# everpeace/kube-throttler

Hardware: AMD Instinct MI355X
Metric: pod_throttle_decisions_per_sec (higher is better)
Workload: dtype int64; 1 GPU; configs[2]: 1M pods x 1k Throttle+ClusterThrottle, D=8; pods_total=1000000, pods_per_gpu=1000000, throttles=1000, dims=8, labels_per_pod=8, namespaces=64, step=reconcile(aggregate+allreduce+finalize,apply)+check(all pods), streams=one, kernel_variant=indexed, parallelism=pods row-sharded x1, throttles replicated, exchange=none

## Files before the change

include/kt_engine.h:

```cpp
#ifndef KT_ENGINE_H
#define KT_ENGINE_H

#include <stdint.h>
#include "kt_snapshot.h"

#ifdef __cplusplus
extern "C" {
#endif

#define KT_OK 0
#define KT_ERR_INVALID_ARGUMENT (-1)
#define KT_ERR_OUT_OF_RANGE (-2)
#define KT_ERR_DEVICE (-3)
#define KT_ERR_OVERFLOW_RISK (-4)
#define KT_ERR_NOT_READY (-5)
#define KT_ERR_NO_DEVICE (-6)
#define KT_ERR_UNSUPPORTED (-7)

#define KT_STATUS_NOT_AFFECTED 0
#define KT_STATUS_NOT_THROTTLED 1
#define KT_STATUS_ACTIVE 2
#define KT_STATUS_INSUFFICIENT 3
#define KT_STATUS_POD_REQUESTS_EXCEEDS_THRESHOLD 4
#define KT_STATUS_ERROR 255
// ... 135 lines not shown
#define KT_KERNEL_FINALIZE 2
#define KT_KERNEL_PREPARE 3
#define KT_KERNEL_REDUCE 4
#define KT_KERNEL_COUNT 5
int32_t kt_timing_enable(kt_engine* e, int32_t on);
int32_t kt_timing_read(kt_engine* e, int32_t kernel, double* total_ms, int64_t* launches);
int32_t kt_timing_reset(kt_engine* e);
int32_t kt_synchronize(kt_engine* e, void* stream);
const char* kt_kernel_name(kt_engine* e, int32_t kernel);
#define KT_COUNTER_FEW_CHECKS 0
#define KT_COUNTER_COMPILES 1
#define KT_COUNTER_INDEX_CHUNKS 2
#define KT_COUNTER_INDEX_WORDS 3
#define KT_COUNTER_NS_WORD_VISITS 4
#define KT_COUNTER_NS_ROWS 5
#define KT_COUNTER_NS_CHUNK_VISITS 6
#define KT_COUNTER_INDEX_IMAGE_WORDS 7
#define KT_COUNTER_SLOW_THROTTLES 8
#define KT_COUNTER_PACKED_WORDS 9
#define KT_COUNTER_VIEW_BUILDS 10
#define KT_COUNTER_AGG_WORKGROUPS 11
#define KT_COUNTER_MATCH_CACHE_BUILDS 12
#define KT_COUNTER_MATCH_CACHE_SCANS 13
#define KT_COUNTER_MATCH_CACHE_PLANES 14
#define KT_COUNTER_MATCH_CACHE_AGG_SCANS 15
int64_t kt_counter(kt_engine* e, int32_t which);
int32_t kt_paged_check(kt_engine* const* pages, int32_t n_pages, int64_t n, const int64_t* pod_rows, int32_t on_equal,
                       uint64_t* out_summary, uint8_t* out_status);
int32_t kt_paged_reconcile(kt_engine* const* pages, int32_t n_pages, int64_t now_s, int32_t now_ns, uint32_t flags, int32_t n,
                           const kt_status* page_out, uint8_t* replaced_any, uint8_t* error_any);
int32_t kt_paged_admit(kt_engine* const* pages, int32_t n_pages, int64_t n, const int64_t* pod_rows, int32_t on_equal, uint32_t flags,
                       uint64_t* out_summary, uint8_t* out_status);
int32_t kt_paged_admit_gangs(kt_engine* const* pages, int32_t n_pages, int64_t n, const int64_t* pod_rows, int64_t n_gangs,
                             const int64_t* gang_off, int32_t on_equal, uint32_t flags, uint64_t* out_summary, uint8_t* out_status,
                             uint8_t* out_gang_admitted);
int32_t kt_paged_headroom(kt_engine* const* pages, int32_t n_pages, int64_t n, const int64_t* pod_rows, int32_t on_equal,
                          int64_t cap, int64_t* out_copies, int32_t* out_limiting);
#define KT_PREEMPT_REPRIEVE 0x1u
int32_t kt_paged_preempt(kt_engine* const* pages, int32_t n_pages, int64_t n, const int64_t* pod_rows, int64_t n_cand,
                         const int64_t* cand_rows, int64_t now_s, int32_t now_ns, int32_t on_equal, uint32_t flags,
                         int64_t* out_prefix , uint8_t* out_victims );
int32_t kt_paged_preempt_gangs(kt_engine* const* pages, int32_t n_pages, int64_t n, const int64_t* pod_rows, int64_t n_gangs,
                               const int64_t* gang_off, int64_t n_cand, const int64_t* cand_rows, int64_t now_s, int32_t now_ns,
                               int32_t on_equal, uint32_t flags, int64_t* out_prefix ,
                               uint8_t* out_victims , int64_t* out_blocker );
int32_t kt_paged_forecast(kt_engine* const* pages, int32_t n_pages, int64_t n, const int64_t* pod_rows, int64_t n_inst, const int64_t* inst_s,
                          const int32_t* inst_ns, int32_t on_equal, int64_t* out_first ,
                          uint8_t* out_verdicts );

int32_t kt_debug_reload_env(kt_engine* e);

int32_t kt_debug_match_planes(kt_engine* e, int32_t which, int64_t cap, uint64_t* out, int64_t* out_rows, int64_t* out_n, int32_t* out_planes);

#ifdef __cplusplus
}
#endif
#endif
```

kube_throttler_amd/csrc/kt_engine.cpp:

```cpp
#include "kt_engine_impl.h"

thread_local std::string g_create_error;

static bool getenv_flag(const char* name) {
  const char* v = getenv(name);
  return v && *v && *v != '0';
}
static void load_env_switches(kt_engine* e) {
  for (int k = 0; k < kSwCount; ++k) e->sw[k] = getenv_flag(kEnvSwitchName[k]);
  const char* cap = getenv("KT_REPRIEVE_LDS_CAP");
  const long cap_n = cap ? strtol(cap, nullptr, 10) : 0;
  e->reprieve_lds_cap_limit = cap_n > 0 && cap_n <= 0x7FFFFFFFl ? (uint32_t)cap_n : 0u;
}

void recs_invalidate_and_drain(kt_engine* e) {
  {
    std::lock_guard<std::mutex> g(e->recs_mu);
    e->recs_valid = false;
  }
  if (e->few_ready) std::lock_guard<std::mutex> drain(e->small_mu);
}

hipStream_t pick_stream(kt_engine* e, void* s) {
  hipStream_t st = s ? (hipStream_t)s : e->own_stream;
// ... 271 lines not shown
  e->cfg.kernel_variant &= 0xFF;
  if (e->incremental && e->cfg.kernel_variant != 0) {
    g_create_error = "KT_VARIANT_INCREMENTAL needs the indexed kernels (kernel_variant 0)";
    delete e;
    return KT_ERR_INVALID_ARGUMENT;
  }
  hipError_t r = hipSetDevice(dev);
  if (r == hipSuccess) r = hipStreamCreateWithFlags(&e->own_stream, hipStreamNonBlocking);
  const size_t cap = (size_t)cfg->pod_capacity;
  e->pods.cap = cfg->pod_capacity;
  e->pods.D = e->D;
  e->pods.L = e->L;
  e->pods.DS = kt::req_stride(e->D);
  e->pods.LS = kt::label_stride(e->L);
  if (r == hipSuccess) r = kt::kt_alloc_device((void**)&e->pods.ns, cap * 4);
  if (r == hipSuccess) r = kt::kt_alloc_device((void**)&e->pods.flags, cap * 4);
  if (r == hipSuccess) r = kt::kt_alloc_device((void**)&e->pods.req, cap * 8 * e->pods.DS);
  if (r == hipSuccess) r = kt::kt_alloc_device((void**)&e->pods.lpair, cap * 4 * e->pods.LS);
  if (r == hipSuccess) r = kt::kt_alloc_device((void**)&e->pods.lkey, cap * 4 * e->pods.LS);
  if (r == hipSuccess) r = kt::kt_alloc_device((void**)&e->pods.meta, cap * 8);
  e->pods.LA = 8;
  if (r == hipSuccess) r = hipMemsetAsync(e->pods.flags, 0, cap * 4, e->own_stream);
  if (r == hipSuccess) r = hipMemsetAsync(e->pods.meta, 0, cap * 8, e->own_stream);
  if (r == hipSuccess) r = hipMemsetAsync(e->pods.lpair, 0, cap * 4 * e->pods.LS, e->own_stream);
  if (r == hipSuccess) r = hipMemsetAsync(e->pods.lkey, 0, cap * 4 * e->pods.LS, e->own_stream);
  if (r == hipSuccess) r = hipStreamSynchronize(e->own_stream);
  if (r != hipSuccess) {
    g_create_error = std::string("device setup failed: ") + hipGetErrorString(r);
    kt_engine_destroy(e);
    return KT_ERR_DEVICE;
  }
  e->ns.resize((size_t)cfg->namespace_capacity);
  e->thr.resize((size_t)cfg->throttle_capacity);
  *out = e;
  return KT_OK;
}

int32_t kt_engine_destroy(kt_engine* e) {
  if (!e) return KT_OK;
  (void)hipSetDevice(e->device);
  (void)hipDeviceSynchronize();
  if (e->comm) (void)rccl()->CommDestroy(e->comm);
  if (e->pods.ns) (void)hipFree(e->pods.ns);
  if (e->pods.flags) (void)hipFree(e->pods.flags);
  if (e->pods.req) (void)hipFree(e->pods.req);
  if (e->pods.lpair) (void)hipFree(e->pods.lpair);
  if (e->pods.lkey) (void)hipFree(e->pods.lkey);
  if (e->pods.meta) (void)hipFree(e->pods.meta);
  e->d_latom.release();
  e->d_overflow.release();
  e->views.release();
  e->d_carry.release();
  e->d_mc.release();
  if (e->h_mc_rows) (void)hipHostFree(e->h_mc_rows);
  if (e->mc_rows_ev) (void)hipEventDestroy(e->mc_rows_ev);
  e->d_slab_tag.release();
  e->d_row_mask.release();
  e->d_req_sums.release();
  e->d_ticket.release();
  if (e->h_small) (void)hipHostFree(e->h_small);
  if (e->h_few) (void)hipHostFree(e->h_few);
  e->d_few_acc.release();
  e->d_few_ticket.release();
  for (auto& ev : e->recs_ev)
    if (ev) (void)hipEventDestroy(ev);
  if (e->admit_pages_ev) (void)hipEventDestroy(e->admit_pages_ev);
  if (e->preempt_pages_ev) (void)hipEventDestroy(e->preempt_pages_ev);
  if (e->small_stream) (void)hipStreamDestroy(e->small_stream);
  if (e->h_stage) (void)hipHostFree(e->h_stage);
  for (auto& sl : e->ev_slots) {
    if (sl.ev) (void)hipEventDestroy(sl.ev);
    if (sl.h) (void)hipHostFree(sl.h);
  }
  if (e->h_overflow) (void)hipHostFree(e->h_overflow);
  DevBuf<uint32_t>* u32s[] = {&e->d_thr_term_off, &e->d_term_thr, &e->d_term_req_off, &e->d_req_key, &e->d_req_val_off,
                              &e->d_req_val, &e->d_ns_term_ok, &e->d_thr_flags, &e->d_thrl_flag, &e->d_thrl_has,
                              &e->d_ovr_off, &e->d_out_thrl_flag, &e->d_out_thrl_has};
  for (auto* b : u32s) b->release();
  DevBuf<uint8_t>* u8s[] = {&e->d_term_flags, &e->d_req_op, &e->d_ns_valid, &e->d_ovr_flags, &e->d_out_calc_updated,
                            &e->d_out_thrl_pod, &e->d_out_error, &e->d_recs2[0], &e->d_recs2[1], &e->d_wvimg[0], &e->d_wvimg[1], &e->d_status, &e->d_stage, &e->d_ev_stage, &e->d_slab, &e->d_admit, &e->d_admit_pages, &e->d_preempt_pages, &e->d_gang_out};
  for (auto* b : u8s) b->release();
  e->d_status_fp.release(); e->d_spec_fp.release(); e->d_summary.release(); e->d_rows.release(); e->d_gang_off.release();
  e->d_headroom_copies.release(); e->d_headroom_limiting.release();
  e->d_preempt_prefix.release(); e->d_preempt_victims.release(); e->d_preempt_partial.release(); e->d_preempt_gang_off.release(); e->d_preempt_blocker.release(); e->d_reprieve_ws.release();
  e->d_forecast_first.release(); e->d_forecast_verdicts.release(); e->d_forecast_inst_s.release(); e->d_forecast_inst_ns.release();
  e->d_forecast_gang_off.release(); e->d_forecast_blocker.release();
  e->d_used_hi.release(); e->d_out_used_hi.release();
  e->d_ovr_begin_s.release(); e->d_ovr_end_s.release(); e->d_ovr_begin_ns.release(); e->d_ovr_end_ns.release();
  e->d_partial.release();
  e->d_out_next_s.release();
  e->d_agg.release();
  e->d_out_next_ns.release();
  e->d_sp.release();
  AmountDev* ams[] = {&e->d_spec, &e->d_calc, &e->d_used, &e->d_reserved, &e->d_ovr_thr, &e->d_out_used, &e->d_out_calc};
  for (auto* a : ams) a->release();
  kt::release_index(e->dindex);
  for (auto& f : e->fam)
    for (auto& pr : f.pool) {
      (void)hipEventDestroy(pr.first);
      (void)hipEventDestroy(pr.second);
    }
  if (e->own_stream) (void)hipStreamDestroy(e->own_stream);
  delete e;
  return KT_OK;
}

// ... 70 lines not shown
  *launches = (int64_t)f.used;
  return KT_OK;
}

int32_t kt_synchronize(kt_engine* e, void* stream) {
  if (!e) return KT_ERR_INVALID_ARGUMENT;
  LaunchLock lk(e);
  KT_HIP(e, hipSetDevice(e->device));
  KT_HIP(e, hipStreamSynchronize(pick_stream(e, stream)));
  return KT_OK;
}

int32_t kt_debug_reload_env(kt_engine* e) {
  if (!e) return KT_ERR_INVALID_ARGUMENT;
  StateLock lk(e);
  load_env_switches(e);
  return KT_OK;
}

int32_t kt_debug_match_planes(kt_engine* e, int32_t which, int64_t cap, uint64_t* out, int64_t* out_rows, int64_t* out_n, int32_t* out_planes) {
  if (!e || which < 0 || which > 1 || cap < 0 || !out_n || !out_planes || (cap > 0 && !out)) return KT_ERR_INVALID_ARGUMENT;
  LaunchLock lk(e);
  KT_HIP(e, hipSetDevice(e->device));
  if (e->last_stream) KT_HIP(e, hipStreamSynchronize(e->last_stream));
  *out_n = 0, *out_planes = 0;
  const uint32_t planes = e->mc_planes;
  if (!e->mc_valid || e->program_dirty || e->mc_gen != e->program_gen || e->mc_planes_gen != e->program_gen || !e->mc_pending.empty() || !e->d_mc.p ||
      planes == 0u || planes > (uint32_t)kt::kMatchPlanes || e->d_mc.cap < (size_t)planes * (size_t)e->cfg.pod_capacity)
    return e->fail(KT_ERR_NOT_READY, "no current match cache: none built for this program, or rows wait for their refresh");
  const ScanView& cv = e->views.countable;
  hipStream_t s = e->own_stream;
  int64_t n = e->pod_rows_hi;
  uint64_t stride = (uint64_t)e->cfg.pod_capacity;
  const uint64_t* src = e->d_mc.p;
  if (which == 1) {
    if (!cv.valid || !cv.mx_valid || !cv.mx.p || !cv.rows.p || !cv.d_n.p || cv.mx_planes != planes || cv.mx.cap < (size_t)planes * ((size_t)cv.cap + 1))
      return e->fail(KT_ERR_NOT_READY, "the countable scan view holds no current planes");
    unsigned long long dn = 0;
    KT_HIP(e, hipMemcpyAsync(&dn, cv.d_n.p, 8, hipMemcpyDeviceToHost, s));
    KT_HIP(e, hipStreamSynchronize(s));
    n = (int64_t)std::min<unsigned long long>(std::min<unsigned long long>(dn, cv.n + (unsigned long long)cv.extra), (unsigned long long)cv.cap);
    stride = (uint64_t)cv.cap + 1u, src = cv.mx.p;
  }
  *out_n = n, *out_planes = (int32_t)planes;
  if (cap == 0 || n == 0) return KT_OK;
  if (cap < n) return e->fail(KT_ERR_OUT_OF_RANGE, "cap=%lld < %lld", (long long)cap, (long long)n);
  for (uint32_t k = 0; k < planes; ++k)
    KT_HIP(e, hipMemcpyAsync(out + (size_t)k * (size_t)cap, src + (size_t)k * stride, (size_t)n * 8, hipMemcpyDeviceToHost, s));
  if (which == 1 && out_rows) KT_HIP(e, hipMemcpyAsync(out_rows, cv.rows.p, (size_t)n * 8, hipMemcpyDeviceToHost, s));
  KT_HIP(e, hipStreamSynchronize(s));
  return KT_OK;
}

int64_t kt_counter(kt_engine* e, int32_t which) {
  if (!e) return -1;
  switch (which) {
    case KT_COUNTER_FEW_CHECKS: return e->few_served.load(std::memory_order_relaxed);
    case KT_COUNTER_COMPILES: return e->n_compiles.load(std::memory_order_relaxed);
    case KT_COUNTER_INDEX_CHUNKS: return e->ctr_index_chunks.load(std::memory_order_relaxed);
    case KT_COUNTER_INDEX_WORDS: return e->ctr_index_words.load(std::memory_order_relaxed);
    case KT_COUNTER_NS_ROWS: return e->ctr_ns_rows.load(std::memory_order_relaxed);
    case KT_COUNTER_NS_WORD_VISITS: return e->ctr_ns_word_visits.load(std::memory_order_relaxed);
    case KT_COUNTER_NS_CHUNK_VISITS: return e->ctr_ns_chunk_visits.load(std::memory_order_relaxed);
    case KT_COUNTER_INDEX_IMAGE_WORDS: return e->ctr_index_image_words.load(std::memory_order_relaxed);
    case KT_COUNTER_SLOW_THROTTLES: return e->ctr_slow_throttles.load(std::memory_order_relaxed);
    case KT_COUNTER_PACKED_WORDS: return e->ctr_packed_words.load(std::memory_order_relaxed);
    case KT_COUNTER_AGG_WORKGROUPS: return e->ctr_agg_workgroups.load(std::memory_order_relaxed);
    case KT_COUNTER_VIEW_BUILDS: return e->ctr_view_builds.load(std::memory_order_relaxed);
    case KT_COUNTER_MATCH_CACHE_BUILDS: return e->ctr_mc_builds.load(std::memory_order_relaxed);
    case KT_COUNTER_MATCH_CACHE_SCANS: return e->ctr_mc_scans.load(std::memory_order_relaxed);
    case KT_COUNTER_MATCH_CACHE_PLANES: return e->ctr_mc_planes.load(std::memory_order_relaxed);
    case KT_COUNTER_MATCH_CACHE_AGG_SCANS: return e->ctr_mc_agg_scans.load(std::memory_order_relaxed);
    default: return -1;
  }
}

int32_t kt_partial_layout(int32_t n_dims, int32_t* stride, int32_t* off_values, int32_t* off_presence, int32_t* off_pods,
                          int32_t* off_errors) {
  if (n_dims < 1 || n_dims > KT_MAX_DIMS) return KT_ERR_INVALID_ARGUMENT;
  if (stride) *stride = kt::partial_stride(n_dims);
  if (off_values) *off_values = 0;
  if (off_presence) *off_presence = kt::partial_off_presence(n_dims);
  if (off_pods) *off_pods = kt::partial_off_pods(n_dims);
  if (off_errors) *off_errors = kt::partial_off_errors(n_dims);
  return KT_OK;
}

const char* kt_kernel_name(kt_engine* e, int32_t kernel) {
  if (!e || kernel < 0 || kernel >= KT_KERNEL_COUNT) return "";
  return e->last_kernel[kernel];
}
```

kube_throttler_amd/csrc/kt_engine_check.cpp:

```cpp
#include "kt_engine_impl.h"

static int32_t ensure_check_recs(kt_engine* e, int32_t on_equal, int DT, hipStream_t s) {
  if (e->recs_valid && e->recs_eq == (on_equal != 0) && e->recs_DT == DT) return KT_OK;
  recs_invalidate_and_drain(e);
  {
    TimedLaunch tl(e, KT_KERNEL_PREPARE, s);
    kt::launch_prepare_check(e->tt, e->thr_rows_hi, e->D, DT, on_equal != 0, e->recs_ptr(), req_bound(e), s);
  }
  if (e->few_ready) KT_HIP(e, hipEventRecord(e->recs_ev[e->recs_cur], s));
  std::lock_guard<std::mutex> g(e->recs_mu);
  e->recs_ev_pending[e->recs_cur] = e->few_ready;
  e->recs_prev_valid = false;
  ++e->recs_seq[e->recs_cur];
  e->recs_valid = true;
  e->recs_eq = on_equal != 0;
  e->recs_DT = DT;
  return KT_OK;
}

int32_t match_cache_for_scan(kt_engine* e, hipStream_t s, kt::MatchCacheArgs& mc) {
  mc = kt::MatchCacheArgs();
  if (e->sw[kSw_NO_MATCH_CACHE] || e->cfg.kernel_variant != 0 || e->incremental || e->program_dirty || e->pod_rows_hi <= 0) return KT_OK;
  if (!kt::match_cache_fits(e->dindex) || e->hindex.has_slow || e->n_overflow != 0 || e->pods.LA > 8 || !e->pods.latom) return KT_OK;
  if (e->mc_planes_gen != e->program_gen) {
    const kt::BmChunk& ch = e->dindex.h_chunks[0];
    const uint32_t* rng = (const uint32_t*)(e->hindex.bm_images.data() + ch.img_off + ch.off_nsl_rng);
    uint32_t longest = 0;
    for (uint32_t n = 0; n < e->hindex.n_ns; ++n) longest = std::max(longest, rng[2 * n + 1] - rng[2 * n]);
    e->mc_planes = longest, e->mc_planes_gen = e->program_gen;
    e->ctr_mc_planes.store((int64_t)longest, std::memory_order_relaxed);
  }
  const uint32_t planes = e->mc_planes;
  if (!kt::check_replays_match_cache(e->pods, e->sp, e->dindex, planes, e->n_overflow != 0, e->sw[kSw_CHECK_ONE_PER_CU])) return KT_OK;
  const uint64_t stride = (uint64_t)e->cfg.pod_capacity;
  ScanView& cv = e->views.countable;
  kt::MatchViewPlanes vp;
  if (cv.valid && cv.mx_valid && cv.mx.p && cv.pos.p && cv.mx_planes == planes && e->mc_gen == e->program_gen)
    vp.mx = cv.mx.p, vp.pos = cv.pos.p, vp.stride = (uint64_t)cv.cap + 1u;
  else
    cv.mx_valid = false;
  if (!e->mc_valid || e->mc_gen != e->program_gen) {
    if (e->d_mc.cap < (size_t)planes * stride) {
      if (e->last_stream) KT_HIP(e, hipStreamSynchronize(e->last_stream));
      KT_HIP(e, e->d_mc.reserve((size_t)planes * stride));
    }
    order_behind_ingest(e, s);
    if (!kt::launch_build_match_cache(e->pods, e->pod_rows_hi, nullptr, e->dindex, e->d_mc.p, stride, planes, s, &vp)) {
      cv.mx_valid = false;
      return KT_OK;
    }
    KT_HIP(e, hipGetLastError());
    e->mc_valid = true, e->mc_gen = e->program_gen;
    e->mc_pending.clear();
    e->ctr_mc_builds.fetch_add(1, std::memory_order_relaxed);
  } else if (!e->mc_pending.empty()) {
    const size_t n = e->mc_pending.size();
    if (!e->h_mc_rows) {
      KT_HIP(e, hipHostMalloc((void**)&e->h_mc_rows, (size_t)kPatchBatchMax * 8, hipHostMallocDefault));
      KT_HIP(e, hipEventCreateWithFlags(&e->mc_rows_ev, hipEventDisableTiming));
    } else if (e->mc_rows_ev_used) {
      KT_HIP(e, hipEventSynchronize(e->mc_rows_ev));
    }
    memcpy(e->h_mc_rows, e->mc_pending.data(), n * 8);
    order_behind_ingest(e, s);
    if (!kt::launch_build_match_cache(e->pods, (int64_t)n, e->h_mc_rows, e->dindex, e->d_mc.p, stride, planes, s, &vp)) {
      e->mc_valid = false, cv.mx_valid = false;
      e->mc_pending.clear();
      return KT_OK;
    }
    KT_HIP(e, hipGetLastError());
    KT_HIP(e, hipEventRecord(e->mc_rows_ev, s));
    e->mc_rows_ev_used = true;
    e->mc_pending.clear();
  }
  mc.mw = e->d_mc.p, mc.stride = stride, mc.planes = planes;
  return KT_OK;
}

static int32_t check_launch_locked(kt_engine* e, int64_t n, const int64_t* pod_rows, int32_t on_equal, uint32_t flags,
                                   hipStream_t s, bool allow_small = true) {
  e->headroom_ready = false;
  e->preempt_ready = false;
  e->forecast_ready = false;
  if (pod_rows) {
    for (int64_t i = 0; i < n; ++i)
      if (pod_rows[i] < 0 || pod_rows[i] >= e->cfg.pod_capacity)
        return e->fail(KT_ERR_OUT_OF_RANGE, "pod row %lld", (long long)pod_rows[i]);
  } else if (n > e->cfg.pod_capacity) {
    return e->fail(KT_ERR_OUT_OF_RANGE, "n=%lld > pod_capacity", (long long)n);
  }
  int32_t rc = ensure_ready(e, s);
  if (rc != KT_OK) return rc;
  const bool want_status = (flags & KT_CHECK_STATUS_MATRIX) != 0;
  const size_t T = (size_t)e->thr_rows_hi;
  if (e->d_summary.cap < (size_t)n + 1 || (want_status && e->d_status.cap < (size_t)n * T + 64) ||
      (pod_rows && e->d_rows.cap < (size_t)n + 1)) {
    if (e->last_stream) KT_HIP(e, hipStreamSynchronize(e->last_stream));
    KT_HIP(e, e->d_summary.reserve((size_t)n + 1));
    if (want_status) KT_HIP(e, e->d_status.reserve((size_t)n * T + 64));
    if (pod_rows) KT_HIP(e, e->d_rows.reserve((size_t)n + 1));
  }
  const bool small = allow_small && e->cfg.kernel_variant != 1 && n > 0 && n <= kt::kCheckSmallMax;
  kt::CheckSmall sm{};
  if (small) {
    if (!e->h_small) {
      KT_HIP(e, hipHostMalloc((void**)&e->h_small, (size_t)kt::kCheckSmallMax * 8, hipHostMallocMapped));
      KT_HIP(e, e->d_ticket.reserve(16));
      KT_HIP(e, hipMemsetAsync(e->d_ticket.p, 0, 16 * 4, s));
    }
    sm.ticket = e->d_ticket.p;
    sm.host_summary = e->h_small;
    if (pod_rows && n <= 8) {
      sm.n_inline = (uint32_t)n;
      for (int64_t k = 0; k < 8; ++k) sm.inline_rows[k] = pod_rows[k < n ? k : n - 1];
    }
  }
  if (pod_rows && n && !sm.n_inline) {
    KT_HIP(e, hipMemcpyAsync(e->d_rows.p, pod_rows, (size_t)n * 8, hipMemcpyHostToDevice, s));
    KT_HIP(e, hipStreamSynchronize(s));
  }
  const int DT = e->cfg.kernel_variant == 1 ? kt::dt_bucket(e->D) : kt::dt_bucket_ix(e->D);
  if ((rc = ensure_check_recs(e, on_equal, DT, s)) != KT_OK) return rc;
  kt::MatchCacheArgs mc;
  if (e->cfg.kernel_variant != 1 && !pod_rows && !small && !want_status && n > 0 && n <= e->cfg.pod_capacity && e->dindex.n_chunks == 1 &&
      !e->sw[kSw_FORCE_NS_ORDER] && !e->sw[kSw_CHECK_ONE_PER_CU]) {
    if ((rc = match_cache_for_scan(e, s, mc)) != KT_OK) return rc;
  }
  {
    TimedLaunch tl(e, KT_KERNEL_CHECK, s);
    if (e->cfg.kernel_variant == 1)
      kt::launch_check_dense(e->pods, n, pod_rows ? e->d_rows.p : nullptr, e->sp, e->uses_keys, e->recs_ptr(),
                             e->d_summary.p, want_status ? e->d_status.p : nullptr, s),
          e->last_kernel[KT_KERNEL_CHECK] = "kt_check_dense";
    else {
      const bool by_ns = !pod_rows && !small && n == e->pod_rows_hi && (e->dindex.n_chunks > 1 || e->sw[kSw_FORCE_NS_ORDER]) && !e->sw[kSw_NO_NS_ORDER];
      if (by_ns && (rc = settle_view_patches(e, s)) != KT_OK) return rc;
      ScanView& av = e->views.all_rows;
      if (by_ns && (!av.valid || (int64_t)av.n != e->pod_rows_hi)) {
        const ViewSpec spec{false, true, kt::check_sweep_blocks, e->pod_rows_hi, false};
        KT_HIP(e, e->d_carry.reserve((size_t)e->pod_rows_hi + 1));
        if ((rc = list_view_rows(e, av, spec, s)) != KT_OK) return rc;
        if ((rc = copy_view_records(e, av, spec, 0, s)) != KT_OK) return rc;
        av.valid = true;
      }
      kt::CheckByNs view{av.meta.p, av.latom.p, e->d_carry.p};
      if (by_ns && av.range_G) view.wg_range = av.range.p, view.wg_range_G = av.range_G;
      if (by_ns && !want_status && e->dindex.n_slow == 0 && e->n_overflow == 0 && e->dindex.n_chunks > 1 && !e->sw[kSw_NO_VERDICT_IMAGES]) {
        const int b = e->recs_cur;
        if (e->wvimg_seq[b] != e->recs_seq[b] || e->wvimg_gen[b] != e->program_gen || e->wvimg_DT[b] != DT) {
          KT_HIP(e, e->d_wvimg[b].reserve(kt::verdict_images_bytes(e->dindex.bm_words, e->D)));
          TimedLaunch tl2(e, KT_KERNEL_PREPARE, s);
          kt::launch_build_verdict_images(e->dindex, e->dindex.bm_words, e->recs_ptr(), e->thr_rows_hi, e->D, e->d_wvimg[b].p, s);
          e->wvimg_seq[b] = e->recs_seq[b], e->wvimg_gen[b] = e->program_gen, e->wvimg_DT[b] = DT;
        }
        view.wv_img = e->d_wvimg[b].p, view.wv_total_words = e->dindex.bm_words;
      }
      const char* k = kt::launch_check_indexed(e->pods, n, by_ns ? av.rows.p : pod_rows ? e->d_rows.p : nullptr, e->sp, e->d_sp.p, e->dindex,
                                               e->recs_ptr(), e->d_summary.p, want_status ? e->d_status.p : nullptr, s,
                                               small ? &sm : nullptr, e->n_overflow != 0, by_ns ? &view : nullptr, e->sw[kSw_CHECK_ONE_PER_CU],
                                               mc.mw ? &mc : nullptr);
      if (mc.used) e->ctr_mc_scans.fetch_add(1, std::memory_order_relaxed);
      if (!k) return e->fail(KT_ERR_UNSUPPORTED, "%d throttle rows exceed the indexed check kernel's LDS budget (use kernel_variant 1)", e->thr_rows_hi);
      e->last_kernel[KT_KERNEL_CHECK] = k;
    }
  }
  KT_HIP(e, hipGetLastError());
  e->check_n = n;
  e->check_in_h_small = small;
  e->check_T = e->thr_rows_hi;
  e->check_has_status = want_status;
  e->check_ready = true;
  e->last_stream = s;
  return KT_OK;
}

int32_t kt_check_launch(kt_engine* e, int64_t n, const int64_t* pod_rows, int32_t on_equal, uint32_t flags, void* stream) {
  if (!e || n < 0) return KT_ERR_INVALID_ARGUMENT;
  LaunchLock lk(e);
  KT_HIP(e, hipSetDevice(e->device));
// ... 1286 lines not shown
```

kube_throttler_amd/csrc/kt_engine_impl.h:

```cpp
#pragma once
#include <hip/hip_runtime.h>
#include <dlfcn.h>

#include <algorithm>
#include <cstdarg>
#include <cstdio>
#include <cstring>
#include <memory>
#include <atomic>
#include <chrono>
#include <mutex>
#include <shared_mutex>
#include <string>
#include <unordered_set>
#include <vector>

#include "../../include/kt_engine.h"
#include "kt_index.h"
#include "kt_launch.h"


#define KT_INTERNAL __attribute__((visibility("hidden")))

namespace kte {
// ... 50 lines not shown
struct HostNamespace {
  bool valid = false;
  std::vector<std::pair<uint32_t, uint32_t>> labels;
};

template <class T>
struct DevBuf {
  T* p = nullptr;
  size_t cap = 0;
  hipError_t reserve(size_t n) {
    if (n <= cap && p) return hipSuccess;
    if (p) (void)hipFree(p);
    p = nullptr;
    cap = 0;
    size_t want = std::max<size_t>(n, 16);
    hipError_t e = kt::kt_alloc_device((void**)&p, want * sizeof(T));
    if (e == hipSuccess) cap = want;
    return e;
  }
  void release() {
    if (p) (void)hipFree(p);
    p = nullptr;
    cap = 0;
  }
};

struct AmountDev {
  DevBuf<int64_t> v;
  DevBuf<uint32_t> present;
  DevBuf<int64_t> count;
  DevBuf<uint8_t> has_count;
  hipError_t reserve(size_t n, int D) {
    hipError_t e;
    if ((e = v.reserve(n * D)) != hipSuccess) return e;
    if ((e = present.reserve(n)) != hipSuccess) return e;
    if ((e = count.reserve(n)) != hipSuccess) return e;
    return has_count.reserve(n);
  }
  kt::AmountTab tab() const { return kt::AmountTab{v.p, present.p, count.p, has_count.p}; }
  void release() { v.release(); present.release(); count.release(); has_count.release(); }
};

struct ScanView {
  DevBuf<int64_t> rows;
  DevBuf<unsigned long long> d_n;
  unsigned long long n = 0;
  DevBuf<uint64_t> meta;
  DevBuf<uint16_t> latom;
  DevBuf<int64_t> req;
  DevBuf<uint64_t> pk;
  kt::PackPlan pack;
  DevBuf<int32_t> pos;
  DevBuf<uint64_t> mx;
  uint32_t mx_planes = 0;
  bool mx_valid = false;
  DevBuf<uint32_t> range;
  int range_G = 0;
  int64_t cap = 0;
  int64_t extra = 0;
  bool by_ns = false;
  bool valid = false;
  void release() { rows.release(); d_n.release(); meta.release(); latom.release(); req.release(); pk.release(); pos.release(); range.release(); mx.release(); mx_valid = false; }
};
struct ViewSpec {
  bool countable_only;
  bool by_ns;
  int (*grid)(int64_t);
  int64_t rows_cap;
  bool requests;
};
struct ScanViews {
  ScanView countable;
  ScanView all_rows;
  DevBuf<unsigned long long> d_ns_cursor;
  std::vector<unsigned long long> h_ns_end;
  std::vector<uint32_t> h_range;
  DevBuf<uint32_t> d_dirty;
  bool check_dirty = false;
  void invalidate() { countable.valid = false, all_rows.valid = false; }
  void release() { countable.release(); all_rows.release(); d_ns_cursor.release(); d_dirty.release(); }
};

struct AmountHostFlat {
  std::vector<int64_t> v;
  std::vector<uint32_t> present;
  std::vector<int64_t> count;
  std::vector<uint8_t> has_count;
  void resize(size_t n, int D) {
    v.assign(n * D, 0);
    present.assign(n, 0);
    count.assign(n, 0);
    has_count.assign(n, 0);
  }
  void set(size_t i, int D, const HostAmount& a) {
    for (int d = 0; d < D; ++d) v[i * D + d] = (a.present >> d) & 1u ? a.v[d] : 0;
    present[i] = a.present;
    count[i] = a.has_count ? a.count : 0;
    has_count[i] = a.has_count;
  }
  void get(size_t i, int D, HostAmount& a) const {
    for (int d = 0; d < D; ++d) a.v[d] = v[i * D + d];
    a.present = present[i];
    a.count = count[i];
    a.has_count = has_count[i];
  }
};

struct TimingFamily {
  std::vector<std::pair<hipEvent_t, hipEvent_t>> pool;
  size_t used = 0;
};

}
using namespace kte;

extern thread_local std::string g_create_error;


enum EnvSwitch { kSw_FEED_NO_STAGE, kSw_FORCE_NS_ORDER, kSw_INGEST_EVENT_WAIT, kSw_NO_FEED_FEW, kSw_NO_FEED_FUSION, kSw_NO_FUSED, kSw_NO_NS_ORDER, kSw_NO_PACK, kSw_NO_SCAN_VIEW, kSw_NO_SWEEP, kSw_NO_VERDICT_IMAGES, kSw_NO_WG_RANGES, kSw_SYNC_INGEST, kSw_INGEST_TRUST_FENCE, kSw_NO_VIEW_PATCH, kSw_CHECK_ONE_PER_CU, kSw_AGG_SMALL_WINDOW, kSw_AGG_ONE_PER_CU, kSw_NO_MATCH_CACHE, kSw_NO_MATCH_CACHE_AGG, kSwCount };
static const char* const kEnvSwitchName[kSwCount] = {"KT_FEED_NO_STAGE", "KT_FORCE_NS_ORDER", "KT_INGEST_EVENT_WAIT", "KT_NO_FEED_FEW", "KT_NO_FEED_FUSION", "KT_NO_FUSED", "KT_NO_NS_ORDER", "KT_NO_PACK", "KT_NO_SCAN_VIEW", "KT_NO_SWEEP", "KT_NO_VERDICT_IMAGES", "KT_NO_WG_RANGES", "KT_SYNC_INGEST", "KT_INGEST_TRUST_FENCE", "KT_NO_VIEW_PATCH", "KT_CHECK_ONE_PER_CU", "KT_AGG_SMALL_WINDOW", "KT_AGG_ONE_PER_CU", "KT_NO_MATCH_CACHE", "KT_NO_MATCH_CACHE_AGG"};
struct kt_engine {
  bool sw[kSwCount] = {};
  uint32_t reprieve_lds_cap_limit = 0;
  kt_config cfg{};
  std::shared_mutex mu;
  std::mutex small_mu;
  std::mutex ingest_mu;
  std::mutex op_mu;
  std::mutex recs_mu;
  std::mutex err_mu;
  std::string err;
  int device = 0;
  hipStream_t own_stream = nullptr;
  int D = 0, L = 0;

  kt::PodTable pods{};
  int64_t pod_rows_hi = 0;
  unsigned __int128 max_abs[KT_MAX_DIMS] = {0};
  uint64_t or_abs[KT_MAX_DIMS] = {0};
  ScanViews views;
  bool cut_plain = false;
  void* cur_launch_lock = nullptr;
  std::atomic<int64_t> ctr_index_chunks{0}, ctr_index_words{0}, ctr_index_image_words{0}, ctr_ns_rows{0}, ctr_ns_word_visits{0}, ctr_ns_chunk_visits{0}, ctr_slow_throttles{0}, ctr_packed_words{0}, ctr_agg_workgroups{0}, ctr_view_builds{0}, ctr_mc_builds{0}, ctr_mc_scans{0}, ctr_mc_planes{0}, ctr_mc_agg_scans{0};
  DevBuf<uint16_t> d_latom;
  DevBuf<uint64_t> d_mc;
  int64_t* h_mc_rows = nullptr;
  hipEvent_t mc_rows_ev = nullptr;
  bool mc_rows_ev_used = false;
  std::vector<int64_t> mc_pending;
  bool mc_valid = false;
  uint64_t mc_gen = ~0ull;
  uint64_t mc_planes_gen = ~0ull;
  uint32_t mc_planes = 0;
  DevBuf<unsigned long long> d_overflow;
  unsigned long long n_overflow = 0;
  static constexpr int kEvSlots = 8;
  static constexpr size_t kEvSlotBytes = 64 * 1024;
  struct EvSlot {
    uint8_t* h = nullptr;
    hipEvent_t ev = nullptr;
    bool used = false;
  } ev_slots[kEvSlots];
  int ev_next = 0;
  std::atomic<bool> ingest_pending{false};
  hipEvent_t ingest_ev = nullptr;
  std::atomic<hipEvent_t> ingest_unretired{nullptr};
  hipStream_t ingest_stream = nullptr;
  unsigned long long* h_overflow = nullptr;
  bool overflow_in_flight = false;
  unsigned long long ingest_seq = 0;
  unsigned long long ingest_spin_seq = 0;
  bool req_sums_valid = true;
  unsigned __int128 req_sum_bound[KT_MAX_DIMS] = {0};
  DevBuf<unsigned long long> d_req_sums;
  DevBuf<uint8_t> d_row_mask;
  DevBuf<uint32_t> d_slab_tag;
  uint32_t slab_epoch = 0;
  bool neg_seen = false;

  std::vector<HostNamespace> ns;
  uint64_t ns_gen = 1;
  int32_t ns_rows_hi = 0;
  int64_t pod_ns_hi = 0;
  size_t ns_compiled = 0;
  std::vector<HostThrottle> thr;
  int32_t thr_rows_hi = 0;
  bool program_dirty = true;
  bool spec_dirty = false;
  bool status_host_dirty = true;
  bool reserved_dev_newer = false;
  bool incremental = false;
  bool agg_valid = false;
  DevBuf<unsigned long long> d_agg;
  bool recs_valid = false;
  bool recs_eq = false;
  int recs_DT = 0;
  bool status_dev_newer = false;

// ... 283 lines not shown
```

kube_throttler_amd/csrc/kt_engine_reconcile.cpp:

```cpp
#include "kt_engine_impl.h"

Rccl* rccl() {
  static Rccl r;
  static std::once_flag once;
  std::call_once(once, [] {
    for (const char* name : {"librccl.so.1", "librccl.so", "/opt/rocm/lib/librccl.so.1"}) {
      r.lib = dlopen(name, RTLD_NOW | RTLD_LOCAL);
      if (r.lib) break;
    }
    if (!r.lib) {
      r.err = std::string("cannot load librccl.so: ") + (dlerror() ? dlerror() : "?");
      return;
    }
    r.GetUniqueId = (decltype(r.GetUniqueId))dlsym(r.lib, "ncclGetUniqueId");
    r.CommInitRank = (decltype(r.CommInitRank))dlsym(r.lib, "ncclCommInitRank");
    r.AllReduce = (decltype(r.AllReduce))dlsym(r.lib, "ncclAllReduce");
    r.CommDestroy = (decltype(r.CommDestroy))dlsym(r.lib, "ncclCommDestroy");
    r.GetErrorString = (decltype(r.GetErrorString))dlsym(r.lib, "ncclGetErrorString");
    if (!r.GetUniqueId || !r.CommInitRank || !r.AllReduce || !r.CommDestroy) r.err = "librccl.so lacks the nccl* entry points";
  });
  return &r;
}
static constexpr int kNcclInt64 = 4, kNcclSum = 0;

// ... 171 lines not shown
    e->agg_pending = true, e->agg_words = words, e->agg_gen = e->program_gen;
    return KT_OK;
  }
  const bool by_ns = (e->dindex.n_chunks > 1 || e->sw[kSw_FORCE_NS_ORDER]) && !e->sw[kSw_NO_NS_ORDER];
  if ((rc = settle_view_patches(e, s)) != KT_OK) return rc;
  ScanView& cv = e->views.countable;
  if (cv.valid && cv.extra && !(!e->sw[kSw_NO_SCAN_VIEW] && (by_ns || e->dindex.n_chunks == 1))) cv.valid = false;
  const bool two_view = !e->sw[kSw_NO_SCAN_VIEW] && !e->sw[kSw_NO_PACK] && e->cfg.kernel_variant != 1 && !by_ns && !e->incremental && !e->wide &&
                        e->dindex.n_chunks == 1;
  const kt::AggTwoLaunch two_launch{!e->sw[kSw_AGG_ONE_PER_CU], e->sw[kSw_AGG_SMALL_WINDOW], e->n_overflow != 0, e->pods.LA};
  if (cv.valid && cv.pack.headroom >= (uint32_t)kt::kPackHeadroomBitsTwo && !(two_view && kt::aggregate_two_per_cu_fits(e->dindex, cv.pack, two_launch)))
    cv.valid = false;
  kt::MatchCacheArgs mc;
  if (two_view && two_launch.enabled && !two_launch.small_window && !two_launch.overflow_pods && e->pods.LA <= 8 && !e->sw[kSw_NO_MATCH_CACHE_AGG] &&
      !e->sw[kSw_CHECK_ONE_PER_CU]) {
    if ((rc = match_cache_for_scan(e, s, mc)) != KT_OK) return rc;
  }
  if (e->cfg.kernel_variant != 1 && (!cv.valid || cv.by_ns != by_ns)) {
    if (e->last_stream && e->last_stream != s) KT_HIP(e, hipStreamSynchronize(e->last_stream));
    const ViewSpec spec{true, by_ns, kt::aggregate_blocks, e->cfg.pod_capacity, true};
    if ((rc = list_view_rows(e, cv, spec, s)) != KT_OK) return rc;
    const int64_t headroom = std::min<int64_t>(std::max<int64_t>(65536, (int64_t)cv.n / 16), e->cfg.pod_capacity - (int64_t)cv.n);
    const bool view_scan = !e->sw[kSw_NO_SCAN_VIEW] && (cv.by_ns || e->dindex.n_chunks == 1);
    cv.pack = kt::PackPlan();
    if (view_scan && !e->incremental && !e->wide && !e->sw[kSw_NO_PACK] && !e->dindex.has_long) {
      const int64_t cap = (int64_t)cv.n + headroom;
      uint64_t slab_pods = kt::aggregate_slab_pods(cap, kt::aggregate_blocks(cap));
      if (cv.range_G) slab_pods = std::max<uint64_t>(slab_pods, (uint64_t)kt::wg_range_cap((int64_t)cv.n, cv.range_G) + 64u);
      cv.pack = kt::make_pack_plan(e->D, e->max_abs, e->or_abs, e->neg_seen, slab_pods, true, kt::pack_max_words(e->D));
      if (cv.pack.nw && cv.pack.rec_bytes > e->dindex.cut_thr_bytes) cv.pack = kt::PackPlan();
      if (two_view && cv.pack.nw) {
        const uint64_t slab_pods2 = kt::aggregate_slab_pods(cap, kt::aggregate_blocks(cap, kt::kAggWorkgroupsTwo));
        const kt::PackPlan two = kt::make_pack_plan(e->D, e->max_abs, e->or_abs, e->neg_seen, slab_pods2, false, 3,
                                                    kt::kPackHeadroomBitsTwo);
        if (two.nw && kt::aggregate_two_per_cu_fits(e->dindex, two, two_launch)) cv.pack = two;
      }
    }
    if (!cv.pack.nw && kt::agg_rec_bytes(e->D, e->incremental) > e->dindex.cut_thr_bytes) {
      upgrade_launch_lock(e);
      e->cut_plain = true, e->program_dirty = true;
      return aggregate_locked(e, s, allow_fused);
    }
    if (!e->sw[kSw_NO_SCAN_VIEW] && (rc = copy_view_records(e, cv, spec, headroom, s)) != KT_OK) return rc;
    cv.valid = true;
  }
  const bool replay = mc.mw != nullptr && mc.planes <= (uint32_t)kt::kMatchReplay && two_view && cv.valid && cv.pack.nw && cv.pk.p &&
                      cv.pack.headroom >= (uint32_t)kt::kPackHeadroomBitsTwo && kt::aggregate_two_per_cu_fits(e->dindex, cv.pack, two_launch);
  if (replay && !(cv.mx_valid && cv.mx_planes == mc.planes)) {
    const size_t need = (size_t)mc.planes * ((size_t)cv.cap + 1);
    if (cv.mx.cap < need) {
      if (e->last_stream) KT_HIP(e, hipStreamSynchronize(e->last_stream));
      KT_HIP(e, cv.mx.reserve(need));
    }
    const int64_t listed = std::min<int64_t>((int64_t)cv.n + cv.extra, cv.cap);
    kt::launch_gather_match_planes(mc.mw, mc.stride, mc.planes, cv.rows.p, listed, cv.mx.p, (uint64_t)cv.cap + 1u, s);
    KT_HIP(e, hipGetLastError());
    cv.mx_planes = mc.planes, cv.mx_valid = true;
  }
  if (words && e->clean_partial != (const void*)e->partial()) KT_HIP(e, hipMemsetAsync(e->partial(), 0, words * 8, s));
  e->clean_partial = nullptr;
  {
    TimedLaunch tl(e, KT_KERNEL_AGGREGATE, s);
    std::unique_ptr<TimedLaunch> tr;
    const bool defer = allow_fused && !e->incremental && !e->wide && e->dindex.n_chunks == 1 && !e->sw[kSw_NO_FUSED];
    auto after_scan = [&]() {
      tl.stop_now();
      if (!(defer && cv.pack.nw)) tr.reset(new TimedLaunch(e, KT_KERNEL_REDUCE, s));
    };
    const int n_pass = e->wide ? 2 : 1;
    for (int pass = 0; pass < n_pass; ++pass) {
      const int limb = e->wide ? pass + 1 : 0;
      unsigned long long* target = e->partial() + (size_t)pass * block_words;
      if (e->cfg.kernel_variant == 1) {
        kt::launch_aggregate_dense(e->pods, e->pod_rows_hi, e->sp, e->uses_keys, target, s, limb);
        e->last_kernel[KT_KERNEL_AGGREGATE] = "kt_aggregate_dense";
      } else {
        kt::AggScan sc;
        sc.n = (int64_t)cv.n, sc.rows = cv.rows.p, sc.counts = e->incremental, sc.nonneg = !e->neg_seen;
        sc.overflow_pods = two_launch.overflow_pods;
        sc.small_window = two_launch.small_window;
        sc.one_per_cu = !two_launch.enabled;
        sc.limb = limb;
        sc.by_ns = !e->sw[kSw_NO_SCAN_VIEW] && (cv.by_ns || e->dindex.n_chunks == 1);
        if (sc.by_ns) sc.n += cv.extra;
        if (sc.by_ns) sc.v_meta = cv.meta.p, sc.v_latom = cv.latom.p, sc.v_req = cv.pack.nw ? nullptr : cv.req.p;
        if (sc.by_ns && cv.pack.nw) sc.pk = &cv.pack, sc.v_pk = cv.pk.p;
        if (sc.by_ns && cv.by_ns && cv.range_G) sc.wg_range = cv.range.p, sc.wg_range_G = cv.range_G;
        if ((rc = slab_tags(e, sc, s)) != KT_OK) return rc;
        sc.defer_reduce = defer && sc.pk != nullptr;
        if (replay && sc.by_ns && sc.v_pk && limb == 0) sc.v_mx = cv.mx.p, sc.mx_stride = (uint64_t)cv.cap + 1u, sc.mx_planes = cv.mx_planes;
        const char* k = kt::launch_aggregate_indexed(e->pods, sc, e->sp, e->d_sp.p, e->dindex, target, e->d_slab.p, s,
                                                     pass == 0 ? std::function<void()>(after_scan) : std::function<void()>());
        if (sc.replayed) e->ctr_mc_agg_scans.fetch_add(1, std::memory_order_relaxed);
        if (!k && sc.refused) return e->fail(KT_ERR_OUT_OF_RANGE, "aggregate launch refused: %s", sc.refused);
        if (!k) return e->fail(KT_ERR_UNSUPPORTED, "a chunk of the selector index exceeds the aggregate kernel's LDS budget (use kernel_variant 1)");
        e->last_kernel[KT_KERNEL_AGGREGATE] = k;
        e->ctr_agg_workgroups.store((int64_t)sc.launched_blocks, std::memory_order_relaxed);
        e->ctr_packed_words.store(sc.launched_packed ? (int64_t)cv.pack.nw : 0, std::memory_order_relaxed);
        if (sc.defer_reduce && sc.launched_packed) e->fused_pending = true, e->fused_nb = sc.launched_blocks, e->fused_epoch = sc.epoch, e->fused_pack = cv.pack;
        e->last_kernel[KT_KERNEL_REDUCE] = e->fused_pending ? "(in kt_reduce_finalize_packed)" : sc.launched_packed ? "kt_reduce_packed_slabs" : "kt_reduce_bitmap_slabs";
      }
    }
  }
  KT_HIP(e, hipGetLastError());
  if (e->incremental) {
    KT_HIP(e, e->d_agg.reserve(words + 1));
    if (words) KT_HIP(e, hipMemcpyAsync(e->d_agg.p, e->partial(), words * 8, hipMemcpyDeviceToDevice, s));
    e->agg_valid = true;
  }
  e->last_stream = s;
  e->agg_pending = true, e->agg_words = words, e->agg_gen = e->program_gen;
  return KT_OK;
}

int32_t delta_scan(kt_engine* e, int64_t n, const int64_t* rows_dev, int64_t row0, int sign, hipStream_t s) {
  if (!e->incremental || !e->agg_valid || n <= 0 || e->thr_rows_hi == 0) return KT_OK;
  kt::AggScan sc;
  sc.n = n, sc.rows = rows_dev, sc.row0 = row0, sc.counts = true, sc.sign = sign, sc.overflow_pods = e->n_overflow != 0;
  sc.small_window = e->sw[kSw_AGG_SMALL_WINDOW];
  int32_t rc = slab_tags(e, sc, s);
  if (rc != KT_OK) return rc;
  const char* k = kt::launch_aggregate_indexed(e->pods, sc, e->sp, e->d_sp.p, e->dindex, e->d_agg.p, e->d_slab.p, s, nullptr);
  if (!k && sc.refused) return e->fail(KT_ERR_OUT_OF_RANGE, "aggregate launch refused: %s", sc.refused);
  if (!k) return e->fail(KT_ERR_UNSUPPORTED, "a chunk of the selector index exceeds the aggregate kernel's LDS budget");
  KT_HIP(e, hipGetLastError());
  return KT_OK;
}

int32_t finalize_locked(kt_engine* e, int64_t now_s, int32_t now_ns, uint32_t flags, hipStream_t s, bool consume,
                               const uint8_t* row_mask) {
  KT_CHECK_PARTIALS_CURRENT(e, "kt_finalize_launch");
  int32_t rc = ensure_ready(e, s);
  if (rc != KT_OK) return rc;
  if (!e->agg_pending) e->agg_wide = e->wide;
  e->agg_pending = false;
  kt::ReconcileOut out{e->d_out_used.tab(), e->d_out_calc.tab(), e->d_out_used_hi.p, e->d_out_calc_updated.p, e->d_out_thrl_flag.p,
                       e->d_out_thrl_has.p, e->d_out_thrl_pod.p, e->d_out_error.p, e->d_out_next_s.p, e->d_out_next_ns.p};
  const bool apply = (flags & KT_RECONCILE_APPLY) != 0;
  const int rec_DT = e->cfg.kernel_variant == 1 ? kt::dt_bucket(e->D) : kt::dt_bucket_ix(e->D);
  bool keep_prev;
  int wbuf;
  {
    std::lock_guard<std::mutex> g(e->recs_mu);
// ... 210 lines not shown
```

kube_throttler_amd/csrc/kt_index.cpp:

```cpp
#include "kt_index.h"

#include <algorithm>
#include <chrono>
#include <cstdio>
#include <cstdlib>
#include <cstring>
#include <map>
#include <thread>
#include <unordered_map>
#include <unordered_set>

#include "../../include/kt_snapshot.h"

namespace kt {

namespace {

struct BT {
  uint32_t g, t;
  bool adj;
  bool slow;
  uint32_t need;
  uint32_t n_pos;
  int64_t pos_key[5];
// ... 826 lines not shown
        if (g.cnt[w]++ == 0) g.words.push_back(w);
      g.ideal = std::min(g.ideal, ideal_n);
    }
    std::vector<ChunkPlan> plan;
    Maxima mx;
    for (Group& g : groups) {
      ordered(g.words, g.cnt);
      std::vector<uint32_t> cuts;
      (void)chunks_of(seq, g.cnt, g.members.size(), &mx, &cuts);
      size_t i0 = 0;
      for (uint32_t i1 : cuts) {
        ChunkPlan cp;
        cp.all = false, cp.served = g.members;
        cp.words.assign(seq.begin() + i0, seq.begin() + i1);
        std::sort(cp.words.begin(), cp.words.end());
        plan.push_back(std::move(cp));
        i0 = i1;
      }
    }
    return plan;
  }
  size_t visits(const std::vector<ChunkPlan>& plan) const {
    size_t v = 0;
    std::vector<uint8_t> in_chunk(W, 0);
    for (const ChunkPlan& cp : plan) {
      for (uint32_t w : cp.words) in_chunk[w] = 1;
      auto touches = [&](uint32_t n) {
        for (uint32_t w : ns_words[n])
          if (in_chunk[w]) return true;
        return false;
      };
      if (cp.all) {
        for (uint32_t n = 0; n < n_ns; ++n) v += touches(n);
      } else {
        for (uint32_t n : cp.served) v += touches(n);
      }
      for (uint32_t w : cp.words) in_chunk[w] = 0;
    }
    return v;
  }

  void emit(const std::vector<ChunkPlan>& plan_in) {
    const std::vector<uint64_t>&any = out.full_any, &vet = out.full_veto, &nsrows = out.full_nsrows;
    const std::vector<WordHdr>& hdr = out.full_hdr;
    const std::vector<uint32_t>&term_t = out.full_term_t, &term_g = out.full_term_g, &term_rank = out.full_term_rank;
    const std::vector<uint8_t>& real = out.full_real;
    uint64_t slab_run = 0;
    out.bm_chunks.clear();
    out.bm_images.clear();
    size_t total_words = 0;
    for (const ChunkPlan& cp : plan_in) total_words += cp.words.size();
    out.bm_images.reserve(((size_t)Rp * total_words * 8 * fam + total_words * (sizeof(WordHdr) + 64 * 10 + 64)) * 5 / 4 + plan_in.size() * ((size_t)n_ns + 8) * 4 * 4);
    out.bm_chunk_ns.clear();
    const uint32_t nsw = (n_ns + 31) / 32;
    out.ns_words = nsw ? nsw : 1u;
    out.bm_max_lds = 0, out.bm_max_thr = 0, out.bm_max_words = 0, out.bm_slab_bytes = 0;
    out.bm_rank_t.clear();
    out.ns_word_visits = 0, out.ns_chunk_visits = 0;
    uint32_t w_run = 0;
    Maxima mx;
    std::vector<ChunkPlan> work(plan_in.rbegin(), plan_in.rend());
    std::vector<uint64_t> irows;
    std::vector<uint32_t> words;
    while (!work.empty()) {
      ChunkPlan cp = std::move(work.back());
      work.pop_back();
      BmChunk ch{};
      const uint32_t nw = (uint32_t)cp.words.size();
      words = cp.words;
      uint32_t nv = 0;
      if (veto) {
        std::stable_partition(words.begin(), words.end(), [&](uint32_t w) { return has_veto(w); });
        for (uint32_t w : words) nv += has_veto(w);
      }
      const uint32_t veto_cols = veto ? nv + (nv < nw ? 1u : 0u) : 0u;
      ch.n_words = nw, ch.n_veto = nv;
      ch.zero_col = veto && nv < nw ? (nw + nv) * Rp * 8u : 0u;
      ch.ns_base = 0u, ch.ns_cnt = 0xFFFFFFFFu;
      ch.col_rows = Rp;
      std::vector<uint32_t> nsl_rng((size_t)n_ns * 2, 0u);
      std::vector<NsWord> nsl, cur;
      {
        std::unordered_map<uint64_t, std::vector<uint32_t>> by_hash;
        size_t si = 0;
        for (uint32_t n = 0; n < n_ns; ++n) {
          bool serve = cp.all;
          if (!cp.all) {
            while (si < cp.served.size() && cp.served[si] < n) ++si;
            serve = si < cp.served.size() && cp.served[si] == n;
          }
          if (!serve) continue;
          cur.clear();
          uint64_t h = 1469598103934665603ull;
          for (uint32_t w = 0; w < nw; ++w) {
            const uint64_t m = nsrows[(size_t)n * W + words[w]];
            if (!m) continue;
            cur.push_back(NsWord{w, word_form[words[w]], m});
            h = (h ^ w) * 1099511628211ull, h = (h ^ m) * 1099511628211ull;
          }
          if (cur.empty()) continue;
          uint32_t begin = ~0u;
          std::vector<uint32_t>& cands = by_hash[h];
          for (uint32_t b0 : cands) {
            if ((size_t)b0 + cur.size() > nsl.size()) continue;
            bool same = true;
            for (size_t q = 0; q < cur.size() && same; ++q) same = nsl[b0 + q].w == cur[q].w && nsl[b0 + q].mask == cur[q].mask;
            if (same) { begin = b0; break; }
          }
          if (begin == ~0u) {
            begin = (uint32_t)nsl.size();
            nsl.insert(nsl.end(), cur.begin(), cur.end());
            cands.push_back(begin);
          }
          nsl_rng[(size_t)n * 2] = begin, nsl_rng[(size_t)n * 2 + 1] = begin + (uint32_t)cur.size();
        }
      }
      const uint32_t rank0 = (uint32_t)out.bm_rank_t.size();
      std::vector<uint32_t> it((size_t)nw * 64, 0u), ig((size_t)nw * 64, 0u);
      std::vector<uint16_t> ir((size_t)nw * 64, 0);
      {
        uint32_t last_rank = ~0u;
        for (uint32_t w = 0; w < nw; ++w)
          for (uint32_t k = 0; k < 64; ++k) {
            const size_t c = (size_t)words[w] * 64 + k;
            it[(size_t)w * 64 + k] = term_t[c], ig[(size_t)w * 64 + k] = term_g[c];
            if (!real[c]) continue;
            if (term_rank[c] != last_rank) last_rank = term_rank[c], out.bm_rank_t.push_back(term_t[c] & kTermRowMask);
            ir[(size_t)w * 64 + k] = (uint16_t)(((uint32_t)out.bm_rank_t.size() - 1u - rank0) | ((term_t[c] & kTermAdj) ? kRankAdj : 0u));
            ch.has_slow |= (hdr[c >> 6].slow >> (c & 63)) & 1ull ? 1u : 0u;
            ch.has_adj |= (term_t[c] & kTermAdj) ? 1u : 0u;
          }
      }
      ch.n_thr = (uint32_t)out.bm_rank_t.size() - rank0;
      ch.rank0 = ch.n_thr ? rank0 : 0u;
      const size_t lds = image_lds(nw, nv, nsl.size());
      if (!fits(lds, nw, ch.n_thr, mx) && nw > 1 && all_splittable) {
        out.bm_rank_t.resize(rank0);
        ChunkPlan lo = cp, hi = cp;
        lo.words.assign(cp.words.begin(), cp.words.begin() + nw / 2), hi.words.assign(cp.words.begin() + nw / 2, cp.words.end());
        work.push_back(std::move(hi)), work.push_back(std::move(lo));
        continue;
      }
      ch.w0 = w_run;
      w_run += nw;
      irows.assign((size_t)Rp * (nw + veto_cols), 0ull);
      const size_t veto_plane = (size_t)Rp * nw;
      for (uint32_t r = 0; r < R; ++r)
        for (uint32_t w = 0; w < nw; ++w) {
          irows[(size_t)w * Rp + r] = any[(size_t)r * W + words[w]];
          if (veto && w < nv) irows[veto_plane + (size_t)w * Rp + r] = vet[(size_t)r * W + words[w]];
        }
      std::vector<WordHdr> ihdr(nw);
      for (uint32_t w = 0; w < nw; ++w) ihdr[w] = hdr[words[w]];
      for (uint32_t n = 0; n < n_ns; ++n) out.ns_word_visits += (int64_t)(nsl_rng[(size_t)n * 2 + 1] - nsl_rng[(size_t)n * 2]);
      {
        const size_t b0 = out.bm_chunk_ns.size();
        out.bm_chunk_ns.resize(b0 + out.ns_words, 0u);
        for (uint32_t n = 0; n < n_ns; ++n)
          if (nsl_rng[(size_t)n * 2 + 1] > nsl_rng[(size_t)n * 2]) out.bm_chunk_ns[b0 + (n >> 5)] |= 1u << (n & 31), ++out.ns_chunk_visits;
      }
      const void* src[7] = {irows.data(), ihdr.data(), nsl_rng.data(), nsl.data(), it.data(), ir.data(), ig.data()};
      const size_t bytes[7] = {irows.size() * 8, ihdr.size() * sizeof(WordHdr), nsl_rng.size() * 4, nsl.size() * sizeof(NsWord),
                               it.size() * 4,    ir.size() * 2,                 ig.size() * 4};
      uint32_t* offs[7] = {nullptr, &ch.off_hdr, &ch.off_nsl_rng, &ch.off_nsl, &ch.off_term_t, &ch.off_term_rank, &ch.off_term_g};
      size_t o = 0;
      const size_t img0 = out.bm_images.size();
      for (int k = 0; k < 7; ++k) {
        if (offs[k]) *offs[k] = (uint32_t)o;
        if (k == 4) ch.lds_bytes = (uint32_t)o;
        o += align16(bytes[k]);
      }
      out.bm_images.resize(img0 + o, 0);
      size_t oo = 0;
      for (int k = 0; k < 7; ++k) {
        if (bytes[k]) memcpy(out.bm_images.data() + img0 + oo, src[k], bytes[k]);
        oo += align16(bytes[k]);
      }
      ch.img_off = (uint32_t)img0, ch.img_bytes = (uint32_t)o;
      ch.slab_off = (uint32_t)(slab_run / 16);
      slab_run += agg_slab_area_bytes(ch.n_thr, thr_bytes);
      mx.lds = std::max(mx.lds, (size_t)ch.lds_bytes), mx.thr = std::max(mx.thr, (size_t)ch.n_thr), mx.nw = std::max(mx.nw, (size_t)nw);
      out.bm_max_lds = std::max(out.bm_max_lds, ch.lds_bytes);
      out.bm_max_thr = std::max(out.bm_max_thr, ch.n_thr);
      out.bm_max_words = std::max(out.bm_max_words, ch.n_words);
      out.bm_chunks.push_back(ch);
      if (getenv("KT_DEBUG_CHUNKS"))
        fprintf(stderr, "chunk %zu: %u words (%u with veto columns; first %u) lds %u B thr %u, serves %zu namespaces, %zu list entries\n", out.bm_chunks.size() - 1,
                nw, nv, nw ? words[0] : 0u, ch.lds_bytes, ch.n_thr, cp.all ? (size_t)n_ns : cp.served.size(), nsl.size());
      out.bm_slab_bytes = slab_run;
    }
    out.img_words = w_run;
  }
};

}

void cut_chunks(HostIndex& out, uint32_t agg_budget, uint32_t chk_budget, uint32_t thr_bytes, uint32_t chk_word, uint32_t thr_bytes_packed) {
// ... 26 lines not shown
  if (want_grouped || getenv("KT_CUT_PLAN_AUTO")) {
    std::vector<ChunkPlan> grouped = cut.plan_grouped();
    const size_t v_global = cut.visits(plan), v_grouped = cut.visits(grouped);
    if (getenv("KT_DEBUG_CHUNKS"))
      fprintf(stderr, "cut_chunks: global %zu chunks / %zu namespace visits, grouped %zu chunks / %zu namespace visits\n", plan.size(), v_global,
              grouped.size(), v_grouped);
    if (want_grouped || (v_grouped * 5 <= v_global * 4 && grouped.size() <= std::max<size_t>(8 * plan.size(), 64) && grouped.size() <= 2048))
      plan.swap(grouped), out.cut_grouped = true;
  }
  cut.emit(plan);
}

template <class T>
static hipError_t up(T*& dev, size_t& cap, const std::vector<T>& h, hipStream_t s) {
  const size_t need = h.size() + 1;
  if (need > cap || !dev) {
    if (dev) (void)hipFree(dev);
    dev = nullptr;
    cap = 0;
    hipError_t e = kt_alloc_device((void**)&dev, need * sizeof(T));
    if (e != hipSuccess) return e;
    cap = need;
  }
  if (!h.empty()) return hipMemcpyAsync(dev, h.data(), h.size() * sizeof(T), hipMemcpyHostToDevice, s);
  return hipSuccess;
}

void index_group_counts(HostIndex& h, uint32_t T) {
  h.thr_ngrp.assign(T, 0u);
  for (uint32_t t : h.bm_rank_t)
    if (t < T) ++h.thr_ngrp[t];
  h.nogroup.clear();
  for (uint32_t t = 0; t < T; ++t)
    if (!h.thr_ngrp[t]) h.nogroup.push_back(t);
}

hipError_t upload_index(const HostIndex& h, IndexDev& d, hipStream_t s) {
  hipError_t e;
  if ((e = up(d.thr_ngrp, d.cap_thr_ngrp, h.thr_ngrp, s)) != hipSuccess) return e;
  if ((e = up(d.nogroup, d.cap_nogroup, h.nogroup, s)) != hipSuccess) return e;
  d.n_nogroup = (uint32_t)h.nogroup.size();
  {
    const std::vector<uint32_t> zeros(h.thr_ngrp.size() + 1, 0u);
    if ((e = up(d.grp_arrive, d.cap_grp_arrive, zeros, s)) != hipSuccess) return e;
    if ((e = hipStreamSynchronize(s)) != hipSuccess) return e;
  }
  if ((e = up(d.slow_thr, d.cap_slow, h.slow_thr, s)) != hipSuccess) return e;
  d.n_slow = (uint32_t)h.slow_thr.size();
  if ((e = up(d.bm_blob, d.cap_bm_blob, h.bm_images, s)) != hipSuccess) return e;
  if ((e = up(d.bm_chunks, d.cap_bm_chunks, h.bm_chunks, s)) != hipSuccess) return e;
  if ((e = up(d.bm_rank_t, d.cap_bm_rank_t, h.bm_rank_t, s)) != hipSuccess) return e;
  if ((e = up(d.bm_chunk_ns, d.cap_bm_chunk_ns, h.bm_chunk_ns, s)) != hipSuccess) return e;
  d.ns_words = h.ns_words;
  if ((e = up(d.atom_table, d.cap_atom_table, h.atom_table, s)) != hipSuccess) return e;
  d.atom_mask = (uint32_t)h.atom_table.size() - 1;
  d.h_chunks = h.bm_chunks;
  d.n_chunks = (uint32_t)h.bm_chunks.size();
  d.bm_max_lds = h.bm_max_lds, d.bm_max_thr = h.bm_max_thr, d.bm_max_words = h.bm_max_words, d.bm_rows = h.bm_rows;
  d.bm_words = h.img_words;
  d.cut_thr_bytes = h.cut_thr_bytes;
  d.has_long = h.has_long;
  d.bm_slab_bytes = h.bm_slab_bytes;
  d.has_veto = h.has_veto ? 1u : 0u;
  d.max_need = h.max_need;
  d.n_atoms = (uint32_t)h.atoms.size();
  d.has_key_atoms = h.n_key_atoms ? 1u : 0u;
  d.la = h.la, d.rich = h.rich;
  if (getenv("KT_DEBUG_LDS"))
    fprintf(stderr, "bitmap index: %u words, %u rows (veto %d, need %u), %zu chunks, largest LDS part %u B, largest chunk %u throttles / %u words, %zu slow throttles\n",
            h.bm_words, h.bm_rows, (int)h.has_veto, h.max_need, h.bm_chunks.size(), h.bm_max_lds, h.bm_max_thr, h.bm_max_words, h.slow_thr.size());
  return hipSuccess;
}

void release_index(IndexDev& d) {
  if (d.slow_thr) (void)hipFree(d.slow_thr);
  if (d.bm_blob) (void)hipFree(d.bm_blob);
  if (d.bm_chunks) (void)hipFree(d.bm_chunks);
  if (d.bm_rank_t) (void)hipFree(d.bm_rank_t);
  if (d.thr_ngrp) (void)hipFree(d.thr_ngrp);
  if (d.nogroup) (void)hipFree(d.nogroup);
  if (d.grp_arrive) (void)hipFree(d.grp_arrive);
  if (d.bm_chunk_ns) (void)hipFree(d.bm_chunk_ns);
  if (d.atom_table) (void)hipFree(d.atom_table);
  d = IndexDev();
}

PackPlan make_pack_plan(int D, const unsigned __int128* max_abs, const uint64_t* or_abs, bool neg_seen, uint64_t n_slab_pods, bool pad_odd,
                        uint32_t max_words, int headroom_bits) {
  PackPlan pk;
  if (neg_seen || D < 1 || D > 16 || n_slab_pods == 0 || headroom_bits < 1 || headroom_bits > 16) return pk;
  const int MW = (int)std::min<uint32_t>(max_words ? max_words : 1u, kPackMaxWords);
  auto bitlen = [](unsigned __int128 x) { int b = 0; while (x) ++b, x >>= 1; return b; };
  const int H = headroom_bits;
  struct F { int d; uint32_t pos, w; };
  std::vector<F> fields[kPackMaxWords];
  uint32_t fill[kPackMaxWords] = {0, 0, 0, 0, 0, 0, 0, 0};
  pk.cnt_width = (uint8_t)std::max(bitlen(n_slab_pods), H);
  if (pk.cnt_width > 64 - H) return PackPlan();
  fields[0].push_back({-1, 0u, pk.cnt_width});
  fill[0] = pk.cnt_width;
  uint32_t nw = 1;
  for (int d = 0; d < D; ++d) {
    if (max_abs[d] == 0) continue;
    const int sh = or_abs[d] ? __builtin_ctzll(or_abs[d]) : 0;
    const int w = std::max(bitlen((max_abs[d] >> sh) * (unsigned __int128)n_slab_pods), H);
    if (w > 64 - H) return PackPlan();
    int k = 0;
    while (k < MW && fill[k] + (uint32_t)w > 64u) ++k;
    if (k == MW) return PackPlan();
    pk.word[d] = (uint8_t)k, pk.pos[d] = (uint8_t)fill[k], pk.width[d] = (uint8_t)w, pk.shift[d] = (uint8_t)sh;
    fields[k].push_back({d, fill[k], (uint32_t)w});
    fill[k] += (uint32_t)w;
    nw = std::max(nw, (uint32_t)k + 1u);
  }
  for (uint32_t k = 0; k < nw; ++k) {
    const size_t n = fields[k].size();
    pk.top_pos[k] = (uint8_t)fields[k][n - 1].pos;
    for (size_t i = 0; i < n; ++i) {
      const F& f = fields[k][i];
      const bool top = i + 1 == n;
      const uint32_t cls = top ? 2u : (uint32_t)(i & 1u);
      if (cls == 0u) pk.even[k] |= ((1ull << f.w) - 1ull) << f.pos;
      const uint32_t desc = pack_desc(k, cls, top ? 0u : f.pos, f.w + (uint32_t)H, f.d >= 0 ? pk.shift[f.d] : 0u);
      if (f.d >= 0) pk.desc[f.d] = desc; else pk.cnt_desc = desc;
    }
  }
  pk.nw = nw;
  pk.headroom = (uint32_t)H;
  pk.stride = nw <= 2 ? 2u : nw <= 4 ? 4u : 8u;
  uint32_t units = nw + 1u;
  if (pad_odd && !(units & 1u)) ++units;
  pk.rec_bytes = units * 8u;
  return pk;
}

// ... 2 lines not shown
```

kube_throttler_amd/csrc/kt_index.h:

```cpp
#pragma once
#include <hip/hip_runtime.h>
#include <stdint.h>

#include <algorithm>
#include <functional>
#include <vector>

#include "kt_device.h"

namespace kt {

constexpr uint32_t kKeyAtom = 0x80000000u;
constexpr uint32_t kMaxIndexedTerms = 512;
constexpr uint32_t kCheckWordLds = 64u * 8u + 560u;

constexpr uint32_t kTermAdj = 0x80000000u;
constexpr uint32_t kTermReal = 0x40000000u;
constexpr uint32_t kTermRowMask = 0x000FFFFFu;
constexpr uint16_t kRankAdj = 0x8000u;

struct ThrInfo {
  bool live;
  bool cluster;
  uint32_t ns;
};

struct alignas(16) WordHdr {
  uint64_t univ;
  uint64_t m2;
  uint64_t m3;
  uint64_t slow;
  uint64_t m4;
  uint64_t m5;
  uint64_t pad[2];
};
static_assert(sizeof(WordHdr) == 64, "the scans address a word's header by a shift");
struct alignas(16) NsWord {
  uint32_t w;
  uint32_t flags;
  uint64_t mask;
};
constexpr uint32_t kNsWordVeto = 1u;
constexpr uint32_t kNsWordNeed3 = 2u;

struct BmChunk {
  uint32_t w0, n_words;
  uint32_t rank0, n_thr;
  uint32_t img_off, lds_bytes;
  uint32_t off_hdr, off_nsl_rng, off_nsl;
  uint32_t off_term_t, off_term_rank, off_term_g;
  uint32_t col_rows;
  uint32_t n_veto;
  uint32_t zero_col;
  uint32_t slab_off;
  uint32_t has_slow;
  uint32_t img_bytes;
  uint32_t has_adj;
  uint32_t ns_base, ns_cnt;
};

inline uint32_t image_col_rows(uint32_t rows) { return (rows + 31u) & ~31u; }

struct AtomId {
  uint32_t atom, id;
  uint32_t home;
};
constexpr int kAtomHomeShift = 48;
constexpr uint32_t kAtomIdMask = 0xFFFFu;

struct HostIndex {
  std::vector<uint32_t> slow_thr;
  uint32_t bm_words = 0;
  uint32_t bm_rows = 0;
  bool has_veto = false;
  uint32_t max_need = 0;
  uint32_t n_pair_keys = 0, n_key_atoms = 0;
  uint32_t n_keys = 0;
  bool has_slow = false;
  bool has_long = false;
  uint32_t la = 8;
  bool rich = false;
  std::vector<AtomId> atoms;
  std::vector<uint32_t> atom_key;
  std::vector<uint64_t> atom_table;
  std::vector<BmChunk> bm_chunks;
  std::vector<unsigned char> bm_images;
  std::vector<uint32_t> bm_rank_t;
  std::vector<uint32_t> thr_ngrp;
  std::vector<uint32_t> nogroup;
  std::vector<uint32_t> bm_chunk_ns;
  uint32_t ns_words = 0;
  uint32_t bm_max_lds = 0, bm_max_thr = 0, bm_max_words = 0;
  uint64_t bm_slab_bytes = 0;
  uint32_t cut_chk_budget = 0;
  uint32_t cut_thr_bytes = 0;
  bool agg_windowed = false;
  bool cut_grouped = false;
  uint32_t img_words = 0;
  int64_t ns_word_visits = 0;
  int64_t ns_chunk_visits = 0;
  uint32_t n_ns = 0;
  std::vector<uint64_t> full_any, full_veto, full_nsrows;
  std::vector<WordHdr> full_hdr;
  std::vector<uint32_t> full_term_t, full_term_g, full_term_rank;
  std::vector<uint8_t> full_real;
};

__host__ __device__ inline uint32_t agg_rec_bytes(int D, bool counts) {
  return (uint32_t)(((size_t)D * 8 + (counts ? (size_t)D * 4 + 4 : 8) + 15) & ~(size_t)15);
}

struct PackPlan {
  uint32_t nw = 0;
  uint32_t stride = 0;
  uint32_t rec_bytes = 0;
  uint8_t word[16] = {0}, pos[16] = {0}, width[16] = {0}, shift[16] = {0};
  uint8_t cnt_width = 0;
  uint64_t even[8] = {0, 0, 0, 0, 0, 0, 0, 0};
  uint8_t top_pos[8] = {0, 0, 0, 0, 0, 0, 0, 0};
  uint32_t desc[16] = {0};
  uint32_t cnt_desc = 0;
  uint32_t headroom = 0;
};
constexpr int kPackHeadroomBits = 8;
constexpr int kPackHeadroomBitsTwo = 9;
constexpr uint32_t kPackMaxWords = 8;
__host__ __device__ inline uint32_t pack_max_words(int D) { return D <= 8 ? 4u : kPackMaxWords; }
__host__ __device__ inline uint32_t packed_rec_max(int D) { return (pack_max_words(D) + 1u) * 8u; }
constexpr int kPackClasses = 3;
__host__ __device__ inline uint32_t pack_desc(uint32_t word, uint32_t cls, uint32_t pos, uint32_t wext, uint32_t shift) {
  return (word * 4u + cls) | pos << 8 | wext << 16 | shift << 24;
}
PackPlan make_pack_plan(int D, const unsigned __int128* max_abs, const uint64_t* or_abs, bool neg_seen, uint64_t n_slab_pods, bool pad_odd,
                        uint32_t max_words = kPackMaxWords, int headroom_bits = kPackHeadroomBits);

struct ViewPatch {
  uint64_t* vc_meta;
  uint16_t* vc_latom;
  int64_t* vc_req;
  uint64_t* vc_pk;
  int64_t* vc_rows;
  int32_t* pos_c;
  unsigned long long* n_c;
  int64_t cap_c;
  uint64_t* va_meta;
  uint16_t* va_latom;
  int32_t* pos_a;
  int64_t rows_a;
  uint32_t by_ns;
  uint32_t* dirty;
  PackPlan pk;
};

__host__ __device__ inline uint32_t atom_slot(uint32_t atom, uint32_t mask) { return ((atom * 0x9E3779B1u) >> 7) & mask; }

struct IndexDev {
  uint32_t* slow_thr = nullptr;
  uint32_t n_slow = 0;
  unsigned char* bm_blob = nullptr;
  BmChunk* bm_chunks = nullptr;
  uint32_t* bm_rank_t = nullptr;
  uint32_t* thr_ngrp = nullptr;
  uint32_t* nogroup = nullptr;
  uint32_t* grp_arrive = nullptr;
  uint32_t n_nogroup = 0;
  size_t cap_thr_ngrp = 0, cap_nogroup = 0, cap_grp_arrive = 0;
  uint32_t* bm_chunk_ns = nullptr;
  uint32_t ns_words = 0;
  uint64_t* atom_table = nullptr;
  uint32_t atom_mask = 0;
  std::vector<BmChunk> h_chunks;
  uint32_t n_chunks = 0, bm_max_lds = 0, bm_max_thr = 0, bm_max_words = 0, bm_rows = 0;
  uint64_t bm_slab_bytes = 0;
  uint32_t has_veto = 0, max_need = 0, n_atoms = 0, has_key_atoms = 0, la = 8;
  uint32_t bm_words = 0;
  uint32_t cut_thr_bytes = 0;
  bool has_long = false;
  bool rich = false;
  size_t cap_bm_blob = 0, cap_bm_chunks = 0, cap_bm_rank_t = 0, cap_bm_chunk_ns = 0, cap_atom_table = 0, cap_slow = 0;
};

void build_index(HostIndex& out, const std::vector<uint32_t>& thr_term_off, const std::vector<uint32_t>& term_thr,
                 const std::vector<uint8_t>& term_flags, const std::vector<uint32_t>& term_req_off,
                 const std::vector<uint8_t>& req_op, const std::vector<uint32_t>& req_key,
                 const std::vector<uint32_t>& req_val_off, const std::vector<uint32_t>& req_val,
                 const std::function<ThrInfo(uint32_t)>& thr_info, uint32_t n_ns,
                 const std::vector<uint32_t>& ns_term_ok, uint32_t gw, uint32_t agg_budget, uint32_t chk_budget, uint32_t thr_bytes,
                 int max_labels, const std::vector<uint32_t>* adm_in = nullptr, uint32_t chk_budget_full = 0,
                 uint32_t chk_word = kCheckWordLds, const HostIndex* atoms_from = nullptr, uint32_t thr_bytes_packed = 0);
void transpose_term_ns_bits(const std::vector<uint32_t>& in, size_t G, uint32_t nsw, uint32_t n_ns, uint32_t gw, std::vector<uint32_t>& out);
void parallel_for(size_t n, size_t min_per_part, const std::function<void(size_t, size_t, size_t)>& f, size_t* parts_out);
void cut_chunks(HostIndex& out, uint32_t agg_budget, uint32_t chk_budget, uint32_t thr_bytes, uint32_t chk_word = kCheckWordLds,
                uint32_t thr_bytes_packed = 0);
void index_group_counts(HostIndex& h, uint32_t T);
hipError_t upload_index(const HostIndex& h, IndexDev& d, hipStream_t s);
void release_index(IndexDev& d);

inline uint32_t atom_slots(uint32_t n_keys, int L) {
  const uint32_t ub = std::min<uint32_t>((uint32_t)L, n_keys);
  return ub <= 8 ? 8u : ub <= 16 ? 16u : 32u;
}

struct PodTable;
struct SelProgram;
uint32_t aggregate_fixed_lds();
uint32_t check_fixed_lds();
uint32_t check_word_lds(int D);
constexpr int kMatchPlanes = 8;
constexpr int kMatchReplay = 4;
struct MatchCacheArgs {
  const uint64_t* mw = nullptr;
  uint64_t stride = 0;
  uint32_t planes = 0;
  mutable bool used = false;
};
struct MatchViewPlanes {
  uint64_t* mx = nullptr;
  const int32_t* pos = nullptr;
  uint64_t stride = 0;
};
struct AggScan {
  int64_t n = 0;
  const int64_t* rows = nullptr;
  int64_t row0 = 0;
  bool counts = false;
  int sign = 1;
  bool nonneg = false;
  bool overflow_pods = false;
  bool by_ns = false;
  const uint64_t* v_meta = nullptr;
  const uint16_t* v_latom = nullptr;
  const int64_t* v_req = nullptr;
  uint32_t* slab_tag = nullptr;
  uint32_t epoch = 0;
  const uint32_t* wg_range = nullptr;
  int wg_range_G = 0;
  const PackPlan* pk = nullptr;
  const uint64_t* v_pk = nullptr;
  int limb = 0;
  bool small_window = false;
  bool defer_reduce = false;
  bool one_per_cu = false;
  const uint64_t* v_mx = nullptr;
  uint64_t mx_stride = 0;
  uint32_t mx_planes = 0;
  mutable bool replayed = false;
  mutable int launched_blocks = 0;
  mutable bool launched_packed = false;
  mutable const char* refused = nullptr;
};
constexpr int kAggWorkgroups = 256, kAggWorkgroupsTwo = 512;
constexpr uint32_t kSlabTagStride = kAggWorkgroupsTwo;
inline uint64_t agg_slab_area_bytes(uint32_t n_thr, uint32_t thr_bytes) {
  return (uint64_t)kAggWorkgroups * (((uint64_t)n_thr * thr_bytes + 15) & ~15ull) + 8192ull;
}
int aggregate_blocks(int64_t n_rows);
int aggregate_blocks(int64_t n_rows, int max_wg);
uint64_t aggregate_slab_pods(int64_t n_rows, int blocks);
struct AggTwoLaunch {
  bool enabled;
  bool small_window;
  bool overflow_pods;
  int pod_LA;
};
bool aggregate_two_per_cu_fits(const IndexDev& ix, const PackPlan& pk, const AggTwoLaunch& launch);
const char* launch_aggregate_indexed(const PodTable& pods, const AggScan& scan, const SelProgram& sp, const SelProgram* sp_dev,
                              const IndexDev& ix, unsigned long long* partial, void* slab, hipStream_t s,
                              const std::function<void()>& after_scan = nullptr);
struct ThrTables;
struct ReconcileOut;
struct ReqBound;
void launch_reduce_finalize_packed(const ThrTables& tt, const SelProgram& sp, int D, const IndexDev& ix, const PackPlan& pk, const void* slab,
                                   int n_slabs, const uint32_t* slab_tag, uint32_t epoch, unsigned long long* partial, bool consume, int64_t now_s,
                                   int32_t now_ns, bool apply, const ReconcileOut& out, void* recs, int rec_DT, bool rec_eq, const ReqBound& vmax,
                                   hipStream_t s, const uint8_t* row_mask, bool scan_adds_rows);
constexpr int64_t kCheckSmallMax = 256;
struct CheckSmall {
  uint32_t* ticket;
  uint64_t* host_summary;
  uint32_t n_inline;
  int64_t inline_rows[8];
};
struct CheckByNs {
  const uint64_t* v_meta;
  const uint16_t* v_latom;
  uint64_t* carry;
  const unsigned char* wv_img = nullptr;
  uint32_t wv_total_words = 0;
  const uint32_t* wg_range = nullptr;
  int wg_range_G = 0;
};
bool match_cache_fits(const IndexDev& ix);
bool check_replays_match_cache(const PodTable& pods, const SelProgram& sp, const IndexDev& ix, uint32_t planes, bool overflow_pods, bool one_per_cu);
bool launch_build_match_cache(const PodTable& pods, int64_t n, const int64_t* rows_dev, const IndexDev& ix, uint64_t* mw, uint64_t stride,
                              uint32_t planes, hipStream_t s, const MatchViewPlanes* view = nullptr);
void launch_gather_match_planes(const uint64_t* mw, uint64_t stride, uint32_t planes, const int64_t* rows, int64_t n, uint64_t* mx,
                                uint64_t mx_stride, hipStream_t s);
int check_sweep_blocks(int64_t n);
size_t verdict_images_bytes(uint32_t total_words, int D);
void launch_build_verdict_images(const IndexDev& ix, uint32_t total_words, const void* recs, int T, int D, void* out, hipStream_t s);
const char* launch_check_indexed(const PodTable& pods, int64_t n, const int64_t* rows_dev, const SelProgram& sp,
                          const SelProgram* sp_dev, const IndexDev& ix, const void* recs, uint64_t* summary,
                          uint8_t* status, hipStream_t s, const CheckSmall* small = nullptr, bool overflow_pods = false,
                          const CheckByNs* by_ns = nullptr, bool one_per_cu = false, const MatchCacheArgs* mc = nullptr);
const char* launch_sweep_indexed(const PodTable& pods, int64_t n, const SelProgram& sp, const SelProgram* sp_dev, const IndexDev& ix,
                                 const void* recs, uint64_t* summary, const PackPlan& pk, void* slab, uint32_t* slab_tag, uint32_t epoch,
                                 int* launched_blocks, hipStream_t s);
bool launch_check_few(const PodTable& pods, int n, const int64_t* rows_host, const SelProgram& sp, const IndexDev& ix, const void* recs,
                      unsigned long long* acc, uint32_t* ticket, uint64_t* host_summary, uint64_t* host_seq, uint64_t seq, hipStream_t s);
void launch_translate_pods(const PodTable& pods, int64_t n, const int64_t* rows_dev, int64_t row0, const IndexDev& ix,
                           unsigned long long* n_overflow, hipStream_t s);

}
```

kube_throttler_amd/csrc/kt_kernels_aggregate.hip:

```cpp
#include <cstdio>
#include <type_traits>

#include "kt_scan.h"

namespace kt {

__host__ __device__ inline uint32_t agg_tab_bytes(uint32_t n_thr, int D, bool counts) { return n_thr * agg_rec_bytes(D, counts); }

template <int DT, bool PK>
constexpr int pk_words() { return PK ? (DT > 8 ? 8 : 4) : 1; }
template <int DT, int LA, bool PK>
struct TileRecAgg {
  uint32_t p;
  uint64_t meta;
  u32x4 raw[LA / 8];
  int64_t v[PK ? 1 : DT];
  unsigned long long pw[pk_words<DT, PK>()];
};

struct BmAggArgs {
  const uint64_t* meta;
  const uint16_t* latom;
  const int64_t* req;
  const uint32_t* lpair;
// ... 321 lines not shown
                  x = andn_64(x, v - seg.x);
                }
                if (__ballot(x != 0ull && qn >= (uint32_t)kWq) != 0ull) flush();
                if (x != 0ull) {
#pragma unroll
                  for (int k = kWq - 1; k > 0; --k) qx[k] = qx[k - 1];
                  qx[0] = x;
                  qw = (qw_t)(qw << 10) | (qw_t)w;
                  qn += 1u;
                }
                return 0ull;
              },
              [&](uint32_t w) -> u64x2 { return seg_on ? segp[w] : u64x2{0ull, 0ull}; });
          flush();
        } else if constexpr (PK) {
          scan_tile<LA, VETO, NEED, VETO>(
              bm, scan_counted, ns, ro, [&](bool, uint32_t) {}, confirm_slow,
              [&](uint32_t w, uint64_t x, int) -> uint64_t {
                uint64_t xf = x;
                while (__ballot(xf != 0ull) != 0ull) {
                  const bool h1 = xf != 0ull;
                  const uint32_t c1 = h1 ? w * 64u + (uint32_t)__ffsll((unsigned long long)xf) - 1u : 0u;
                  xf &= xf - 1ull;
                  const bool h2 = xf != 0ull;
                  const uint32_t c2 = h2 ? w * 64u + (uint32_t)__ffsll((unsigned long long)xf) - 1u : 0u;
                  xf &= xf - 1ull;
                  const uint32_t tr1 = trank[c1], tr2 = trank[c2];
                  add_match(h1, tr1);
                  add_match(h2, tr2);
                }
                return 0ull;
              });
        } else {
          scan_tile<LA, VETO, NEED, VETO>(
              bm, scan_counted, ns, ro, [&](bool has, uint32_t c) { add_match(has, trank[c]); }, confirm_slow);
        }
      }
      __syncthreads();
      u32x4* dst = (u32x4*)(a.slab + (size_t)ch.slab_off * 16 + (size_t)blockIdx.x * slab_pitch + (size_t)r0 * rec);
      lds_u4p src = (lds_u4p)(lds + a.off_tab);
      for (uint32_t i = threadIdx.x; i < tab_bytes / 16; i += kBlockIx) dst[i] = src[i];
    }
    if (threadIdx.x == 0) a.slab_tag[ci * kSlabTagStride + blockIdx.x] = a.epoch;
  }
}

struct BmAggOneArgs {
  const uint64_t* v_meta;
  const uint16_t* v_latom;
  const uint64_t* v_pk;
  const uint64_t* v_mx;
  uint64_t mx_stride;
  uint32_t mx_planes;
  unsigned char* slab;
  BmIndexArgs ix;
  BmChunk ch;
  uint32_t n_rows, tpb;
  uint32_t off_rank, off_tab, off_seg;
  uint32_t tab_bytes;
  uint32_t pk_nw, pk_stride, pk_rec, skew;
};
__device__ __forceinline__ uint32_t agg_one_rec_off(uint32_t r, uint32_t rec, uint32_t skew) { return __umul24(r, rec) + (skew ? (r >> 3) << 3 : 0u); }

template <bool VETO, int NEED, bool CACHED = false>
__global__ __launch_bounds__(kBlockIx, 8) void kt_aggregate_bitmap_one(const BmAggOneArgs a) {
  static_assert(!CACHED || (!VETO && NEED == 2), "the cached form is one instantiation: nothing of the scan's form is left in it");
  constexpr int LA = 8, NW = 3, kWq = VETO ? 3 : 4;
  KT_LDS unsigned char* lds = (KT_LDS unsigned char*)kt_smem;
  const uint32_t lane = threadIdx.x & (kWave - 1);
  const uint32_t wave = __builtin_amdgcn_readfirstlane(threadIdx.x / kWave);
  const uint32_t n_rows = a.n_rows;
  const uint32_t n_wtiles = (n_rows + kWave - 1u) / kWave;
  const uint32_t t_lo = min(blockIdx.x * a.tpb, n_wtiles), t_hi = min(t_lo + a.tpb, n_wtiles);
  const BmChunk& ch = a.ch;
  const uint32_t rec = a.pk_rec, skew = a.skew, pk_nw = a.pk_nw;
  KT_LDS const uint16_t* trank = (KT_LDS const uint16_t*)(lds + a.off_rank);
  KT_LDS unsigned char* tab = lds + a.off_tab;
  struct Rec {
    uint64_t meta;
    u32x4 raw;
    uint64_t mx[kMatchReplay];
    unsigned long long pw[NW];
  };
  auto fetch_tile = [&](uint32_t wt) {
    Rec r{};
    const uint32_t ic = min(wt * kWave + lane, n_rows - 1u);
    r.meta = a.v_meta[ic];
    if constexpr (CACHED) {
      const uint64_t* q = a.v_mx + ic;
#pragma unroll
      for (int j = 0; j < kMatchReplay; ++j)
        if ((uint32_t)j < a.mx_planes) r.mx[j] = q[(uint64_t)j * a.mx_stride];
    } else {
      r.raw = *(const u32x4*)(a.v_latom + (uint64_t)ic * LA);
    }
    const u64x2* q = (const u64x2*)(a.v_pk + (uint64_t)ic * a.pk_stride);
    const u64x2 q0 = q[0];
    r.pw[0] = q0.x, r.pw[1] = q0.y, r.pw[2] = 0ull;
    if (a.pk_stride > 2u) r.pw[2] = q[1].x;
    return r;
  };
  for (uint32_t i = threadIdx.x; i < a.tab_bytes / 4; i += kBlockIx) ((lds_u32wp)tab)[i] = 0u;
  {
    const StageSeg img = CACHED ? StageSeg{a.ix.lds_img + ch.off_nsl_rng, (const u32x4*)(a.ix.blob + ch.img_off + ch.off_nsl_rng),
                                           (ch.lds_bytes - ch.off_nsl_rng) / 16u}
                                : chunk_image_segment(a.ix, ch);
    const StageSeg segs[2] = {img, StageSeg{a.off_rank, (const u32x4*)(a.ix.blob + ch.img_off + ch.off_term_rank), ch.n_words * 8u}};
    lds_stage_segments<2, 4>(lds, segs);
  }
  if (ch.has_adj) {
    const uint16_t* g_rank = (const uint16_t*)(a.ix.blob + ch.img_off + ch.off_term_rank);
    for (uint32_t w = wave; w < ch.n_words; w += (uint32_t)(kBlockIx / kWave)) {
      const uint32_t tr = g_rank[w * 64u + lane];
      const uint32_t tp = (uint32_t)__shfl_up((int)tr, 1), tn = (uint32_t)__shfl_down((int)tr, 1);
      const bool adj = (tr & kRankAdj) != 0u;
      const bool same_prev = lane > 0u && adj && tp == tr, same_next = lane < 63u && adj && tn == tr;
      const uint64_t m_lo = __ballot(!same_prev), m_hi = __ballot(!same_next);
      if (lane < 2u) ((lds_u64wp)(lds + a.off_seg))[w * 2u + lane] = lane == 0u ? m_lo : m_hi;
    }
  }
  const BmView bm = open_chunk<VETO>(lds, a.ix, ch);
  __syncthreads();
  const bool seg_on = ch.has_adj != 0u;
  KT_LDS const u64x2* segp = (KT_LDS const u64x2*)(lds + a.off_seg);
  for (uint32_t wt = t_lo + wave; wt < t_hi; wt += (uint32_t)(kBlockIx / kWave)) {
    const Rec cur = fetch_tile(wt);
    const bool in = wt * kWave + lane < n_rows;
    const uint64_t meta = cur.meta;
    const uint32_t st = (uint32_t)(meta >> kMetaStateShift) & 0xFu;
    const bool counted = in && (st & (kPodValid | kPodSchedMatch | kPodScheduled | kPodFinished)) == (kPodValid | kPodSchedMatch | kPodScheduled);
    if (__ballot(counted) == 0ull) continue;
    const uint32_t ns = counted ? (uint32_t)(meta & kMetaNsMask) : 0u;
    const uint32_t present = (uint32_t)(meta >> kMetaPresentShift) & 0xFFFFu;
    const uint32_t zero_keys = present & ~(uint32_t)(meta >> kMetaNzShift) & 0xFFFFu;
    unsigned long long pw[NW];
#pragma unroll
    for (int k = 0; k < NW; ++k) pw[k] = cur.pw[k];
    uint64_t qx[kWq];
    typedef typename std::conditional<(kWq > 3), uint64_t, uint32_t>::type qw_t;
    qw_t qw = 0;
    uint32_t qn = 0u;
#pragma unroll
    for (int k = 0; k < kWq; ++k) qx[k] = 0ull;
    auto flush = [&]() {
      while (__ballot(qn != 0u) != 0ull) {
        const bool has = qn != 0u;
        const uint32_t cw = ((uint32_t)qw & 1023u) * 64u;
        const uint32_t c = cw + (uint32_t)__ffsll((unsigned long long)qx[0]) - 1u;
        qx[0] &= qx[0] - 1ull;
        const uint32_t r = trank[has ? c : 0u] & 0x7FFFu;
        if (has && qx[0] == 0ull) {
#pragma unroll
          for (int k = 0; k + 1 < kWq; ++k) qx[k] = qx[k + 1];
          qx[kWq - 1] = 0ull;
          qw >>= 10;
          qn -= 1u;
        }
        if (has) {
          KT_LDS unsigned char* rp = tab + agg_one_rec_off(r, rec, skew);
          lds_u64wp tv = (lds_u64wp)rp;
          lds_add64(tv, pw[0]);
          if (pk_nw > 1u) lds_add64(tv + 1, pw[1]);
          if (pk_nw > 2u) lds_add64(tv + 2, pw[2]);
          if (zero_keys) (void)__hip_atomic_fetch_or((lds_u32wp)(rp + pk_nw * 8u), zero_keys, __ATOMIC_RELAXED, __HIP_MEMORY_SCOPE_WORKGROUP);
        }
      }
    };
    auto push_word = [&](uint32_t w, uint64_t x, const u64x2& seg) -> uint64_t {
      if (seg_on) {
        const uint64_t v = x | seg.y;
        x = andn_64(x, v - seg.x);
      }
      if (__ballot(x != 0ull && qn >= (uint32_t)kWq) != 0ull) flush();
      if (x != 0ull) {
#pragma unroll
        for (int k = kWq - 1; k > 0; --k) qx[k] = qx[k - 1];
        qx[0] = x;
        qw = (qw_t)(qw << 10) | (qw_t)w;
        qn += 1u;
      }
      return 0ull;
    };
    auto run_masks = [&](uint32_t w) -> u64x2 { return seg_on ? segp[w] : u64x2{0ull, 0ull}; };
    if constexpr (CACHED) {
      replay_tile(bm, counted, ns, cur.mx, a.mx_planes, [&](bool, uint32_t) {}, push_word, run_masks);
    } else {
      const u32x4 raw[1] = {cur.raw};
      uint32_t ro[LA];
      atom_row_offsets<LA>(raw, ro);
      scan_tile<LA, VETO, NEED, false>(bm, counted, ns, ro, [&](bool, uint32_t) {}, [&](uint32_t) { return true; }, push_word, run_masks);
    }
    flush();
  }
  __syncthreads();
  const uint32_t slab_pitch = (ch.n_thr * rec + 15u) & ~15u;
  u32x4* dst = (u32x4*)(a.slab + (size_t)blockIdx.x * slab_pitch);
  for (uint32_t i = threadIdx.x; i < slab_pitch / 16u; i += kBlockIx) {
    KT_LDS const u32x2* src = (KT_LDS const u32x2*)(tab + i * 16u + (skew ? (i >> 4) << 3 : 0u));
    const u32x2 lo = src[0], hi = src[1];
    dst[i] = u32x4{lo.x, lo.y, hi.x, hi.y};
  }
}

static BmAggOneArgs make_bm_agg_one_args(const IndexDev& ix, const PackPlan& pk, uint32_t* total) {
  BmAggOneArgs a{};
  uint32_t o = 0;
  auto take = [&](uint32_t bytes) { uint32_t r = o; o += (bytes + 15u) & ~15u; return r; };
  a.pk_nw = pk.nw, a.pk_stride = pk.stride, a.pk_rec = pk.rec_bytes, a.skew = pk.rec_bytes == 32u ? 1u : 0u;
  a.off_rank = take(ix.bm_max_words * 64u * 2u);
  a.tab_bytes = (ix.bm_max_thr * pk.rec_bytes + (a.skew ? ((ix.bm_max_thr + 7u) >> 3) * 8u : 0u) + 15u) & ~15u;
  a.off_tab = take(a.tab_bytes);
  a.off_seg = take(ix.bm_max_words * 16u);
  plan_bitmap_index(ix, a.ix, take);
  *total = o;
  return a;
}

bool aggregate_two_per_cu_fits(const IndexDev& ix, const PackPlan& pk, const AggTwoLaunch& launch) {
  if (!launch.enabled || launch.small_window || launch.overflow_pods || launch.pod_LA > 8) return false;
  if (ix.n_chunks != 1 || ix.h_chunks.size() != 1 || ix.n_slow != 0 || ix.has_long || ix.la > 8u || ix.max_need > 3u) return false;
  if (!pk.nw || pk.nw > 3u || pk.rec_bytes > 32u || pk.headroom < (uint32_t)kPackHeadroomBitsTwo) return false;
  const BmChunk& ch = ix.h_chunks[0];
  if (ch.has_slow || ch.n_thr == 0u) return false;
  uint32_t total = 0;
  (void)make_bm_agg_one_args(ix, pk, &total);
  if (2u * total > (uint32_t)kMaxLds) return false;
  const uint64_t pitch = ((uint64_t)ch.n_thr * pk.rec_bytes + 15u) & ~15ull;
  return (uint64_t)kAggWorkgroupsTwo * pitch <= agg_slab_area_bytes(ch.n_thr, ix.cut_thr_bytes);
}

constexpr int kSlabSplits = 4;
__global__ __launch_bounds__(256) void kt_reduce_bitmap_slabs(const unsigned char* slab, const BmChunk* chunks,
                                                              const uint32_t* rank_t, int n_slabs, int D, int counts, int sign,
                                                              const uint32_t* slab_tag, uint32_t epoch, unsigned long long* partial) {
  constexpr int G = 4;
  __shared__ unsigned long long part[G][64][4];
  const BmChunk ch = chunks[blockIdx.y];
  const uint32_t rec = agg_rec_bytes(D, counts != 0), ppr = rec / 16u;
  const uint32_t n_pieces = ch.n_thr * ppr;
  if (blockIdx.x * 64u >= n_pieces) return;
  const size_t pitch = (size_t)ch.n_thr * rec;
  const uint32_t wl = threadIdx.x & 63u, g = threadIdx.x >> 6;
  const uint32_t pi = blockIdx.x * 64u + wl;
  const bool in = pi < n_pieces;
  const uint32_t r = in ? pi / ppr : 0u, q = in ? pi - r * ppr : 0u;
// ... 108 lines not shown
int aggregate_blocks(int64_t n_rows) { return aggregate_blocks(n_rows, kAggWorkgroups); }
uint64_t aggregate_slab_pods(int64_t n_rows, int blocks) {
  const int64_t tiles = (n_rows + kWave - 1) / kWave;
  const int64_t per_wg = (tiles + blocks - 1) / blocks + (kBlockIx / kWave);
  return (uint64_t)per_wg * kWave;
}

const char* launch_aggregate_indexed(const PodTable& pods, const AggScan& sc, const SelProgram& sp, const SelProgram* sp_dev,
                              const IndexDev& ix, unsigned long long* partial, void* slab_, hipStream_t s,
                              const std::function<void()>& after_scan) {
  const int64_t n_rows = sc.n;
  if (n_rows <= 0 || sp.T <= 0) return "";
  const int DT = dt_bucket_ix(pods.D), LA = pods.LA;
  unsigned char* slab = (unsigned char*)slab_;
  uint32_t bm_total = 0;
  BmAggArgs bm_args = make_bm_agg_args(pods, sc, sp, sp_dev, ix, partial, slab, &bm_total);
  if (bm_total > (uint32_t)kMaxLds) return nullptr;
  const bool packed = bm_args.v_pk != nullptr && bm_args.ix.by_ns && !sc.counts && sc.sign == 1 && sc.nonneg &&
                      bm_args.pk.rec_bytes <= ix.cut_thr_bytes && !ix.has_long;
  if (bm_args.v_pk != nullptr && !packed) return nullptr;
  if (!packed && agg_rec_bytes(pods.D, sc.counts) > ix.cut_thr_bytes) return nullptr;
  const bool two_per_cu = packed && aggregate_two_per_cu_fits(ix, bm_args.pk, AggTwoLaunch{!sc.one_per_cu, sc.small_window, sc.overflow_pods, LA});
  if (packed && bm_args.pk.headroom >= (uint32_t)kPackHeadroomBitsTwo && !two_per_cu) {
    sc.refused = "the packed words were planned for two workgroups per CU and this launch cannot run that form";
    return nullptr;
  }
  int nb = aggregate_blocks(n_rows, two_per_cu ? kAggWorkgroupsTwo : kAggWorkgroups);
  if (two_per_cu) bm_args.wg_range = nullptr;
  if (bm_args.ix.by_ns && bm_args.wg_range) {
    if (ix.n_chunks == 1) bm_args.wg_range = nullptr;
  }
  if (bm_args.ix.by_ns && !bm_args.wg_range) {
    const int64_t tiles = (n_rows + kWave - 1) / kWave, tpb = (tiles + nb - 1) / nb;
    nb = (int)((tiles + tpb - 1) / tpb);
  }
  {
    const uint32_t rec_bytes = packed ? bm_args.pk.rec_bytes : agg_rec_bytes(pods.D, sc.counts);
    for (const BmChunk& ch : ix.h_chunks)
      if ((uint64_t)nb * (((uint64_t)ch.n_thr * rec_bytes + 15u) & ~15ull) > agg_slab_area_bytes(ch.n_thr, ix.cut_thr_bytes)) {
        sc.refused = "the slabs of the launch's workgroups do not fit the chunk's slab area";
        return nullptr;
      }
  }
  dim3 g_(nb), b_(kBlockIx);
  const size_t lds_bm = bm_total;
  if (two_per_cu) {
    uint32_t one_total = 0;
    BmAggOneArgs oa = make_bm_agg_one_args(ix, bm_args.pk, &one_total);
    const BmChunk& ch = ix.h_chunks[0];
    oa.v_meta = sc.v_meta, oa.v_latom = sc.v_latom, oa.v_pk = sc.v_pk, oa.ch = ch;
    const bool cached = sc.v_mx != nullptr && sc.limb == 0 && sc.mx_planes >= 1u && sc.mx_planes <= (uint32_t)kMatchReplay &&
                        (uint64_t)n_rows <= sc.mx_stride && match_cache_fits(ix);
    if (cached) oa.v_mx = sc.v_mx, oa.mx_stride = sc.mx_stride, oa.mx_planes = sc.mx_planes;
    oa.slab = slab + (size_t)ch.slab_off * 16;
    oa.n_rows = (uint32_t)n_rows;
    oa.tpb = (uint32_t)((((n_rows + kWave - 1) / kWave) + nb - 1) / nb);
    static const bool dbg_one = getenv("KT_DEBUG_LDS") != nullptr;
    if (dbg_one)
      fprintf(stderr, "kt_aggregate_bitmap_one: lds=%u (2 per CU) workgroups=%d tiles per workgroup=%u nw=%u rec=%u skew=%u cached=%d\n", one_total, nb,
              oa.tpb, oa.pk_nw, oa.pk_rec, oa.skew, cached ? 1 : 0);
#define KT_AGG_ONE_LAUNCH(VETO_, NEED_, ...)                                                                     \
  {                                                                                                             \
    auto kfn = kt_aggregate_bitmap_one<VETO_, NEED_, ##__VA_ARGS__>;                                            \
    (void)hipFuncSetAttribute((const void*)kfn, hipFuncAttributeMaxDynamicSharedMemorySize, (int)one_total);    \
    hipLaunchKernelGGL(kfn, g_, b_, one_total, s, oa);                                                          \
  }
    if (cached) {
      KT_AGG_ONE_LAUNCH(false, 2, true)
      sc.replayed = true;
    } else {
#ifdef KT_FAST_BUILD
      KT_AGG_ONE_LAUNCH(false, 2)
#else
      if (!ix.rich) KT_AGG_ONE_LAUNCH(false, 2) else KT_AGG_ONE_LAUNCH(true, 3)
#endif
    }
#undef KT_AGG_ONE_LAUNCH
  } else {
  const bool windowed = bm_args.win_recs != 0u;
  const bool wide_pk = packed && bm_args.pk.nw > 4u;
  static const bool dbg_lds = getenv("KT_DEBUG_LDS") != nullptr;
  if (dbg_lds)
    fprintf(stderr, "kt_aggregate_bitmap: lds=%u chunks=%u largest LDS part=%u max thr=%u T=%d packed=%d nw=%u rec=%u\n", bm_total, ix.n_chunks,
            ix.bm_max_lds, ix.bm_max_thr, sp.T, packed ? 1 : 0, bm_args.pk.nw, bm_args.pk.rec_bytes);
#ifdef KT_FAST_BUILD
  KT_AGG_BM_CASE(8, 8, false, 2)
#else
  if (!ix.rich) { if (DT <= 8) KT_AGG_BM_CASE(8, 8, false, 2) else KT_AGG_BM_CASE(16, 8, false, 2) }
  else if (ix.max_need > 3u) {
    if (LA <= 8) { if (DT <= 8) KT_AGG_BM_CASE(8, 8, true, 5) else KT_AGG_BM_CASE(16, 8, true, 5) }
    else if (LA <= 16) { if (DT <= 8) KT_AGG_BM_CASE(8, 16, true, 5) else KT_AGG_BM_CASE(16, 16, true, 5) }
    else { if (DT <= 8) KT_AGG_BM_CASE(8, 32, true, 5) else KT_AGG_BM_CASE(16, 32, true, 5) }
  }
  else if (LA <= 8) { if (DT <= 8) KT_AGG_BM_CASE(8, 8, true, 3) else KT_AGG_BM_CASE(16, 8, true, 3) }
  else if (LA <= 16) { if (DT <= 8) KT_AGG_BM_CASE(8, 16, true, 3) else KT_AGG_BM_CASE(16, 16, true, 3) }
  else { if (DT <= 8) KT_AGG_BM_CASE(8, 32, true, 3) else KT_AGG_BM_CASE(16, 32, true, 3) }
#endif
  }
  if (after_scan) after_scan();
  sc.launched_blocks = nb, sc.launched_packed = packed;
  if (packed && sc.defer_reduce) {
  } else if (packed) {
    const uint32_t rb_ = (uint32_t)(nb > 16 * kRecWaves ? kRecTileUnits / 2 : kRecTileUnits) / (bm_args.pk.rec_bytes >> 3);
    if (ix.bm_max_thr > 0 && nb > 16 * kRecWaves)
      hipLaunchKernelGGL(kt_reduce_packed_slabs<32>, dim3((ix.bm_max_thr + rb_ - 1u) / rb_, ix.n_chunks), dim3(kRecBlock), 0, s, slab,
                         ix.bm_chunks, ix.bm_rank_t, nb, pods.D, bm_args.pk, sc.slab_tag, sc.epoch, ix.n_chunks > 1 ? 1 : 0, partial);
    else if (ix.bm_max_thr > 0)
      hipLaunchKernelGGL(kt_reduce_packed_slabs<16>, dim3((ix.bm_max_thr + rb_ - 1u) / rb_, ix.n_chunks), dim3(kRecBlock), 0, s, slab,
                         ix.bm_chunks, ix.bm_rank_t, nb, pods.D, bm_args.pk, sc.slab_tag, sc.epoch, ix.n_chunks > 1 ? 1 : 0, partial);
  } else {
    const uint32_t max_pieces = ix.bm_max_thr * (agg_rec_bytes(pods.D, sc.counts) / 16u);
    if (max_pieces > 0)
      hipLaunchKernelGGL(kt_reduce_bitmap_slabs, dim3((max_pieces + 63) / 64, ix.n_chunks, kSlabSplits), dim3(256), 0, s, slab,
                         ix.bm_chunks, ix.bm_rank_t, nb, pods.D, sc.counts ? 1 : 0, sc.sign, sc.slab_tag, sc.epoch, partial);
  }
  return packed ? (ix.n_chunks == 1 ? "kt_aggregate_bitmap_packed" : "kt_aggregate_bitmap_packed_chunked")
                : (ix.n_chunks == 1 ? "kt_aggregate_bitmap" : "kt_aggregate_bitmap_chunked");
}

}
// ... 1 lines not shown
```

kube_throttler_amd/csrc/kt_kernels_check.hip:

```cpp
#include <cassert>
#include <type_traits>

#include "kt_scan.h"

#ifdef KT_PROFILE_PHASES
__device__ unsigned long long kt_prof_check[16];
extern "C" int kt_debug_prof_check(unsigned long long* out16, int reset) {
  if (hipMemcpyFromSymbol(out16, HIP_SYMBOL(kt_prof_check), 16 * 8) != hipSuccess) return -1;
  if (reset) { unsigned long long z[16] = {0}; (void)hipMemcpyToSymbol(HIP_SYMBOL(kt_prof_check), z, 16 * 8); }
  return 0;
}
#define KT_PROF_T(var) const unsigned long long var = __builtin_amdgcn_s_memtime()
#define KT_PROF_ADD(slot, dt) prof_acc[slot] += (dt)
#else
#define KT_PROF_T(var)
#define KT_PROF_ADD(slot, dt)
#endif

namespace kt {


constexpr uint32_t kListCap = 128;
template <int DT>
struct alignas(16) WordVerdict {
// ... 521 lines not shown
            const unsigned long long w = __hip_atomic_load((unsigned long long*)a.summary + i, __ATOMIC_RELAXED, __HIP_MEMORY_SCOPE_AGENT);
            const unsigned long long c = w & ~3ull;
            const unsigned long long fin = !on ? 0ull : (w & 2ull) ? 2ull : (c | (c ? 1ull : 0ull));
            a.summary[i] = fin;
            if (a.host_summary) a.host_summary[i] = fin;
            if (FULL && a.status && on && (w & 2ull))
              for (int t = 0; t < a.T; ++t) a.status[(uint64_t)i * (uint32_t)a.T + t] = 255;
          }
          if (lane == 0) a.ticket[wt] = 0u;
        }
      } else if (in) {
        const unsigned long long c = my + cnt[lane];
        if (last) {
          a.summary[si] = !on ? 0ull : pod_err ? 2ull : (c | (c ? 1ull : 0ull));
          if (FULL && a.status && pod_err)
            for (int t = 0; t < a.T; ++t) a.status[(uint64_t)si * (uint32_t)a.T + t] = 255;
        } else {
          *carry_w = c | (pod_err ? 2ull : 0ull);
        }
      }
#ifdef KT_PROFILE_PHASES
      __builtin_amdgcn_s_waitcnt(0);
      KT_PROF_T(t_d1);
      KT_PROF_ADD(5, t_d1 - t_s1);
#endif
    }
    if constexpr (AGG) {
      __syncthreads();
      const uint32_t tab_bytes = (ch.n_thr * a.pk_rec + 15u) & ~15u;
      u32x4* dst = (u32x4*)(a.slab + (size_t)ch.slab_off * 16 + (size_t)blockIdx.x * tab_bytes);
      lds_u4p src = (lds_u4p)(lds + a.off_tab);
      for (uint32_t i = threadIdx.x; i < tab_bytes / 16; i += kBlockIx) dst[i] = src[i];
      if (threadIdx.x == 0) a.slab_tag[ci * kSlabTagStride + blockIdx.x] = a.epoch;
    }
  }
#ifdef KT_PROFILE_PHASES
  if (!SMALL && lane == 0) {
    KT_PROF_T(t_kernel1);
    for (int k = 0; k < 8; ++k) atomicAdd(&kt_prof_check[k], prof_acc[k]);
    atomicAdd(&kt_prof_check[8], t_kernel1 - t_kernel0);
    atomicAdd(&kt_prof_check[9], 1ull);
  }
#endif
}

struct BmCheckCachedArgs {
  const uint64_t* meta;
  const int64_t* req;
  const void* recs;
  uint64_t* summary;
  const uint8_t* ns_valid;
  const uint64_t* mw;
  uint64_t mw_stride;
  const unsigned char* blob;
  BmChunk ch;
  uint32_t n;
  int32_t DS, T;
  uint32_t lds_img, off_cnt, off_list, off_tinfo, off_wv;
};
static_assert(kTermRowMask == (1u << 20) - 1u && kWave == 64, "a list entry is lane << 20 | term number");

static BmCheckCachedArgs make_check_cached_args(const IndexDev& ix, uint32_t* total) {
  BmCheckCachedArgs a{};
  uint32_t o = 0;
  auto take = [&](uint32_t bytes) { uint32_t r = o; o += (bytes + 15u) & ~15u; return r; };
  a.off_cnt = take(kBlockIx * 8u);
  a.off_list = take((kBlockIx / kWave) * kListCap * 4);
  a.off_tinfo = take(ix.bm_max_words * 64u * 8u);
  a.off_wv = take(ix.bm_max_words * (uint32_t)sizeof(WordVerdict<8>));
  a.lds_img = take(ix.bm_max_lds);
  *total = o;
  return a;
}

template <int PL>
__global__ __launch_bounds__(kBlockIx, 8) void kt_check_bitmap_cached(const BmCheckCachedArgs a) {
  static_assert(PL >= 1 && PL <= kMatchReplay, "one instantiation per plane count");
  constexpr int DT = 8;
  KT_LDS unsigned char* lds = (KT_LDS unsigned char*)kt_smem;
  const CheckRec<DT>* recs = (const CheckRec<DT>*)a.recs;
  const u32x2* g_rflags = (const u32x2*)rec_flags<DT>((void*)a.recs, a.T);
  const uint32_t n = a.n;
  const int DS = a.DS;
  const uint32_t lane = threadIdx.x & (kWave - 1);
  const uint32_t wave = __builtin_amdgcn_readfirstlane(threadIdx.x / kWave);
  lds_u64wp cnt = (lds_u64wp)(lds + a.off_cnt) + wave * kWave;
  lds_u32wp list = (lds_u32wp)(lds + a.off_list) + wave * kListCap;
  KT_LDS u32x2* tinfo = (KT_LDS u32x2*)(lds + a.off_tinfo);
  KT_LDS const unsigned char* wv = lds + a.off_wv;
  const BmChunk& ch = a.ch;
  const uint32_t n_wtiles = (n + kWave - 1) / kWave;
  const uint32_t wstep = gridDim.x * (kBlockIx / kWave);
  BmIndexArgs ixa{};
  ixa.blob = a.blob, ixa.lds_img = a.lds_img;
  const BmView bm = open_chunk<false>(lds, ixa, ch);
  {
    const uint32_t* term_t = (const uint32_t*)(a.blob + ch.img_off + ch.off_term_t);
    uint32_t tt_first = 0u;
    if (threadIdx.x < ch.n_words * 64u) tt_first = term_t[threadIdx.x];
    const StageSeg segs[1] = {StageSeg{a.lds_img + ch.off_nsl_rng, (const u32x4*)(a.blob + ch.img_off + ch.off_nsl_rng), (ch.lds_bytes - ch.off_nsl_rng) / 16u}};
    lds_stage_segments<1>(lds, segs);
    for (uint32_t c = threadIdx.x; c < ch.n_words * 64u; c += kBlockIx)
      build_term_verdicts<DT, true>(c == threadIdx.x ? tt_first : term_t[c], c, g_rflags, tinfo, (KT_LDS WordVerdict<DT>*)(lds + a.off_wv));
  }
  __syncthreads();
  const bool seg_on = ch.has_adj != 0u;

  struct Rec {
    uint64_t meta;
    uint64_t mx[kMatchReplay];
  };
  auto fetch_tile = [&](uint32_t wt) {
    Rec r{};
    const uint32_t ic = min(wt * kWave + lane, n - 1u);
    r.meta = ld_issued(a.meta + ic);
    const uint64_t* q = a.mw + ic;
#pragma unroll
    for (int j = 0; j < PL; ++j) r.mx[j] = ld_issued(q + (uint64_t)j * a.mw_stride);
    return r;
  };
  for (uint32_t wt = blockIdx.x * (kBlockIx / kWave) + wave; wt < n_wtiles; wt += wstep) {
    const Rec r = fetch_tile(wt);
    cnt[lane] = 0ull;
    uint32_t n_list = 0;

    auto drain = [&](auto unroll_tag) {
      constexpr int UNROLL = decltype(unroll_tag)::value;
      for (uint32_t base = 0; base < n_list; base += kWave) {
        const uint32_t j = base + lane;
        const bool vv = j < n_list;
        const uint32_t e = list[vv ? j : 0u];
        const uint32_t pl = e >> 20;
        const u32x2 ti = tinfo[e & kTermRowMask];
        const uint32_t t = ti.x & kTermRowMask;
        const uint32_t prow = min(wt * kWave + pl, n - 1u);
        static_assert(kMetaNzShift == 48, "the non-zero mask is the meta word's top 16 bits");
        const uint32_t pnz = ((const uint16_t*)(a.meta + prow))[3];
        const CheckRec<DT>* rc = recs + t;
        const kt_i64x2* xr = (const kt_i64x2*)(a.req + (uint64_t)prow * (uint32_t)DS);
        const uint32_t sh_act = (ti.y >> kTiShActive) & 63u, sh_idle = (ti.y >> kTiShIdle) & 63u;
        const uint32_t fx = (sh_act == 4u ? kRecExceedsByCount : 0u) | (sh_idle == 24u ? kRecActiveByCount : 0u) | (sh_idle == 44u ? kRecInsufficientByCount : 0u);
        const uint32_t fy = ti.y & 0xFFFFu;
        bool exc = false, ins = false;
        if constexpr (UNROLL == 0) {
#pragma unroll 1
          for (int d = 0; d < DT; ++d) {
            const int64_t x = a.req[(uint64_t)prow * (uint32_t)DS + (uint32_t)(d < DS ? d : 0)], th = rc->thr[d], hd = rc->head[d];
            const bool nzd = (pnz >> d) & 1u;
            exc |= nzd && x > th, ins |= nzd && x > hd;
          }
        } else {
#pragma unroll 1
        for (int q0 = 0; q0 < DT / 2; q0 += UNROLL) {
          kt_i64x2 x[UNROLL], th[UNROLL], hd[UNROLL];
#pragma unroll
          for (int u = 0; u < UNROLL; ++u) {
            const int q = q0 + u;
            x[u] = xr[2 * q < DS ? q : 0];
            th[u] = *(const kt_i64x2*)(rc->thr + 2 * q);
            hd[u] = *(const kt_i64x2*)(rc->head + 2 * q);
          }
#pragma unroll
          for (int u = 0; u < UNROLL; ++u) {
            const int q = q0 + u;
            const bool nz0 = (pnz >> (2 * q)) & 1u, nz1 = (pnz >> (2 * q + 1)) & 1u;
            exc |= (nz0 && x[u].x > th[u].x) || (nz1 && x[u].y > th[u].y);
            ins |= (nz0 && x[u].x > hd[u].x) || (nz1 && x[u].y > hd[u].y);
          }
        }
        }
        exc |= (fx & kRecExceedsByCount) != 0, ins |= (fx & kRecInsufficientByCount) != 0;
        const bool act = (fx & kRecActiveByCount) || (pnz & fy);
        const uint32_t st = exc ? 4u : act ? 2u : ins ? 3u : 1u;
        if (vv && st != 1u) lds_add64(cnt + pl, st == 4u ? 1ull << 4 : st == 2u ? 1ull << 24 : 1ull << 44);
      }
      n_list = 0;
    };
    auto push = [&](bool want, uint32_t e) {
      const uint64_t mk = __ballot(want);
      if (mk == 0ull) return;
      if (want) list[n_list + lane_rank(mk)] = e;
      n_list += (uint32_t)__popcll(mk);
      if (n_list > kListCap - kWave) drain(std::integral_constant<int, 0>());
    };
    {
      const uint64_t meta = r.meta;
      const bool on = wt * kWave + lane < n && ((meta >> kMetaStateShift) & kPodValid) != 0;
      const uint32_t ns = on ? (uint32_t)(meta & kMetaNsMask) : 0u;
      const uint32_t nz = (uint32_t)(meta >> kMetaNzShift) & 0xFFFFu;
      const uint32_t ns_ok_raw = a.ns_valid[ns];
      auto nib_offset = [&](int q) { return (uint32_t)offsetof(WordVerdict<DT>, act_nib) + (uint32_t)q * 128u + ((nz >> (4 * q)) & 15u) * 8u; };
      uint32_t n_exc = 0u, n_act = 0u, n_ins = 0u;
      auto settle_word = [&](uint32_t w, uint64_t x, int) -> uint64_t {
        KT_LDS const unsigned char* q = wv + __umul24(w, (uint32_t)sizeof(WordVerdict<DT>));
        if (seg_on) {
          const u64x2 seg = *(KT_LDS const u64x2*)(q + offsetof(WordVerdict<DT>, seg_lo));
          const uint64_t v = x | seg.y;
          x = andn_64(x, v - seg.x);
        }
        const u64x2 te = *(KT_LDS const u64x2*)(q + offsetof(WordVerdict<DT>, tight));
        const u64x2 ai = *(KT_LDS const u64x2*)(q + offsetof(WordVerdict<DT>, act));
        uint64_t act = *(KT_LDS const unsigned long long*)(q + nib_offset(0));
#pragma unroll
        for (int k = 1; k < DT / 4; ++k) act |= *(KT_LDS const unsigned long long*)(q + nib_offset(k));
        const uint64_t xe = and_not_and_64(x, te.x, te.y);
        const uint64_t xf = and_not_not_64(x, te.x, te.y);
        const uint64_t xa = xf & act, xi = and_not_and_64(xf, act, ai.y);
        n_exc = (uint32_t)__popc((uint32_t)xe) + ((uint32_t)__popc((uint32_t)(xe >> 32)) + n_exc);
        n_act = (uint32_t)__popc((uint32_t)xa) + ((uint32_t)__popc((uint32_t)(xa >> 32)) + n_act);
        n_ins = (uint32_t)__popc((uint32_t)xi) + ((uint32_t)__popc((uint32_t)(xi >> 32)) + n_ins);
        return x & te.x;
      };
      replay_tile(bm, on, ns, r.mx, (uint32_t)PL, [&](bool has, uint32_t c) { push(has, lane << 20 | c); }, settle_word, ScanNoPrefetch());
      const unsigned long long my = (unsigned long long)n_exc << 4 | (unsigned long long)n_act << 24 | (unsigned long long)n_ins << 44;
      cnt[lane] += my | (on ? 1ull : 0ull) | ((on && ns_ok_raw == 0u) ? 2ull : 0ull);
    }
    if (n_list) drain(std::integral_constant<int, 2>());
    if (wt * kWave + lane < n) {
      const unsigned long long w = cnt[lane], c = w & ~3ull;
      a.summary[wt * kWave + lane] = !(w & 1ull) ? 0ull : (w & 2ull) ? 2ull : (c | (c ? 1ull : 0ull));
    }
  }
}

static void launch_check_cached(const PodTable& pods, int64_t n, const SelProgram& sp, const IndexDev& ix, const void* recs, uint64_t* summary,
                                const MatchCacheArgs& mc, dim3 grid, hipStream_t s) {
  uint32_t total = 0;
  BmCheckCachedArgs a = make_check_cached_args(ix, &total);
  assert(2u * total <= (uint32_t)kMaxLds && (uint64_t)ix.bm_max_words * 64u <= (uint64_t)kTermRowMask + 1u);
  a.meta = pods.meta, a.req = pods.req, a.recs = recs, a.summary = summary, a.ns_valid = sp.ns_valid;
  a.mw = mc.mw, a.mw_stride = mc.stride;
  a.blob = ix.bm_blob, a.ch = ix.h_chunks[0];
  a.n = (uint32_t)n, a.DS = pods.DS, a.T = sp.T;
  static const bool dbg_lds = getenv("KT_DEBUG_LDS") != nullptr;
  if (dbg_lds) fprintf(stderr, "kt_check_bitmap_cached: lds=%u (2 per CU) workgroups=%u planes=%u\n", total, grid.x, mc.planes);
#define KT_CHECK_CACHED_LAUNCH(PL_)                                                                             \
  {                                                                                                             \
    auto kfn = kt_check_bitmap_cached<PL_>;                                                                     \
    (void)hipFuncSetAttribute((const void*)kfn, hipFuncAttributeMaxDynamicSharedMemorySize, (int)total);        \
    hipLaunchKernelGGL(kfn, grid, dim3(kBlockIx), total, s, a);                                                 \
  }
  static_assert(kMatchReplay == 4, "one instantiation per plane count");
#ifdef KT_FAST_BUILD
  KT_CHECK_CACHED_LAUNCH(kMatchReplay)
#else
  switch (mc.planes) {
    case 1: KT_CHECK_CACHED_LAUNCH(1) break;
    case 2: KT_CHECK_CACHED_LAUNCH(2) break;
    case 3: KT_CHECK_CACHED_LAUNCH(3) break;
    default: KT_CHECK_CACHED_LAUNCH(4) break;
  }
#endif
#undef KT_CHECK_CACHED_LAUNCH
}

#define KT_BM_LAUNCH(DT_, LA_, VETO_, NEED_, WPE_, FULL_, SMALL_, ONE_)                                         \
  {                                                                                                             \
    auto kfn = kt_check_bitmap<DT_, LA_, VETO_, NEED_, WPE_, FULL_, SMALL_, ONE_>;                              \
    (void)hipFuncSetAttribute((const void*)kfn, hipFuncAttributeMaxDynamicSharedMemorySize, (int)lds_bytes);    \
    hipLaunchKernelGGL(kfn, g_, b_, lds_bytes, s, bm_args);                                                     \
  }
#define KT_BM_CASE(DT_, LA_, VETO_, NEED_)                                                   \
  {                                                                                          \
    if (small) KT_BM_LAUNCH(DT_, LA_, VETO_, NEED_, 4, true, true, false)                    \
    else if (full) KT_BM_LAUNCH(DT_, LA_, VETO_, NEED_, 4, true, false, false)               \
    else if (cached) launch_check_cached(pods, n, sp, ix, recs, summary, *mc, g_, s); \
    else if (two_per_cu) KT_BM_LAUNCH(DT_, LA_, VETO_, NEED_, 8, false, false, true)         \
    else KT_BM_LAUNCH(DT_, LA_, VETO_, NEED_, 4, false, false, false)                        \
  }

#define KT_BM_CASE5(DT_, LA_)                                                           \
  {                                                                                     \
    if (small) KT_BM_LAUNCH(DT_, LA_, true, 5, 4, true, true, false)                    \
    else if (full) KT_BM_LAUNCH(DT_, LA_, true, 5, 4, true, false, false)               \
    else KT_BM_LAUNCH(DT_, LA_, true, 5, 4, false, false, false)                        \
  }

const char* launch_check_indexed(const PodTable& pods, int64_t n, const int64_t* rows_dev, const SelProgram& sp,
                          const SelProgram* sp_dev, const IndexDev& ix, const void* recs, uint64_t* summary,
                          uint8_t* status, hipStream_t s, const CheckSmall* sm, bool overflow_pods, const CheckByNs* by_ns, bool one_per_cu,
                          const MatchCacheArgs* mc) {
  if (n <= 0) return "";
  const int DT = dt_bucket_ix(pods.D), LA = pods.LA;
  if (status) (void)hipMemsetAsync(status, 0, (size_t)n * (size_t)sp.T, s);
  uint32_t bm_total = 0;
  BmCheckArgs bm_args = make_bm_check_args(pods, n, rows_dev, sp, sp_dev, ix, recs, summary, status, &bm_total);
  if (bm_total > (uint32_t)kMaxLds) return nullptr;
  const size_t lds_bytes = bm_total;
  const bool small = sm != nullptr && n <= kCheckSmallMax;
  if (small) {
    (void)hipMemsetAsync(summary, 0, (size_t)n * 8, s);
    bm_args.ticket = sm->ticket, bm_args.host_summary = sm->host_summary;
    bm_args.n_inline = sm->n_inline;
    for (int k = 0; k < 8; ++k) bm_args.inline_rows[k] = sm->inline_rows[k];
  }
  bm_args.has_overflow = overflow_pods ? 1u : 0u;
  if (by_ns && !small && rows_dev) {
    bm_args.ix.by_ns = 1u;
    bm_args.v_meta = by_ns->v_meta, bm_args.v_latom = by_ns->v_latom, bm_args.carry = by_ns->carry;
    bm_args.wv_img = by_ns->wv_img, bm_args.wv_total_words = by_ns->wv_total_words;
    bm_args.wg_range = by_ns->wg_range_G == check_sweep_blocks(n) ? by_ns->wg_range : nullptr;
  }
  const bool full = status != nullptr || ix.n_slow != 0 || overflow_pods || ix.has_long;
  const bool need5 = ix.max_need > 3u;
  const bool one = ix.n_chunks == 1 && bm_args.ix.by_ns == 0u;
  const bool two_per_cu = one && !full && !small && !need5 && !one_per_cu && LA <= 8 && 2 * bm_total <= (uint32_t)kMaxLds;
// ... 70 lines not shown
```

kube_throttler_amd/csrc/kt_kernels_match.hip:

```cpp
#include "kt_scan.h"

namespace kt {

struct MatchBuildArgs {
  const uint64_t* meta;
  const uint16_t* latom;
  const int64_t* rows;
  uint64_t* mw;
  uint64_t stride;
  uint32_t planes;
  uint32_t n;
  uint32_t cap;
  uint64_t* vx;
  const int32_t* vpos;
  uint64_t vstride;
  BmIndexArgs ix;
  BmChunk ch;
};

template <bool VETO, int NEED>
__global__ __launch_bounds__(kBlockIx) void kt_build_match_cache(const MatchBuildArgs a) {
  constexpr int LA = 8;
  KT_LDS unsigned char* lds = (KT_LDS unsigned char*)kt_smem;
  const uint32_t lane = threadIdx.x & (kWave - 1);
  const uint32_t wave = __builtin_amdgcn_readfirstlane(threadIdx.x / kWave);
  const BmChunk& ch = a.ch;
  {
    const StageSeg segs[1] = {chunk_image_segment(a.ix, ch)};
    lds_stage_segments<1, 4>(lds, segs);
  }
  const BmView bm = open_chunk<VETO>(lds, a.ix, ch);
  __syncthreads();
  const uint32_t n = a.n, planes = a.planes;
  const uint32_t n_wtiles = (n + kWave - 1u) / kWave;
  const uint32_t wstep = gridDim.x * (uint32_t)(kBlockIx / kWave);
  for (uint32_t wt = blockIdx.x * (uint32_t)(kBlockIx / kWave) + wave; wt < n_wtiles; wt += wstep) {
    const uint32_t i = wt * kWave + lane;
    const uint32_t ic = min(i, n - 1u);
    const uint32_t p = a.rows ? (uint32_t)a.rows[ic] : ic;
    const bool in = i < n && p < a.cap;
    const uint32_t pc = min(p, a.cap - 1u);
    const uint64_t meta = a.meta[pc];
    const int32_t vj = a.vx ? a.vpos[pc] : -1;
    u32x4 raw[1];
    load_atoms<LA>(a.latom, (int64_t)pc, raw);
    const bool on = in && ((meta >> kMetaStateShift) & kPodValid) != 0;
    const uint32_t ns = on ? (uint32_t)(meta & kMetaNsMask) : 0u;
    uint32_t ro[LA];
    atom_row_offsets<LA>(raw, ro);
    uint64_t* q = a.mw + pc;
    const bool thru = in && vj >= 0 && (uint64_t)vj < a.vstride;
    uint64_t* qv = a.vx + (thru ? (uint32_t)vj : 0u);
    uint32_t round = 0u;
    scan_tile<LA, VETO, NEED, false>(
        bm, on, ns, ro, [&](bool, uint32_t) {}, [&](uint32_t) { return true; },
        [&](uint32_t, uint64_t xx, int) -> uint64_t {
          if (in && round < planes) q[(uint64_t)round * a.stride] = xx;
          if (thru && round < planes) qv[(uint64_t)round * a.vstride] = xx;
          round += 1u;
          return 0ull;
        });
    for (; round < planes; ++round) {
      if (in) q[(uint64_t)round * a.stride] = 0ull;
      if (thru) qv[(uint64_t)round * a.vstride] = 0ull;
    }
  }
}

__global__ __launch_bounds__(256) void kt_gather_match_planes(const uint64_t* mw, uint64_t stride, uint32_t planes, const int64_t* rows, int64_t n,
                                                             uint64_t* mx, uint64_t mx_stride) {
  for (int64_t j = (int64_t)blockIdx.x * 256 + threadIdx.x; j < n; j += (int64_t)gridDim.x * 256) {
    const uint64_t p = (uint64_t)rows[j];
    if (p >= stride) continue;
    uint64_t x[kMatchReplay];
#pragma unroll
    for (int k = 0; k < kMatchReplay; ++k) x[k] = (uint32_t)k < planes ? mw[(uint64_t)k * stride + p] : 0ull;
#pragma unroll
    for (int k = 0; k < kMatchReplay; ++k)
      if ((uint32_t)k < planes) mx[(uint64_t)k * mx_stride + (uint64_t)j] = x[k];
  }
}
void launch_gather_match_planes(const uint64_t* mw, uint64_t stride, uint32_t planes, const int64_t* rows, int64_t n, uint64_t* mx,
                                uint64_t mx_stride, hipStream_t s) {
  if (n <= 0 || !mw || !mx || planes == 0u || planes > (uint32_t)kMatchReplay || (uint64_t)n > mx_stride) return;
  const int64_t nb = std::min<int64_t>((n + 255) / 256, 4096);
  hipLaunchKernelGGL(kt_gather_match_planes, dim3((unsigned)nb), dim3(256), 0, s, mw, stride, planes, rows, n, mx, mx_stride);
}

bool match_cache_fits(const IndexDev& ix) {
  if (ix.n_chunks != 1 || ix.h_chunks.size() != 1 || ix.n_slow != 0 || ix.has_long || ix.la > 8u || ix.max_need > 3u) return false;
  const BmChunk& ch = ix.h_chunks[0];
  return !ch.has_slow && ch.n_words != 0u && ix.bm_max_lds <= (uint32_t)kMaxLds;
}

bool launch_build_match_cache(const PodTable& pods, int64_t n, const int64_t* rows_dev, const IndexDev& ix, uint64_t* mw, uint64_t stride,
                              uint32_t planes, hipStream_t s, const MatchViewPlanes* view) {
  if (n <= 0) return true;
  if (!match_cache_fits(ix) || pods.LA > 8 || !mw || planes == 0u || planes > (uint32_t)kMatchPlanes || stride == 0u || n > (int64_t)stride)
    return false;
  MatchBuildArgs a{};
  a.meta = pods.meta, a.latom = pods.latom, a.rows = rows_dev, a.mw = mw, a.stride = stride, a.planes = planes;
  a.n = (uint32_t)n, a.cap = (uint32_t)std::min<uint64_t>(stride, 0x80000000ull);
  if (view && view->mx && view->pos && view->stride) a.vx = view->mx, a.vpos = view->pos, a.vstride = view->stride;
  uint32_t o = 0;
  auto take = [&](uint32_t bytes) { uint32_t r = o; o += (bytes + 15u) & ~15u; return r; };
  plan_bitmap_index(ix, a.ix, take);
  a.ch = ix.h_chunks[0];
  const uint32_t lds_bytes = o;
  const int64_t tiles = (n + kWave - 1) / kWave, per_wg = kBlockIx / kWave;
  const int64_t nb = std::min<int64_t>((tiles + per_wg - 1) / per_wg, 2 * kCUs);
  dim3 g_((unsigned)nb), b_(kBlockIx);
#define KT_MATCH_LAUNCH(VETO_, NEED_)                                                                           \
  {                                                                                                             \
    auto kfn = kt_build_match_cache<VETO_, NEED_>;                                                              \
    (void)hipFuncSetAttribute((const void*)kfn, hipFuncAttributeMaxDynamicSharedMemorySize, (int)lds_bytes);    \
    hipLaunchKernelGGL(kfn, g_, b_, lds_bytes, s, a);                                                           \
  }
#ifdef KT_FAST_BUILD
  KT_MATCH_LAUNCH(false, 2)
#else
  if (!ix.rich) KT_MATCH_LAUNCH(false, 2) else KT_MATCH_LAUNCH(true, 3)
#endif
#undef KT_MATCH_LAUNCH
  return true;
}

}
```

kube_throttler_amd/engine.py:

```python
from __future__ import annotations

import ctypes as C
import os
import subprocess

import numpy as np

from . import snapshot as S

_HERE = os.path.dirname(os.path.abspath(__file__))
_CSRC = os.path.join(_HERE, "csrc")
LIB_PATH = os.path.join(_CSRC, "libkt_engine.so")
if os.environ.get("KT_ENGINE_LIB"):
    LIB_PATH = os.path.abspath(os.environ["KT_ENGINE_LIB"])
_LIB = None

KT_OK = 0
ERR_NAMES = {-1: "KT_ERR_INVALID_ARGUMENT", -2: "KT_ERR_OUT_OF_RANGE", -3: "KT_ERR_DEVICE", -4: "KT_ERR_OVERFLOW_RISK",
             -5: "KT_ERR_NOT_READY", -6: "KT_ERR_NO_DEVICE", -7: "KT_ERR_UNSUPPORTED"}
RECONCILE_APPLY = 0x1
ADMIT_COMMIT = 0x1
VARIANT_INCREMENTAL = 0x100
CHECK_STATUS_MATRIX = 0x1
KERNEL_CHECK, KERNEL_AGGREGATE, KERNEL_FINALIZE, KERNEL_PREPARE, KERNEL_REDUCE = 0, 1, 2, 3, 4
VARIANT_INDEXED, VARIANT_DENSE = 0, 1

EXPORTS = [
    "kt_version", "kt_engine_create", "kt_engine_destroy", "kt_last_error", "kt_upsert_namespaces", "kt_upsert_pods",
    "kt_upsert_throttles", "kt_delete_namespaces", "kt_delete_pods", "kt_delete_throttles", "kt_load_snapshot",
    "kt_set_reserved", "kt_set_status", "kt_reconcile_launch", "kt_aggregate_launch", "kt_partial_used_buffer",
    "kt_use_partial_buffer", "kt_finalize_launch", "kt_reconcile_fetch", "kt_check_launch", "kt_check_fetch", "kt_throttle_rows", "kt_sweep_launch",
    "kt_check_device_summary", "kt_fetch_pod_requests", "kt_timing_enable", "kt_timing_read", "kt_timing_reset",
    "kt_synchronize", "kt_kernel_name", "kt_admit_launch", "kt_fetch_reserved", "kt_reconcile_fetch_next_override",
    "kt_check", "kt_upsert_namespace", "kt_upsert_pod", "kt_upsert_throttle", "kt_comm_unique_id", "kt_comm_init",
    "kt_comm_allreduce_partial", "kt_comm_destroy", "kt_reconcile_rows_launch", "kt_set_exchange_world", "kt_counter", "kt_reconcile_fetch_used_hi",
    "kt_set_wide_sums", "kt_partial_words", "kt_partial_layout", "kt_debug_reload_env", "kt_affected_pods", "kt_paged_check", "kt_paged_reconcile",
    "kt_paged_admit", "kt_admit_gangs_launch", "kt_admit_gangs_fetch", "kt_paged_admit_gangs",
    "kt_headroom_launch", "kt_headroom_fetch", "kt_paged_headroom", "kt_preempt_launch", "kt_preempt_fetch",
    "kt_preempt_reprieve_launch", "kt_preempt_gangs_launch", "kt_preempt_gangs_reprieve_launch", "kt_preempt_gangs_fetch", "kt_forecast_launch", "kt_forecast_fetch", "kt_forecast_gangs_launch", "kt_forecast_gangs_fetch", "kt_override_instants",
    "kt_paged_preempt", "kt_paged_forecast", "kt_debug_match_planes", "kt_paged_preempt_gangs",
]
HEADROOM_MAX_CAP = 0x7FFFFFFF
PREEMPT_NONE = -1
PREEMPT_REPRIEVE = 0x1
FORECAST_NONE = -1
COUNTER_FEW_CHECKS, COUNTER_COMPILES, COUNTER_INDEX_CHUNKS, COUNTER_INDEX_WORDS, COUNTER_NS_WORD_VISITS, COUNTER_NS_ROWS = range(6)
COUNTER_NS_CHUNK_VISITS, COUNTER_INDEX_IMAGE_WORDS, COUNTER_SLOW_THROTTLES, COUNTER_PACKED_WORDS = 6, 7, 8, 9
COUNTER_AGG_WORKGROUPS = 11
COUNTER_VIEW_BUILDS = 10
COUNTER_MATCH_CACHE_BUILDS, COUNTER_MATCH_CACHE_SCANS, COUNTER_MATCH_CACHE_PLANES = 12, 13, 14
COUNTER_MATCH_CACHE_AGG_SCANS = 15


def partial_layout(n_dims: int) -> dict:
    v = [C.c_int32() for _ in range(5)]
    rc = lib().kt_partial_layout(int(n_dims), *[C.byref(x) for x in v])
    if rc != KT_OK:
        raise EngineError(rc, f"kt_partial_layout({n_dims})")
    return dict(zip(("stride", "values", "presence", "pods", "errors"), (int(x.value) for x in v)))


def version() -> str:
    return lib().kt_version().decode()


def paged_check(engines, n, rows=None, on_equal=False):
    hs = (C.c_void_p * len(engines))(*[e._h for e in engines])
    T = engines[0].throttle_rows()
    rows_a = None if rows is None else np.ascontiguousarray(rows, dtype=np.int64)
    if rows_a is None:
        rows_a = np.arange(n, dtype=np.int64)
    status = np.zeros((max(n, 1), max(T, 1)), np.uint8)
    summary = np.zeros(max(n, 1), np.uint64)
    rc = lib().kt_paged_check(hs, len(engines), n, rows_a.ctypes.data, int(on_equal), summary.ctypes.data, status.ctypes.data)
    if rc != KT_OK:
        raise EngineError(rc, "kt_paged_check: " + "; ".join(lib().kt_last_error(e._h).decode() for e in engines))
    return status[:n, :T], summary[:n]


def paged_admit(engines, rows, on_equal=False, commit=False):
    hs = (C.c_void_p * len(engines))(*[e._h for e in engines])
    T = engines[0].throttle_rows()
    rows_a = np.ascontiguousarray(rows, dtype=np.int64)
    n = len(rows_a)
    status = np.zeros((max(n, 1), max(T, 1)), np.uint8)
    summary = np.zeros(max(n, 1), np.uint64)
    rc = lib().kt_paged_admit(hs, len(engines), n, rows_a.ctypes.data if n else None, int(on_equal),
                              ADMIT_COMMIT if commit else 0, summary.ctypes.data, status.ctypes.data)
    if rc != KT_OK:
        raise EngineError(rc, "kt_paged_admit: " + "; ".join(lib().kt_last_error(e._h).decode() for e in engines))
    return status[:n, :T], summary[:n]


# ... 114 lines not shown


def build(force: bool = False) -> str:
    args = ["make", "-C", _CSRC, "-j8"]
    if force:
        args.append("-B")
    subprocess.check_call(args, stdout=subprocess.DEVNULL)
    return LIB_PATH


def lib():
    global _LIB
    if _LIB is None:
        if not os.path.exists(LIB_PATH):
            raise EngineError(-6, f"{LIB_PATH} is missing: build it with kube_throttler_amd.engine.build() "
                                  "(there is no CPU fallback)")
        L = C.CDLL(LIB_PATH)
        L.kt_version.restype = C.c_char_p
        L.kt_last_error.restype = C.c_char_p
        L.kt_last_error.argtypes = [C.c_void_p]
        L.kt_kernel_name.restype = C.c_char_p
        L.kt_kernel_name.argtypes = [C.c_void_p, C.c_int32]
        L.kt_engine_create.argtypes = [C.POINTER(KtConfig), C.POINTER(C.c_void_p)]
        L.kt_engine_destroy.argtypes = [C.c_void_p]
        for name in ("kt_upsert_namespaces", "kt_upsert_pods", "kt_upsert_throttles"):
            getattr(L, name).argtypes = [C.c_void_p, C.POINTER(S.KtSnapshot), C.c_void_p]
        L.kt_delete_namespaces.argtypes = [C.c_void_p, C.c_int32, C.c_void_p]
        L.kt_delete_pods.argtypes = [C.c_void_p, C.c_int64, C.c_void_p]
        L.kt_delete_throttles.argtypes = [C.c_void_p, C.c_int32, C.c_void_p]
        L.kt_load_snapshot.argtypes = [C.c_void_p, C.POINTER(S.KtSnapshot)]
        L.kt_set_reserved.argtypes = [C.c_void_p, C.c_int32, C.c_void_p, C.POINTER(S.KtAmounts)]
        L.kt_set_status.argtypes = [C.c_void_p, C.c_int32, C.c_void_p, C.POINTER(KtStatus)]
        L.kt_reconcile_launch.argtypes = [C.c_void_p, C.c_int64, C.c_int32, C.c_uint32, C.c_void_p]
        L.kt_reconcile_rows_launch.argtypes = [C.c_void_p, C.c_int64, C.c_int32, C.c_uint32, C.c_int32, C.c_void_p, C.c_void_p]
        L.kt_aggregate_launch.argtypes = [C.c_void_p, C.c_void_p]
        L.kt_partial_used_buffer.argtypes = [C.c_void_p, C.POINTER(C.c_void_p), C.POINTER(C.c_int64)]
        L.kt_use_partial_buffer.argtypes = [C.c_void_p, C.c_void_p, C.c_int64]
        L.kt_finalize_launch.argtypes = [C.c_void_p, C.c_int64, C.c_int32, C.c_uint32, C.c_void_p]
        L.kt_reconcile_fetch.argtypes = [C.c_void_p, C.c_int32, C.POINTER(KtStatus)]
        L.kt_check_launch.argtypes = [C.c_void_p, C.c_int64, C.c_void_p, C.c_int32, C.c_uint32, C.c_void_p]
        L.kt_sweep_launch.argtypes = [C.c_void_p, C.c_int64, C.c_int32, C.c_uint32, C.c_int32, C.c_void_p]
        L.kt_check_fetch.argtypes = [C.c_void_p, C.c_int64, C.c_void_p, C.c_void_p]
        L.kt_check.argtypes = [C.c_void_p, C.c_int64, C.c_void_p, C.c_int32, C.c_void_p, C.c_void_p]
        L.kt_comm_unique_id.argtypes = [C.c_void_p]
        L.kt_comm_init.argtypes = [C.c_void_p, C.c_int32, C.c_int32, C.c_void_p]
        L.kt_comm_allreduce_partial.argtypes = [C.c_void_p, C.c_void_p]
        L.kt_comm_destroy.argtypes = [C.c_void_p]
        L.kt_set_exchange_world.argtypes = [C.c_void_p, C.c_int32]
        L.kt_set_wide_sums.argtypes = [C.c_void_p, C.c_int32]
        L.kt_partial_words.argtypes = [C.c_void_p, C.POINTER(C.c_int64), C.POINTER(C.c_int32)]
        L.kt_partial_layout.argtypes = [C.c_int32] + [C.POINTER(C.c_int32)] * 5
        L.kt_debug_reload_env.argtypes = [C.c_void_p]
        L.kt_debug_match_planes.argtypes = [C.c_void_p, C.c_int32, C.c_int64, C.c_void_p, C.c_void_p, C.POINTER(C.c_int64), C.POINTER(C.c_int32)]
        L.kt_affected_pods.argtypes = [C.c_void_p, C.c_int64, C.c_void_p, C.c_int32, C.c_void_p, C.c_void_p]
        L.kt_paged_check.argtypes = [C.POINTER(C.c_void_p), C.c_int32, C.c_int64, C.c_void_p, C.c_int32, C.c_void_p, C.c_void_p]
        L.kt_paged_reconcile.argtypes = [C.POINTER(C.c_void_p), C.c_int32, C.c_int64, C.c_int32, C.c_uint32, C.c_int32,
                                         C.POINTER(KtStatus), C.c_void_p, C.c_void_p]
        L.kt_paged_admit.argtypes = [C.POINTER(C.c_void_p), C.c_int32, C.c_int64, C.c_void_p, C.c_int32, C.c_uint32, C.c_void_p,
                                     C.c_void_p]
        L.kt_counter.argtypes = [C.c_void_p, C.c_int32]
        L.kt_reconcile_fetch_used_hi.argtypes = [C.c_void_p, C.c_int32, C.c_void_p, C.POINTER(C.c_int32)]
        L.kt_counter.restype = C.c_int64
        L.kt_throttle_rows.argtypes = [C.c_void_p, C.POINTER(C.c_int32)]
        L.kt_check_device_summary.argtypes = [C.c_void_p, C.POINTER(C.c_void_p)]
        L.kt_fetch_pod_requests.argtypes = [C.c_void_p, C.c_int64, C.c_void_p, C.c_void_p, C.c_void_p]
        L.kt_timing_enable.argtypes = [C.c_void_p, C.c_int32]
        L.kt_timing_read.argtypes = [C.c_void_p, C.c_int32, C.POINTER(C.c_double), C.POINTER(C.c_int64)]
        L.kt_timing_reset.argtypes = [C.c_void_p]
        L.kt_synchronize.argtypes = [C.c_void_p, C.c_void_p]
        L.kt_reconcile_fetch_next_override.argtypes = [C.c_void_p, C.c_int32, C.c_void_p, C.c_void_p, C.c_void_p]
        L.kt_admit_launch.argtypes = [C.c_void_p, C.c_int64, C.c_void_p, C.c_int32, C.c_uint32, C.c_void_p]
        L.kt_fetch_reserved.argtypes = [C.c_void_p, C.c_int32, C.c_void_p, C.POINTER(S.KtAmounts)]
        L.kt_admit_gangs_launch.argtypes = [C.c_void_p, C.c_int64, C.c_void_p, C.c_int64, C.c_void_p, C.c_int32, C.c_uint32, C.c_void_p]
        L.kt_admit_gangs_fetch.argtypes = [C.c_void_p, C.c_int64, C.c_void_p]
        L.kt_paged_admit_gangs.argtypes = [C.POINTER(C.c_void_p), C.c_int32, C.c_int64, C.c_void_p, C.c_int64, C.c_void_p, C.c_int32,
                                           C.c_uint32, C.c_void_p, C.c_void_p, C.c_void_p]
        L.kt_headroom_launch.argtypes = [C.c_void_p, C.c_int64, C.c_void_p, C.c_int32, C.c_int64, C.c_void_p]
        L.kt_headroom_fetch.argtypes = [C.c_void_p, C.c_int64, C.c_void_p, C.c_void_p]
        L.kt_paged_headroom.argtypes = [C.POINTER(C.c_void_p), C.c_int32, C.c_int64, C.c_void_p, C.c_int32, C.c_int64, C.c_void_p,
                                        C.c_void_p]
        L.kt_paged_preempt.argtypes = [C.POINTER(C.c_void_p), C.c_int32, C.c_int64, C.c_void_p, C.c_int64, C.c_void_p, C.c_int64, C.c_int32,
                                       C.c_int32, C.c_uint32, C.c_void_p, C.c_void_p]
        L.kt_paged_preempt_gangs.argtypes = [C.POINTER(C.c_void_p), C.c_int32, C.c_int64, C.c_void_p, C.c_int64, C.c_void_p, C.c_int64,
                                             C.c_void_p, C.c_int64, C.c_int32, C.c_int32, C.c_uint32, C.c_void_p, C.c_void_p, C.c_void_p]
        L.kt_preempt_launch.argtypes = [C.c_void_p, C.c_int64, C.c_void_p, C.c_int64, C.c_void_p, C.c_int64, C.c_int32, C.c_int32,
                                        C.c_void_p]
        L.kt_preempt_fetch.argtypes = [C.c_void_p, C.c_int64, C.c_void_p, C.c_void_p]
        L.kt_preempt_reprieve_launch.argtypes = L.kt_preempt_launch.argtypes
        L.kt_preempt_gangs_launch.argtypes = [C.c_void_p, C.c_int64, C.c_void_p, C.c_int64, C.c_void_p, C.c_int64, C.c_void_p, C.c_int64,
                                              C.c_int32, C.c_int32, C.c_void_p]
        L.kt_preempt_gangs_reprieve_launch.argtypes = L.kt_preempt_gangs_launch.argtypes
        L.kt_preempt_gangs_fetch.argtypes = [C.c_void_p, C.c_int64, C.c_void_p, C.c_void_p, C.c_void_p]
        L.kt_paged_forecast.argtypes = [C.POINTER(C.c_void_p), C.c_int32, C.c_int64, C.c_void_p, C.c_int64, C.c_void_p, C.c_void_p, C.c_int32,
                                        C.c_void_p, C.c_void_p]
        L.kt_forecast_launch.argtypes = [C.c_void_p, C.c_int64, C.c_void_p, C.c_int64, C.c_void_p, C.c_void_p, C.c_int32, C.c_void_p]
        L.kt_forecast_fetch.argtypes = [C.c_void_p, C.c_int64, C.c_void_p, C.c_void_p]
        L.kt_forecast_gangs_launch.argtypes = [C.c_void_p, C.c_int64, C.c_void_p, C.c_int64, C.c_void_p, C.c_int64, C.c_void_p, C.c_void_p,
                                               C.c_int32, C.c_void_p]
        L.kt_forecast_gangs_fetch.argtypes = [C.c_void_p, C.c_int64, C.c_void_p, C.c_void_p, C.c_void_p]
        L.kt_override_instants.argtypes = [C.c_void_p, C.c_int64, C.c_int32, C.c_int64, C.c_int32, C.c_int64, C.c_void_p, C.c_void_p,
                                           C.POINTER(C.c_int64)]
        _LIB = L
    return _LIB


class ReconcileResult:
# ... 124 lines not shown

    @staticmethod
    def comm_unique_id() -> bytes:
        buf = C.create_string_buffer(128)
        rc = lib().kt_comm_unique_id(buf)
        if rc != 0:
            raise EngineError(rc, lib().kt_last_error(None).decode())
        return buf.raw

    def comm_init(self, rank: int, world: int, unique_id: bytes):
        self._ck(lib().kt_comm_init(self._h, rank, world, C.create_string_buffer(unique_id, 128)))

    def comm_allreduce_partial(self, stream=None):
        self._ck(lib().kt_comm_allreduce_partial(self._h, stream))

    def comm_destroy(self):
        self._ck(lib().kt_comm_destroy(self._h))

    def reconcile_fetch_used_hi(self, n=None):
        n = self.throttle_rows() if n is None else n
        hi = np.zeros((max(n, 1), self.D), np.int64)
        anyw = C.c_int32()
        self._ck(lib().kt_reconcile_fetch_used_hi(self._h, n, hi.ctypes.data_as(C.c_void_p), C.byref(anyw)))
        return hi[:n], bool(anyw.value)

    def few_checks_served(self) -> int:
        return int(lib().kt_counter(self._h, 0))

    def compiles(self) -> int:
        return int(lib().kt_counter(self._h, 1))

    def set_exchange_world(self, world: int):
        self._ck(lib().kt_set_exchange_world(self._h, world))

    def affected_pods(self, pod_rows, throttle_rows):
        pr = np.ascontiguousarray(pod_rows, dtype=np.int64)
        tr = np.ascontiguousarray(throttle_rows, dtype=np.int32)
        out = np.zeros((max(len(pr), 1), max(len(tr), 1)), np.uint8)
        self._ck(lib().kt_affected_pods(self._h, len(pr), pr.ctypes.data, len(tr), tr.ctypes.data, out.ctypes.data))
        return out[:len(pr), :len(tr)]

    def reload_env(self):
        self._ck(lib().kt_debug_reload_env(self._h))

    def match_planes(self, view=False):
        n, planes = C.c_int64(), C.c_int32()
        self._ck(lib().kt_debug_match_planes(self._h, int(view), 0, None, None, C.byref(n), C.byref(planes)))
        cap = max(int(n.value), 1)
        out = np.zeros((int(planes.value), cap), dtype=np.uint64)
        rows = np.zeros(cap, dtype=np.int64)
        self._ck(lib().kt_debug_match_planes(self._h, int(view), cap, out.ctypes.data, rows.ctypes.data if view else None, C.byref(n), C.byref(planes)))
        return out[:, :int(n.value)], (rows[:int(n.value)] if view else None)

    def index_stats(self) -> dict:
        ch, words, visits, rows, cvis, iw, slow = (int(lib().kt_counter(self._h, k)) for k in (
            COUNTER_INDEX_CHUNKS, COUNTER_INDEX_WORDS, COUNTER_NS_WORD_VISITS, COUNTER_NS_ROWS, COUNTER_NS_CHUNK_VISITS, COUNTER_INDEX_IMAGE_WORDS,
            COUNTER_SLOW_THROTTLES))
        return {"chunks": ch, "words": words, "image_words": iw, "namespace_rows": rows,
                "word_visits_per_namespace": round(visits / rows, 3) if rows > 0 else None,
                "chunks_per_namespace": round(cvis / rows, 3) if rows > 0 else None, "slow_throttles": slow}

    def packed_words(self) -> int:
        return int(lib().kt_counter(self._h, COUNTER_PACKED_WORDS))

    def aggregate_workgroups(self) -> int:
        return int(lib().kt_counter(self._h, COUNTER_AGG_WORKGROUPS))

    def view_builds(self) -> int:
        return int(lib().kt_counter(self._h, COUNTER_VIEW_BUILDS))

    def match_cache_builds(self) -> int:
        return int(lib().kt_counter(self._h, COUNTER_MATCH_CACHE_BUILDS))

    def match_cache_planes(self) -> int:
        return int(lib().kt_counter(self._h, COUNTER_MATCH_CACHE_PLANES))

    def match_cache_scans(self) -> int:
        return int(lib().kt_counter(self._h, COUNTER_MATCH_CACHE_SCANS))

    def match_cache_agg_scans(self) -> int:
        return int(lib().kt_counter(self._h, COUNTER_MATCH_CACHE_AGG_SCANS))

    def partial_words(self) -> int:
        return self.throttle_rows() * partial_layout(self.D)["stride"]

    def set_wide_sums(self, mode: int):
        self._ck(lib().kt_set_wide_sums(self._h, mode))

    def pending_partial_words(self):
        n, w = C.c_int64(), C.c_int32()
        self._ck(lib().kt_partial_words(self._h, C.byref(n), C.byref(w)))
        return int(n.value), bool(w.value)

    def finalize_launch(self, now, apply=True, stream=None):
        self._ck(lib().kt_finalize_launch(self._h, int(now[0]), int(now[1]), RECONCILE_APPLY if apply else 0, stream))

    def throttle_rows(self) -> int:
        n = C.c_int32()
        self._ck(lib().kt_throttle_rows(self._h, C.byref(n)))
        return n.value

    def reconcile_fetch(self, n=None) -> ReconcileResult:
        n = self.throttle_rows() if n is None else n
        r = ReconcileResult(n, self.D)
        st = r.as_struct()
        self._ck(lib().kt_reconcile_fetch(self._h, n, C.byref(st)))
# ... 225 lines not shown
```

Baseline: 23740 billion decisions/s.

## Add compact per-pod match-code records to the match cache for check and aggregate

```diff
diff --git a/include/kt_engine.h b/include/kt_engine.h
--- a/include/kt_engine.h
+++ b/include/kt_engine.h
@@ -211,6 +211,9 @@
 
 int32_t kt_debug_match_planes(kt_engine* e, int32_t which, int64_t cap, uint64_t* out, int64_t* out_rows, int64_t* out_n, int32_t* out_planes);
 
+int32_t kt_debug_match_codes(kt_engine* e, int32_t which, int64_t cap, uint64_t* out, int64_t* out_rows, int64_t* out_n);
+int32_t kt_debug_match_runs(kt_engine* e, int32_t ns_row, int32_t k, int32_t* out_word, uint64_t* out_lo, uint64_t* out_hi);
+
 #ifdef __cplusplus
 }
 #endif
diff --git a/kube_throttler_amd/csrc/kt_engine.cpp b/kube_throttler_amd/csrc/kt_engine.cpp
--- a/kube_throttler_amd/csrc/kt_engine.cpp
+++ b/kube_throttler_amd/csrc/kt_engine.cpp
@@ -347,6 +347,7 @@
   e->views.release();
   e->d_carry.release();
   e->d_mc.release();
+  e->d_mcodes.release();
   if (e->h_mc_rows) (void)hipHostFree(e->h_mc_rows);
   if (e->mc_rows_ev) (void)hipEventDestroy(e->mc_rows_ev);
   e->d_slab_tag.release();
@@ -523,6 +524,54 @@
   return KT_OK;
 }
 
+int32_t kt_debug_match_codes(kt_engine* e, int32_t which, int64_t cap, uint64_t* out, int64_t* out_rows, int64_t* out_n) {
+  if (!e || which < 0 || which > 1 || cap < 0 || !out_n || (cap > 0 && !out)) return KT_ERR_INVALID_ARGUMENT;
+  LaunchLock lk(e);
+  KT_HIP(e, hipSetDevice(e->device));
+  if (e->last_stream) KT_HIP(e, hipStreamSynchronize(e->last_stream));
+  *out_n = 0;
+  const uint32_t planes = e->mc_planes;
+  if (!e->mc_valid || e->program_dirty || e->mc_gen != e->program_gen || e->mc_planes_gen != e->program_gen || !e->mc_pending.empty() || !e->d_mcodes.p ||
+      planes == 0u || planes > (uint32_t)kt::kMatchReplay || e->d_mcodes.cap < (size_t)e->cfg.pod_capacity)
+    return e->fail(KT_ERR_NOT_READY, "no current match-code records: no table built for this program, or rows wait for their refresh");
+  int64_t n = e->pod_rows_hi;
+  const kt::MatchCodes* src = e->d_mcodes.p;
+  hipStream_t s = e->own_stream;
+  const ScanView& cv = e->views.countable;
+  if (which == 1) {
+    if (!cv.valid || !cv.mx_valid || !cv.mc_there || !cv.mc.p || !cv.rows.p || !cv.d_n.p || cv.mx_planes != planes || cv.mc.cap < (size_t)cv.cap + 1)
+      return e->fail(KT_ERR_NOT_READY, "the countable scan view holds no current match-code records");
+    unsigned long long dn = 0;
+    KT_HIP(e, hipMemcpyAsync(&dn, cv.d_n.p, 8, hipMemcpyDeviceToHost, s));
+    KT_HIP(e, hipStreamSynchronize(s));
+    n = (int64_t)std::min<unsigned long long>(std::min<unsigned long long>(dn, cv.n + (unsigned long long)cv.extra), (unsigned long long)cv.cap);
+    src = cv.mc.p;
+  }
+  *out_n = n;
+  if (cap == 0 || n == 0) return KT_OK;
+  if (cap < n) return e->fail(KT_ERR_OUT_OF_RANGE, "cap=%lld < %lld", (long long)cap, (long long)n);
+  KT_HIP(e, hipMemcpyAsync(out, src, (size_t)n * sizeof(kt::MatchCodes), hipMemcpyDeviceToHost, s));
+  if (which == 1 && out_rows) KT_HIP(e, hipMemcpyAsync(out_rows, cv.rows.p, (size_t)n * 8, hipMemcpyDeviceToHost, s));
+  KT_HIP(e, hipStreamSynchronize(s));
+  return KT_OK;
+}
+
+int32_t kt_debug_match_runs(kt_engine* e, int32_t ns_row, int32_t k, int32_t* out_word, uint64_t* out_lo, uint64_t* out_hi) {
+  if (!e || ns_row < 0 || k < 0 || !out_word || !out_lo || !out_hi) return KT_ERR_INVALID_ARGUMENT;
+  LaunchLock lk(e);
+  const kt::HostIndex& h = e->hindex;
+  if (e->program_dirty || h.bm_chunks.size() != 1 || (uint32_t)ns_row >= h.n_ns) return e->fail(KT_ERR_NOT_READY, "no current single-chunk program with that namespace row");
+  const kt::BmChunk& ch = h.bm_chunks[0];
+  const uint32_t* rng = (const uint32_t*)(h.bm_images.data() + ch.img_off + ch.off_nsl_rng);
+  const kt::NsWord* nsl = (const kt::NsWord*)(h.bm_images.data() + ch.img_off + ch.off_nsl);
+  *out_word = -1, *out_lo = ~0ull, *out_hi = ~0ull;
+  if ((uint32_t)k >= rng[2 * ns_row + 1] - rng[2 * ns_row]) return KT_OK;
+  const uint32_t w = nsl[rng[2 * ns_row] + (uint32_t)k].w;
+  *out_word = (int32_t)w;
+  if (ch.has_adj && h.bm_runs.size() >= ((size_t)ch.w0 + w + 1) * 2) *out_lo = h.bm_runs[((size_t)ch.w0 + w) * 2], *out_hi = h.bm_runs[((size_t)ch.w0 + w) * 2 + 1];
+  return KT_OK;
+}
+
 int64_t kt_counter(kt_engine* e, int32_t which) {
   if (!e) return -1;
   switch (which) {
diff --git a/kube_throttler_amd/csrc/kt_engine_check.cpp b/kube_throttler_amd/csrc/kt_engine_check.cpp
--- a/kube_throttler_amd/csrc/kt_engine_check.cpp
+++ b/kube_throttler_amd/csrc/kt_engine_check.cpp
@@ -35,17 +35,20 @@
   const uint64_t stride = (uint64_t)e->cfg.pod_capacity;
   ScanView& cv = e->views.countable;
   kt::MatchViewPlanes vp;
-  if (cv.valid && cv.mx_valid && cv.mx.p && cv.pos.p && cv.mx_planes == planes && e->mc_gen == e->program_gen)
-    vp.mx = cv.mx.p, vp.pos = cv.pos.p, vp.stride = (uint64_t)cv.cap + 1u;
+  const bool recs = kt::match_codes_fit(e->dindex, planes);
+  if (cv.valid && cv.mx_valid && cv.mx.p && cv.pos.p && cv.mx_planes == planes && e->mc_gen == e->program_gen &&
+      (!recs || (cv.mc_there && cv.mc.cap >= (size_t)cv.cap + 1)))
+    vp.mx = cv.mx.p, vp.pos = cv.pos.p, vp.stride = (uint64_t)cv.cap + 1u, vp.mc = recs ? cv.mc.p : nullptr;
   else
     cv.mx_valid = false;
   if (!e->mc_valid || e->mc_gen != e->program_gen) {
-    if (e->d_mc.cap < (size_t)planes * stride) {
+    if (e->d_mc.cap < (size_t)planes * stride || (recs && e->d_mcodes.cap < (size_t)stride)) {
       if (e->last_stream) KT_HIP(e, hipStreamSynchronize(e->last_stream));
       KT_HIP(e, e->d_mc.reserve((size_t)planes * stride));
+      if (recs) KT_HIP(e, e->d_mcodes.reserve((size_t)stride));
     }
     order_behind_ingest(e, s);
-    if (!kt::launch_build_match_cache(e->pods, e->pod_rows_hi, nullptr, e->dindex, e->d_mc.p, stride, planes, s, &vp)) {
+    if (!kt::launch_build_match_cache(e->pods, e->pod_rows_hi, nullptr, e->dindex, e->d_mc.p, stride, planes, s, &vp, recs ? e->d_mcodes.p : nullptr)) {
       cv.mx_valid = false;
       return KT_OK;
     }
@@ -63,7 +66,7 @@
     }
     memcpy(e->h_mc_rows, e->mc_pending.data(), n * 8);
     order_behind_ingest(e, s);
-    if (!kt::launch_build_match_cache(e->pods, (int64_t)n, e->h_mc_rows, e->dindex, e->d_mc.p, stride, planes, s, &vp)) {
+    if (!kt::launch_build_match_cache(e->pods, (int64_t)n, e->h_mc_rows, e->dindex, e->d_mc.p, stride, planes, s, &vp, recs ? e->d_mcodes.p : nullptr)) {
       e->mc_valid = false, cv.mx_valid = false;
       e->mc_pending.clear();
       return KT_OK;
@@ -74,6 +77,7 @@
     e->mc_pending.clear();
   }
   mc.mw = e->d_mc.p, mc.stride = stride, mc.planes = planes;
+  if (recs && e->d_mcodes.p && e->d_mcodes.cap >= (size_t)stride) mc.codes = e->d_mcodes.p;
   return KT_OK;
 }
 
@@ -125,6 +129,7 @@
   if (e->cfg.kernel_variant != 1 && !pod_rows && !small && !want_status && n > 0 && n <= e->cfg.pod_capacity && e->dindex.n_chunks == 1 &&
       !e->sw[kSw_FORCE_NS_ORDER] && !e->sw[kSw_CHECK_ONE_PER_CU]) {
     if ((rc = match_cache_for_scan(e, s, mc)) != KT_OK) return rc;
+    if (e->sw[kSw_NO_MATCH_CODES]) mc.codes = nullptr;
   }
   {
     TimedLaunch tl(e, KT_KERNEL_CHECK, s);
diff --git a/kube_throttler_amd/csrc/kt_engine_impl.h b/kube_throttler_amd/csrc/kt_engine_impl.h
--- a/kube_throttler_amd/csrc/kt_engine_impl.h
+++ b/kube_throttler_amd/csrc/kt_engine_impl.h
@@ -126,6 +126,8 @@
   kt::PackPlan pack;
   DevBuf<int32_t> pos;
   DevBuf<uint64_t> mx;
+  DevBuf<kt::MatchCodes> mc;
+  bool mc_there = false;
   uint32_t mx_planes = 0;
   bool mx_valid = false;
   DevBuf<uint32_t> range;
@@ -134,7 +136,7 @@
   int64_t extra = 0;
   bool by_ns = false;
   bool valid = false;
-  void release() { rows.release(); d_n.release(); meta.release(); latom.release(); req.release(); pk.release(); pos.release(); range.release(); mx.release(); mx_valid = false; }
+  void release() { rows.release(); d_n.release(); meta.release(); latom.release(); req.release(); pk.release(); pos.release(); range.release(); mx.release(); mc.release(); mx_valid = false, mc_there = false; }
 };
 struct ViewSpec {
   bool countable_only;
@@ -191,8 +193,8 @@
 extern thread_local std::string g_create_error;
 
 
-enum EnvSwitch { kSw_FEED_NO_STAGE, kSw_FORCE_NS_ORDER, kSw_INGEST_EVENT_WAIT, kSw_NO_FEED_FEW, kSw_NO_FEED_FUSION, kSw_NO_FUSED, kSw_NO_NS_ORDER, kSw_NO_PACK, kSw_NO_SCAN_VIEW, kSw_NO_SWEEP, kSw_NO_VERDICT_IMAGES, kSw_NO_WG_RANGES, kSw_SYNC_INGEST, kSw_INGEST_TRUST_FENCE, kSw_NO_VIEW_PATCH, kSw_CHECK_ONE_PER_CU, kSw_AGG_SMALL_WINDOW, kSw_AGG_ONE_PER_CU, kSw_NO_MATCH_CACHE, kSw_NO_MATCH_CACHE_AGG, kSwCount };
-static const char* const kEnvSwitchName[kSwCount] = {"KT_FEED_NO_STAGE", "KT_FORCE_NS_ORDER", "KT_INGEST_EVENT_WAIT", "KT_NO_FEED_FEW", "KT_NO_FEED_FUSION", "KT_NO_FUSED", "KT_NO_NS_ORDER", "KT_NO_PACK", "KT_NO_SCAN_VIEW", "KT_NO_SWEEP", "KT_NO_VERDICT_IMAGES", "KT_NO_WG_RANGES", "KT_SYNC_INGEST", "KT_INGEST_TRUST_FENCE", "KT_NO_VIEW_PATCH", "KT_CHECK_ONE_PER_CU", "KT_AGG_SMALL_WINDOW", "KT_AGG_ONE_PER_CU", "KT_NO_MATCH_CACHE", "KT_NO_MATCH_CACHE_AGG"};
+enum EnvSwitch { kSw_FEED_NO_STAGE, kSw_FORCE_NS_ORDER, kSw_INGEST_EVENT_WAIT, kSw_NO_FEED_FEW, kSw_NO_FEED_FUSION, kSw_NO_FUSED, kSw_NO_NS_ORDER, kSw_NO_PACK, kSw_NO_SCAN_VIEW, kSw_NO_SWEEP, kSw_NO_VERDICT_IMAGES, kSw_NO_WG_RANGES, kSw_SYNC_INGEST, kSw_INGEST_TRUST_FENCE, kSw_NO_VIEW_PATCH, kSw_CHECK_ONE_PER_CU, kSw_AGG_SMALL_WINDOW, kSw_AGG_ONE_PER_CU, kSw_NO_MATCH_CACHE, kSw_NO_MATCH_CACHE_AGG, kSw_NO_MATCH_CODES, kSw_NO_MATCH_CODES_AGG, kSwCount };
+static const char* const kEnvSwitchName[kSwCount] = {"KT_FEED_NO_STAGE", "KT_FORCE_NS_ORDER", "KT_INGEST_EVENT_WAIT", "KT_NO_FEED_FEW", "KT_NO_FEED_FUSION", "KT_NO_FUSED", "KT_NO_NS_ORDER", "KT_NO_PACK", "KT_NO_SCAN_VIEW", "KT_NO_SWEEP", "KT_NO_VERDICT_IMAGES", "KT_NO_WG_RANGES", "KT_SYNC_INGEST", "KT_INGEST_TRUST_FENCE", "KT_NO_VIEW_PATCH", "KT_CHECK_ONE_PER_CU", "KT_AGG_SMALL_WINDOW", "KT_AGG_ONE_PER_CU", "KT_NO_MATCH_CACHE", "KT_NO_MATCH_CACHE_AGG", "KT_NO_MATCH_CODES", "KT_NO_MATCH_CODES_AGG"};
 struct kt_engine {
   bool sw[kSwCount] = {};
   uint32_t reprieve_lds_cap_limit = 0;
@@ -218,6 +220,7 @@
   std::atomic<int64_t> ctr_index_chunks{0}, ctr_index_words{0}, ctr_index_image_words{0}, ctr_ns_rows{0}, ctr_ns_word_visits{0}, ctr_ns_chunk_visits{0}, ctr_slow_throttles{0}, ctr_packed_words{0}, ctr_agg_workgroups{0}, ctr_view_builds{0}, ctr_mc_builds{0}, ctr_mc_scans{0}, ctr_mc_planes{0}, ctr_mc_agg_scans{0};
   DevBuf<uint16_t> d_latom;
   DevBuf<uint64_t> d_mc;
+  DevBuf<kt::MatchCodes> d_mcodes;
   int64_t* h_mc_rows = nullptr;
   hipEvent_t mc_rows_ev = nullptr;
   bool mc_rows_ev_used = false;
diff --git a/kube_throttler_amd/csrc/kt_engine_reconcile.cpp b/kube_throttler_amd/csrc/kt_engine_reconcile.cpp
--- a/kube_throttler_amd/csrc/kt_engine_reconcile.cpp
+++ b/kube_throttler_amd/csrc/kt_engine_reconcile.cpp
@@ -247,10 +247,14 @@
       if (e->last_stream) KT_HIP(e, hipStreamSynchronize(e->last_stream));
       KT_HIP(e, cv.mx.reserve(need));
     }
+    if (mc.codes && cv.mc.cap < (size_t)cv.cap + 1) {
+      if (e->last_stream) KT_HIP(e, hipStreamSynchronize(e->last_stream));
+      KT_HIP(e, cv.mc.reserve((size_t)cv.cap + 1));
+    }
     const int64_t listed = std::min<int64_t>((int64_t)cv.n + cv.extra, cv.cap);
-    kt::launch_gather_match_planes(mc.mw, mc.stride, mc.planes, cv.rows.p, listed, cv.mx.p, (uint64_t)cv.cap + 1u, s);
+    kt::launch_gather_match_planes(mc.mw, mc.stride, mc.planes, cv.rows.p, listed, cv.mx.p, (uint64_t)cv.cap + 1u, s, mc.codes, cv.mc.p);
     KT_HIP(e, hipGetLastError());
-    cv.mx_planes = mc.planes, cv.mx_valid = true;
+    cv.mx_planes = mc.planes, cv.mx_valid = true, cv.mc_there = mc.codes != nullptr;
   }
   if (words && e->clean_partial != (const void*)e->partial()) KT_HIP(e, hipMemsetAsync(e->partial(), 0, words * 8, s));
   e->clean_partial = nullptr;
@@ -284,6 +288,8 @@
         if ((rc = slab_tags(e, sc, s)) != KT_OK) return rc;
         sc.defer_reduce = defer && sc.pk != nullptr;
         if (replay && sc.by_ns && sc.v_pk && limb == 0) sc.v_mx = cv.mx.p, sc.mx_stride = (uint64_t)cv.cap + 1u, sc.mx_planes = cv.mx_planes;
+        if (sc.v_mx && mc.codes && cv.mc_there && cv.mc.p && e->dindex.runs_agree && !e->sw[kSw_NO_MATCH_CODES] && !e->sw[kSw_NO_MATCH_CODES_AGG])
+          sc.v_mc = cv.mc.p;
         const char* k = kt::launch_aggregate_indexed(e->pods, sc, e->sp, e->d_sp.p, e->dindex, target, e->d_slab.p, s,
                                                      pass == 0 ? std::function<void()>(after_scan) : std::function<void()>());
         if (sc.replayed) e->ctr_mc_agg_scans.fetch_add(1, std::memory_order_relaxed);
diff --git a/kube_throttler_amd/csrc/kt_index.cpp b/kube_throttler_amd/csrc/kt_index.cpp
--- a/kube_throttler_amd/csrc/kt_index.cpp
+++ b/kube_throttler_amd/csrc/kt_index.cpp
@@ -902,6 +902,7 @@
     for (const ChunkPlan& cp : plan_in) total_words += cp.words.size();
     out.bm_images.reserve(((size_t)Rp * total_words * 8 * fam + total_words * (sizeof(WordHdr) + 64 * 10 + 64)) * 5 / 4 + plan_in.size() * ((size_t)n_ns + 8) * 4 * 4);
     out.bm_chunk_ns.clear();
+    out.bm_runs.clear(), out.runs_agree = true;
     const uint32_t nsw = (n_ns + 31) / 32;
     out.ns_words = nsw ? nsw : 1u;
     out.bm_max_lds = 0, out.bm_max_thr = 0, out.bm_max_words = 0, out.bm_slab_bytes = 0;
@@ -993,6 +994,25 @@
       }
       ch.w0 = w_run;
       w_run += nw;
+      {
+        out.bm_runs.resize((size_t)w_run * 2, 0ull);
+        for (uint32_t w = 0; w < nw; ++w) {
+          uint64_t t_lo = 0, t_hi = 0, r_lo = 0, r_hi = 0;
+          for (uint32_t k = 0; k < 64; ++k) {
+            const size_t c = (size_t)w * 64 + k;
+            const uint32_t tt = it[c];
+            if (!(tt & kTermReal)) continue;
+            auto same_t = [&](size_t o) { return (tt & kTermAdj) && (it[o] & kTermReal) && (it[o] & kTermAdj) && ((it[o] ^ tt) & kTermRowMask) == 0u; };
+            auto same_r = [&](size_t o) { return (ir[c] & kRankAdj) && ir[o] == ir[c]; };
+            if (!(k > 0 && same_t(c - 1))) t_lo |= 1ull << k;
+            if (!(k < 63 && same_t(c + 1))) t_hi |= 1ull << k;
+            if (!(k > 0 && same_r(c - 1))) r_lo |= 1ull << k;
+            if (!(k < 63 && same_r(c + 1))) r_hi |= 1ull << k;
+          }
+          out.bm_runs[((size_t)ch.w0 + w) * 2] = t_lo, out.bm_runs[((size_t)ch.w0 + w) * 2 + 1] = t_hi;
+          if (t_lo != r_lo || t_hi != r_hi) out.runs_agree = false;
+        }
+      }
       irows.assign((size_t)Rp * (nw + veto_cols), 0ull);
       const size_t veto_plane = (size_t)Rp * nw;
       for (uint32_t r = 0; r < R; ++r)
@@ -1125,6 +1145,8 @@
   if ((e = up(d.bm_rank_t, d.cap_bm_rank_t, h.bm_rank_t, s)) != hipSuccess) return e;
   if ((e = up(d.bm_chunk_ns, d.cap_bm_chunk_ns, h.bm_chunk_ns, s)) != hipSuccess) return e;
   d.ns_words = h.ns_words;
+  d.runs_agree = h.runs_agree;
+  if ((e = up(d.bm_runs, d.cap_bm_runs, h.bm_runs, s)) != hipSuccess) return e;
   if ((e = up(d.atom_table, d.cap_atom_table, h.atom_table, s)) != hipSuccess) return e;
   d.atom_mask = (uint32_t)h.atom_table.size() - 1;
   d.h_chunks = h.bm_chunks;
@@ -1140,8 +1162,9 @@
   d.has_key_atoms = h.n_key_atoms ? 1u : 0u;
   d.la = h.la, d.rich = h.rich;
   if (getenv("KT_DEBUG_LDS"))
-    fprintf(stderr, "bitmap index: %u words, %u rows (veto %d, need %u), %zu chunks, largest LDS part %u B, largest chunk %u throttles / %u words, %zu slow throttles\n",
-            h.bm_words, h.bm_rows, (int)h.has_veto, h.max_need, h.bm_chunks.size(), h.bm_max_lds, h.bm_max_thr, h.bm_max_words, h.slow_thr.size());
+    fprintf(stderr, "bitmap index: %u words, %u rows (veto %d, need %u), %zu chunks, largest LDS part %u B, largest chunk %u throttles / %u words, %zu slow throttles, run masks of sweep and aggregate %s\n",
+            h.bm_words, h.bm_rows, (int)h.has_veto, h.max_need, h.bm_chunks.size(), h.bm_max_lds, h.bm_max_thr, h.bm_max_words, h.slow_thr.size(),
+            h.runs_agree ? "agree" : "differ");
   return hipSuccess;
 }
 
@@ -1154,6 +1177,7 @@
   if (d.nogroup) (void)hipFree(d.nogroup);
   if (d.grp_arrive) (void)hipFree(d.grp_arrive);
   if (d.bm_chunk_ns) (void)hipFree(d.bm_chunk_ns);
+  if (d.bm_runs) (void)hipFree(d.bm_runs);
   if (d.atom_table) (void)hipFree(d.atom_table);
   d = IndexDev();
 }
diff --git a/kube_throttler_amd/csrc/kt_index.h b/kube_throttler_amd/csrc/kt_index.h
--- a/kube_throttler_amd/csrc/kt_index.h
+++ b/kube_throttler_amd/csrc/kt_index.h
@@ -7,6 +7,7 @@
 #include <vector>
 
 #include "kt_device.h"
+#include "kt_match_codes.h"
 
 namespace kt {
 
@@ -89,6 +90,8 @@
   std::vector<uint32_t> thr_ngrp;
   std::vector<uint32_t> nogroup;
   std::vector<uint32_t> bm_chunk_ns;
+  std::vector<uint64_t> bm_runs;
+  bool runs_agree = true;
   uint32_t ns_words = 0;
   uint32_t bm_max_lds = 0, bm_max_thr = 0, bm_max_words = 0;
   uint64_t bm_slab_bytes = 0;
@@ -167,6 +170,9 @@
   size_t cap_thr_ngrp = 0, cap_nogroup = 0, cap_grp_arrive = 0;
   uint32_t* bm_chunk_ns = nullptr;
   uint32_t ns_words = 0;
+  uint64_t* bm_runs = nullptr;
+  bool runs_agree = true;
+  size_t cap_bm_runs = 0;
   uint64_t* atom_table = nullptr;
   uint32_t atom_mask = 0;
   std::vector<BmChunk> h_chunks;
@@ -208,14 +214,17 @@
 uint32_t check_word_lds(int D);
 constexpr int kMatchPlanes = 8;
 constexpr int kMatchReplay = 4;
+static_assert((uint32_t)kMatchReplay == kMatchCodeLists, "a match code names a list position in two bits");
 struct MatchCacheArgs {
   const uint64_t* mw = nullptr;
   uint64_t stride = 0;
   uint32_t planes = 0;
+  const MatchCodes* codes = nullptr;
   mutable bool used = false;
 };
 struct MatchViewPlanes {
   uint64_t* mx = nullptr;
+  MatchCodes* mc = nullptr;
   const int32_t* pos = nullptr;
   uint64_t stride = 0;
 };
@@ -244,6 +253,7 @@
   const uint64_t* v_mx = nullptr;
   uint64_t mx_stride = 0;
   uint32_t mx_planes = 0;
+  const MatchCodes* v_mc = nullptr;
   mutable bool replayed = false;
   mutable int launched_blocks = 0;
   mutable bool launched_packed = false;
@@ -293,9 +303,10 @@
 bool match_cache_fits(const IndexDev& ix);
 bool check_replays_match_cache(const PodTable& pods, const SelProgram& sp, const IndexDev& ix, uint32_t planes, bool overflow_pods, bool one_per_cu);
 bool launch_build_match_cache(const PodTable& pods, int64_t n, const int64_t* rows_dev, const IndexDev& ix, uint64_t* mw, uint64_t stride,
-                              uint32_t planes, hipStream_t s, const MatchViewPlanes* view = nullptr);
+                              uint32_t planes, hipStream_t s, const MatchViewPlanes* view = nullptr, MatchCodes* codes = nullptr);
 void launch_gather_match_planes(const uint64_t* mw, uint64_t stride, uint32_t planes, const int64_t* rows, int64_t n, uint64_t* mx,
-                                uint64_t mx_stride, hipStream_t s);
+                                uint64_t mx_stride, hipStream_t s, const MatchCodes* codes = nullptr, MatchCodes* vmc = nullptr);
+bool match_codes_fit(const IndexDev& ix, uint32_t planes);
 int check_sweep_blocks(int64_t n);
 size_t verdict_images_bytes(uint32_t total_words, int D);
 void launch_build_verdict_images(const IndexDev& ix, uint32_t total_words, const void* recs, int T, int D, void* out, hipStream_t s);
diff --git a/kube_throttler_amd/csrc/kt_kernels_aggregate.hip b/kube_throttler_amd/csrc/kt_kernels_aggregate.hip
--- a/kube_throttler_amd/csrc/kt_kernels_aggregate.hip
+++ b/kube_throttler_amd/csrc/kt_kernels_aggregate.hip
@@ -397,6 +397,8 @@
   const uint64_t* v_mx;
   uint64_t mx_stride;
   uint32_t mx_planes;
+  const MatchCodes* v_mc;
+  const uint64_t* runs;
   unsigned char* slab;
   BmIndexArgs ix;
   BmChunk ch;
@@ -407,9 +409,10 @@
 };
 __device__ __forceinline__ uint32_t agg_one_rec_off(uint32_t r, uint32_t rec, uint32_t skew) { return __umul24(r, rec) + (skew ? (r >> 3) << 3 : 0u); }
 
-template <bool VETO, int NEED, bool CACHED = false>
+template <bool VETO, int NEED, bool CACHED = false, bool CODES = false>
 __global__ __launch_bounds__(kBlockIx, 8) void kt_aggregate_bitmap_one(const BmAggOneArgs a) {
   static_assert(!CACHED || (!VETO && NEED == 2), "the cached form is one instantiation: nothing of the scan's form is left in it");
+  static_assert(!CODES || CACHED, "records are a form of the match cache");
   constexpr int LA = 8, NW = 3, kWq = VETO ? 3 : 4;
   KT_LDS unsigned char* lds = (KT_LDS unsigned char*)kt_smem;
   const uint32_t lane = threadIdx.x & (kWave - 1);
@@ -431,7 +434,10 @@
     Rec r{};
     const uint32_t ic = min(wt * kWave + lane, n_rows - 1u);
     r.meta = a.v_meta[ic];
-    if constexpr (CACHED) {
+    if constexpr (CODES) {
+      const u64x2 rc = *(const u64x2*)(a.v_mc + ic);
+      r.mx[0] = rc.x, r.mx[1] = rc.y;
+    } else if constexpr (CACHED) {
       const uint64_t* q = a.v_mx + ic;
 #pragma unroll
       for (int j = 0; j < kMatchReplay; ++j)
@@ -453,7 +459,7 @@
     const StageSeg segs[2] = {img, StageSeg{a.off_rank, (const u32x4*)(a.ix.blob + ch.img_off + ch.off_term_rank), ch.n_words * 8u}};
     lds_stage_segments<2, 4>(lds, segs);
   }
-  if (ch.has_adj) {
+  if (ch.has_adj && !CODES) {
     const uint16_t* g_rank = (const uint16_t*)(a.ix.blob + ch.img_off + ch.off_term_rank);
     for (uint32_t w = wave; w < ch.n_words; w += (uint32_t)(kBlockIx / kWave)) {
       const uint32_t tr = g_rank[w * 64u + lane];
@@ -481,6 +487,53 @@
     unsigned long long pw[NW];
 #pragma unroll
     for (int k = 0; k < NW; ++k) pw[k] = cur.pw[k];
+    if constexpr (CODES) {
+      auto fold = [&](bool has, uint32_t c) {
+        const uint32_t r = trank[has ? c : 0u] & 0x7FFFu;
+        if (has) {
+          KT_LDS unsigned char* rp = tab + agg_one_rec_off(r, rec, skew);
+          lds_u64wp tv = (lds_u64wp)rp;
+          lds_add64(tv, pw[0]);
+          if (pk_nw > 1u) lds_add64(tv + 1, pw[1]);
+          if (pk_nw > 2u) lds_add64(tv + 2, pw[2]);
+          if (zero_keys) (void)__hip_atomic_fetch_or((lds_u32wp)(rp + pk_nw * 8u), zero_keys, __ATOMIC_RELAXED, __HIP_MEMORY_SCOPE_WORKGROUP);
+        }
+      };
+      const u32x2 rng = bm.nsl_rng[ns];
+      const uint32_t len = counted ? min(rng.y - rng.x, a.mx_planes) : 0u;
+      uint32_t wn[kMatchReplay];
+#pragma unroll
+      for (int k = 0; k < kMatchReplay; ++k) wn[k] = bm.nsl[(uint32_t)k < len ? rng.x + (uint32_t)k : 0u].w;
+      const uint32_t w01 = wn[0] | wn[1] << 16, w23 = wn[2] | wn[3] << 16;
+      auto word_of = [&](uint32_t k) { const uint32_t wp = (k & 2u) ? w23 : w01; return (k & 1u) ? wp >> 16 : wp & 0xFFFFu; };
+      const uint32_t hdr = (uint32_t)cur.mx[0] & 0xFFu;
+      if (__ballot(counted && hdr == kMatchCodesOverflow) == 0ull) {
+        const uint32_t mine = counted ? hdr : 0u;
+        uint64_t lo = cur.mx[0] >> 8 | cur.mx[1] << 56, hi = cur.mx[1] >> 8;
+        for (uint32_t i = 0; __ballot(i < mine) != 0ull; ++i) {
+          const uint32_t cd = (uint32_t)lo & 0xFFu;
+          lo = lo >> 8 | hi << 56, hi >>= 8;
+          fold(i < mine, word_of(cd >> 6) * 64u + (cd & 63u));
+        }
+      } else {
+#pragma unroll 1
+        for (uint32_t k = 0; k < a.mx_planes; ++k) {
+          const uint32_t ic = min(wt * kWave + lane, n_rows - 1u);
+          uint64_t x = k < len ? a.v_mx[(uint64_t)k * a.mx_stride + ic] : 0ull;
+          const uint32_t w = word_of(k);
+          if (a.runs) {
+            const uint64_t* sg = a.runs + 2u * (k < len ? w : 0u);
+            x = match_run_rule(x, sg[0], sg[1]);
+          }
+          while (__ballot(x != 0ull) != 0ull) {
+            const bool has = x != 0ull;
+            const uint32_t c = has ? w * 64u + (uint32_t)__ffsll((unsigned long long)x) - 1u : 0u;
+            x &= x - 1ull;
+            fold(has, c);
+          }
+        }
+      }
+    } else {
     uint64_t qx[kWq];
     typedef typename std::conditional<(kWq > 3), uint64_t, uint32_t>::type qw_t;
     qw_t qw = 0;
@@ -536,6 +589,7 @@
       scan_tile<LA, VETO, NEED, false>(bm, counted, ns, ro, [&](bool, uint32_t) {}, [&](uint32_t) { return true; }, push_word, run_masks);
     }
     flush();
+    }
   }
   __syncthreads();
   const uint32_t slab_pitch = (ch.n_thr * rec + 15u) & ~15u;
@@ -750,20 +804,25 @@
     const bool cached = sc.v_mx != nullptr && sc.limb == 0 && sc.mx_planes >= 1u && sc.mx_planes <= (uint32_t)kMatchReplay &&
                         (uint64_t)n_rows <= sc.mx_stride && match_cache_fits(ix);
     if (cached) oa.v_mx = sc.v_mx, oa.mx_stride = sc.mx_stride, oa.mx_planes = sc.mx_planes;
+    const bool codes = cached && sc.v_mc != nullptr && (!ch.has_adj || ix.bm_runs != nullptr);
+    if (codes) oa.v_mc = sc.v_mc, oa.runs = ch.has_adj ? ix.bm_runs + (size_t)ch.w0 * 2 : nullptr;
     oa.slab = slab + (size_t)ch.slab_off * 16;
     oa.n_rows = (uint32_t)n_rows;
     oa.tpb = (uint32_t)((((n_rows + kWave - 1) / kWave) + nb - 1) / nb);
     static const bool dbg_one = getenv("KT_DEBUG_LDS") != nullptr;
     if (dbg_one)
       fprintf(stderr, "kt_aggregate_bitmap_one: lds=%u (2 per CU) workgroups=%d tiles per workgroup=%u nw=%u rec=%u skew=%u cached=%d\n", one_total, nb,
-              oa.tpb, oa.pk_nw, oa.pk_rec, oa.skew, cached ? 1 : 0);
+              oa.tpb, oa.pk_nw, oa.pk_rec, oa.skew, codes ? 2 : cached ? 1 : 0);
 #define KT_AGG_ONE_LAUNCH(VETO_, NEED_, ...)                                                                     \
   {                                                                                                             \
     auto kfn = kt_aggregate_bitmap_one<VETO_, NEED_, ##__VA_ARGS__>;                                            \
     (void)hipFuncSetAttribute((const void*)kfn, hipFuncAttributeMaxDynamicSharedMemorySize, (int)one_total);    \
     hipLaunchKernelGGL(kfn, g_, b_, one_total, s, oa);                                                          \
   }
-    if (cached) {
+    if (codes) {
+      KT_AGG_ONE_LAUNCH(false, 2, true, true)
+      sc.replayed = true;
+    } else if (cached) {
       KT_AGG_ONE_LAUNCH(false, 2, true)
       sc.replayed = true;
     } else {
diff --git a/kube_throttler_amd/csrc/kt_kernels_check.hip b/kube_throttler_amd/csrc/kt_kernels_check.hip
--- a/kube_throttler_amd/csrc/kt_kernels_check.hip
+++ b/kube_throttler_amd/csrc/kt_kernels_check.hip
@@ -597,6 +597,8 @@
   const uint8_t* ns_valid;
   const uint64_t* mw;
   uint64_t mw_stride;
+  const MatchCodes* codes;
+  const uint64_t* runs;
   const unsigned char* blob;
   BmChunk ch;
   uint32_t n;
@@ -605,20 +607,20 @@
 };
 static_assert(kTermRowMask == (1u << 20) - 1u && kWave == 64, "a list entry is lane << 20 | term number");
 
-static BmCheckCachedArgs make_check_cached_args(const IndexDev& ix, uint32_t* total) {
+static BmCheckCachedArgs make_check_cached_args(const IndexDev& ix, uint32_t* total, bool codes = false) {
   BmCheckCachedArgs a{};
   uint32_t o = 0;
   auto take = [&](uint32_t bytes) { uint32_t r = o; o += (bytes + 15u) & ~15u; return r; };
   a.off_cnt = take(kBlockIx * 8u);
   a.off_list = take((kBlockIx / kWave) * kListCap * 4);
   a.off_tinfo = take(ix.bm_max_words * 64u * 8u);
-  a.off_wv = take(ix.bm_max_words * (uint32_t)sizeof(WordVerdict<8>));
+  a.off_wv = take(codes ? 0u : ix.bm_max_words * (uint32_t)sizeof(WordVerdict<8>));
   a.lds_img = take(ix.bm_max_lds);
   *total = o;
   return a;
 }
 
-template <int PL>
+template <int PL, bool CODES = false>
 __global__ __launch_bounds__(kBlockIx, 8) void kt_check_bitmap_cached(const BmCheckCachedArgs a) {
   static_assert(PL >= 1 && PL <= kMatchReplay, "one instantiation per plane count");
   constexpr int DT = 8;
@@ -639,6 +641,24 @@
   BmIndexArgs ixa{};
   ixa.blob = a.blob, ixa.lds_img = a.lds_img;
   const BmView bm = open_chunk<false>(lds, ixa, ch);
+  struct Rec {
+    uint64_t meta;
+    uint64_t mx[CODES ? 2 : kMatchReplay];
+  };
+  auto fetch_tile = [&](uint32_t wt) {
+    Rec r{};
+    const uint32_t ic = min(wt * kWave + lane, n - 1u);
+    r.meta = ld_issued(a.meta + ic);
+    if constexpr (CODES) {
+      const uint64_t* q = (const uint64_t*)(a.codes + ic);
+      r.mx[0] = ld_issued(q), r.mx[1] = ld_issued(q + 1);
+    } else {
+      const uint64_t* q = a.mw + ic;
+#pragma unroll
+      for (int j = 0; j < PL; ++j) r.mx[j] = ld_issued(q + (uint64_t)j * a.mw_stride);
+    }
+    return r;
+  };
   {
     const uint32_t* term_t = (const uint32_t*)(a.blob + ch.img_off + ch.off_term_t);
     uint32_t tt_first = 0u;
@@ -646,24 +666,11 @@
     const StageSeg segs[1] = {StageSeg{a.lds_img + ch.off_nsl_rng, (const u32x4*)(a.blob + ch.img_off + ch.off_nsl_rng), (ch.lds_bytes - ch.off_nsl_rng) / 16u}};
     lds_stage_segments<1>(lds, segs);
     for (uint32_t c = threadIdx.x; c < ch.n_words * 64u; c += kBlockIx)
-      build_term_verdicts<DT, true>(c == threadIdx.x ? tt_first : term_t[c], c, g_rflags, tinfo, (KT_LDS WordVerdict<DT>*)(lds + a.off_wv));
+      build_term_verdicts<DT, !CODES>(c == threadIdx.x ? tt_first : term_t[c], c, g_rflags, tinfo, (KT_LDS WordVerdict<DT>*)(lds + a.off_wv));
   }
   __syncthreads();
   const bool seg_on = ch.has_adj != 0u;
 
-  struct Rec {
-    uint64_t meta;
-    uint64_t mx[kMatchReplay];
-  };
-  auto fetch_tile = [&](uint32_t wt) {
-    Rec r{};
-    const uint32_t ic = min(wt * kWave + lane, n - 1u);
-    r.meta = ld_issued(a.meta + ic);
-    const uint64_t* q = a.mw + ic;
-#pragma unroll
-    for (int j = 0; j < PL; ++j) r.mx[j] = ld_issued(q + (uint64_t)j * a.mw_stride);
-    return r;
-  };
   for (uint32_t wt = blockIdx.x * (kBlockIx / kWave) + wave; wt < n_wtiles; wt += wstep) {
     const Rec r = fetch_tile(wt);
     cnt[lane] = 0ull;
@@ -734,30 +741,93 @@
       const uint32_t ns = on ? (uint32_t)(meta & kMetaNsMask) : 0u;
       const uint32_t nz = (uint32_t)(meta >> kMetaNzShift) & 0xFFFFu;
       const uint32_t ns_ok_raw = a.ns_valid[ns];
-      auto nib_offset = [&](int q) { return (uint32_t)offsetof(WordVerdict<DT>, act_nib) + (uint32_t)q * 128u + ((nz >> (4 * q)) & 15u) * 8u; };
-      uint32_t n_exc = 0u, n_act = 0u, n_ins = 0u;
-      auto settle_word = [&](uint32_t w, uint64_t x, int) -> uint64_t {
-        KT_LDS const unsigned char* q = wv + __umul24(w, (uint32_t)sizeof(WordVerdict<DT>));
-        if (seg_on) {
-          const u64x2 seg = *(KT_LDS const u64x2*)(q + offsetof(WordVerdict<DT>, seg_lo));
-          const uint64_t v = x | seg.y;
-          x = andn_64(x, v - seg.x);
-        }
-        const u64x2 te = *(KT_LDS const u64x2*)(q + offsetof(WordVerdict<DT>, tight));
-        const u64x2 ai = *(KT_LDS const u64x2*)(q + offsetof(WordVerdict<DT>, act));
-        uint64_t act = *(KT_LDS const unsigned long long*)(q + nib_offset(0));
-#pragma unroll
-        for (int k = 1; k < DT / 4; ++k) act |= *(KT_LDS const unsigned long long*)(q + nib_offset(k));
-        const uint64_t xe = and_not_and_64(x, te.x, te.y);
-        const uint64_t xf = and_not_not_64(x, te.x, te.y);
-        const uint64_t xa = xf & act, xi = and_not_and_64(xf, act, ai.y);
-        n_exc = (uint32_t)__popc((uint32_t)xe) + ((uint32_t)__popc((uint32_t)(xe >> 32)) + n_exc);
-        n_act = (uint32_t)__popc((uint32_t)xa) + ((uint32_t)__popc((uint32_t)(xa >> 32)) + n_act);
-        n_ins = (uint32_t)__popc((uint32_t)xi) + ((uint32_t)__popc((uint32_t)(xi >> 32)) + n_ins);
-        return x & te.x;
-      };
-      replay_tile(bm, on, ns, r.mx, (uint32_t)PL, [&](bool has, uint32_t c) { push(has, lane << 20 | c); }, settle_word, ScanNoPrefetch());
-      const unsigned long long my = (unsigned long long)n_exc << 4 | (unsigned long long)n_act << 24 | (unsigned long long)n_ins << 44;
+      unsigned long long my = 0ull;
+      if constexpr (CODES) {
+        const u32x2 rng = bm.nsl_rng[ns];
+        const uint32_t len = on ? min(rng.y - rng.x, (uint32_t)PL) : 0u;
+        uint32_t wn[PL];
+#pragma unroll
+        for (int k = 0; k < PL; ++k) wn[k] = bm.nsl[(uint32_t)k < len ? rng.x + (uint32_t)k : 0u].w;
+        static_assert(kTermRowMask >> 6 <= 0xFFFFu, "a word number is a 16-bit field");
+        const uint32_t w01 = wn[0] | (PL > 1 ? wn[PL > 1 ? 1 : 0] << 16 : 0u), w23 = (PL > 2 ? wn[PL > 2 ? 2 : 0] : 0u) | (PL > 3 ? wn[PL > 3 ? 3 : 0] << 16 : 0u);
+        auto term = [&](bool has, uint32_t c, const u32x2 ti) {
+          const bool tight = (ti.y & kTiTight) != 0u;
+          const uint32_t sh = (nz & ti.y & 0xFFFFu) ? (ti.y >> kTiShActive) & 63u : (ti.y >> kTiShIdle) & 63u;
+          if (has && !tight && sh != 0u) my += 1ull << sh;
+          push(has && tight, lane << 20 | c);
+        };
+        const uint32_t hdr = (uint32_t)r.mx[0] & 0xFFu;
+        if (__ballot(on && hdr == kMatchCodesOverflow) == 0ull) {
+          const uint32_t mine = on ? hdr : 0u;
+          uint32_t top = 0u;
+          uint64_t among = ~0ull;
+#pragma unroll
+          for (int b = 3; b >= 0; --b) {
+            const uint64_t t = __ballot((mine >> b) & 1u) & among;
+            if (t != 0ull) among = t, top |= 1u << b;
+          }
+          uint64_t lo = r.mx[0] >> 8 | r.mx[1] << 56, hi = r.mx[1] >> 8;
+          auto number = [&](uint32_t cd) {
+            const uint32_t wp = (cd & 0x80u) ? w23 : w01;
+            return ((cd & 0x40u) ? wp >> 16 : wp & 0xFFFFu) * 64u + (cd & 63u);
+          };
+          constexpr uint32_t UN = 2;
+          for (uint32_t i = 0; i < top; i += UN) {
+            uint32_t c[UN];
+            u32x2 t[UN];
+#pragma unroll
+            for (uint32_t u = 0; u < UN; ++u) c[u] = number((uint32_t)(lo >> (8u * u)) & 0xFFu);
+            lo = lo >> (8u * UN) | hi << (64u - 8u * UN), hi >>= 8u * UN;
+#pragma unroll
+            for (uint32_t u = 0; u < UN; ++u) t[u] = tinfo[i + u < mine ? c[u] : 0u];
+#pragma unroll
+            for (uint32_t u = 0; u < UN; ++u) term(i + u < mine, c[u], t[u]);
+          }
+        } else {
+#pragma unroll 1
+          for (uint32_t k = 0; k < (uint32_t)PL; ++k) {
+            const uint32_t ic = min(wt * kWave + lane, n - 1u);
+            uint64_t x = k < len ? a.mw[(uint64_t)k * a.mw_stride + ic] : 0ull;
+            const uint32_t wp = (k & 2u) ? w23 : w01;
+            const uint32_t w = (k & 1u) ? wp >> 16 : wp & 0xFFFFu;
+            if (seg_on) {
+              const uint64_t* sg = a.runs + 2u * (k < len ? w : 0u);
+              x = match_run_rule(x, sg[0], sg[1]);
+            }
+            while (__ballot(x != 0ull) != 0ull) {
+              const bool has = x != 0ull;
+              const uint32_t c = has ? w * 64u + (uint32_t)__ffsll((unsigned long long)x) - 1u : 0u;
+              x &= x - 1ull;
+              term(has, c, tinfo[c]);
+            }
+          }
+        }
+      } else {
+        auto nib_offset = [&](int q) { return (uint32_t)offsetof(WordVerdict<DT>, act_nib) + (uint32_t)q * 128u + ((nz >> (4 * q)) & 15u) * 8u; };
+        uint32_t n_exc = 0u, n_act = 0u, n_ins = 0u;
+        auto settle_word = [&](uint32_t w, uint64_t x, int) -> uint64_t {
+          KT_LDS const unsigned char* q = wv + __umul24(w, (uint32_t)sizeof(WordVerdict<DT>));
+          if (seg_on) {
+            const u64x2 seg = *(KT_LDS const u64x2*)(q + offsetof(WordVerdict<DT>, seg_lo));
+            const uint64_t v = x | seg.y;
+            x = andn_64(x, v - seg.x);
+          }
+          const u64x2 te = *(KT_LDS const u64x2*)(q + offsetof(WordVerdict<DT>, tight));
+          const u64x2 ai = *(KT_LDS const u64x2*)(q + offsetof(WordVerdict<DT>, act));
+          uint64_t act = *(KT_LDS const unsigned long long*)(q + nib_offset(0));
+#pragma unroll
+          for (int k = 1; k < DT / 4; ++k) act |= *(KT_LDS const unsigned long long*)(q + nib_offset(k));
+          const uint64_t xe = and_not_and_64(x, te.x, te.y);
+          const uint64_t xf = and_not_not_64(x, te.x, te.y);
+          const uint64_t xa = xf & act, xi = and_not_and_64(xf, act, ai.y);
+          n_exc = (uint32_t)__popc((uint32_t)xe) + ((uint32_t)__popc((uint32_t)(xe >> 32)) + n_exc);
+          n_act = (uint32_t)__popc((uint32_t)xa) + ((uint32_t)__popc((uint32_t)(xa >> 32)) + n_act);
+          n_ins = (uint32_t)__popc((uint32_t)xi) + ((uint32_t)__popc((uint32_t)(xi >> 32)) + n_ins);
+          return x & te.x;
+        };
+        replay_tile(bm, on, ns, r.mx, (uint32_t)PL, [&](bool has, uint32_t c) { push(has, lane << 20 | c); }, settle_word, ScanNoPrefetch());
+        my = (unsigned long long)n_exc << 4 | (unsigned long long)n_act << 24 | (unsigned long long)n_ins << 44;
+      }
       cnt[lane] += my | (on ? 1ull : 0ull) | ((on && ns_ok_raw == 0u) ? 2ull : 0ull);
     }
     if (n_list) drain(std::integral_constant<int, 2>());
@@ -771,20 +841,24 @@
 static void launch_check_cached(const PodTable& pods, int64_t n, const SelProgram& sp, const IndexDev& ix, const void* recs, uint64_t* summary,
                                 const MatchCacheArgs& mc, dim3 grid, hipStream_t s) {
   uint32_t total = 0;
-  BmCheckCachedArgs a = make_check_cached_args(ix, &total);
+  const bool codes = mc.codes != nullptr && (!ix.h_chunks[0].has_adj || ix.bm_runs != nullptr);
+  BmCheckCachedArgs a = make_check_cached_args(ix, &total, codes);
   assert(2u * total <= (uint32_t)kMaxLds && (uint64_t)ix.bm_max_words * 64u <= (uint64_t)kTermRowMask + 1u);
   a.meta = pods.meta, a.req = pods.req, a.recs = recs, a.summary = summary, a.ns_valid = sp.ns_valid;
   a.mw = mc.mw, a.mw_stride = mc.stride;
+  if (codes) a.codes = mc.codes, a.runs = ix.bm_runs ? ix.bm_runs + (size_t)ix.h_chunks[0].w0 * 2 : nullptr;
   a.blob = ix.bm_blob, a.ch = ix.h_chunks[0];
   a.n = (uint32_t)n, a.DS = pods.DS, a.T = sp.T;
   static const bool dbg_lds = getenv("KT_DEBUG_LDS") != nullptr;
-  if (dbg_lds) fprintf(stderr, "kt_check_bitmap_cached: lds=%u (2 per CU) workgroups=%u planes=%u\n", total, grid.x, mc.planes);
-#define KT_CHECK_CACHED_LAUNCH(PL_)                                                                             \
+  if (dbg_lds) fprintf(stderr, "kt_check_bitmap_cached: lds=%u (2 per CU) workgroups=%u planes=%u %s\n", total, grid.x, mc.planes, codes ? "match codes" : "planes");
+#define KT_CHECK_CACHED_LAUNCH_(PL_, CODES_)                                                                    \
   {                                                                                                             \
-    auto kfn = kt_check_bitmap_cached<PL_>;                                                                     \
+    auto kfn = kt_check_bitmap_cached<PL_, CODES_>;                                                             \
     (void)hipFuncSetAttribute((const void*)kfn, hipFuncAttributeMaxDynamicSharedMemorySize, (int)total);        \
     hipLaunchKernelGGL(kfn, grid, dim3(kBlockIx), total, s, a);                                                 \
   }
+#define KT_CHECK_CACHED_LAUNCH(PL_) \
+  { if (codes) KT_CHECK_CACHED_LAUNCH_(PL_, true) else KT_CHECK_CACHED_LAUNCH_(PL_, false) }
   static_assert(kMatchReplay == 4, "one instantiation per plane count");
 #ifdef KT_FAST_BUILD
   KT_CHECK_CACHED_LAUNCH(kMatchReplay)
@@ -797,6 +871,7 @@
   }
 #endif
 #undef KT_CHECK_CACHED_LAUNCH
+#undef KT_CHECK_CACHED_LAUNCH_
 }
 
 #define KT_BM_LAUNCH(DT_, LA_, VETO_, NEED_, WPE_, FULL_, SMALL_, ONE_)                                         \
diff --git a/kube_throttler_amd/csrc/kt_kernels_match.hip b/kube_throttler_amd/csrc/kt_kernels_match.hip
--- a/kube_throttler_amd/csrc/kt_kernels_match.hip
+++ b/kube_throttler_amd/csrc/kt_kernels_match.hip
@@ -14,6 +14,10 @@
   uint64_t* vx;
   const int32_t* vpos;
   uint64_t vstride;
+  MatchCodes* vmc;
+  MatchCodes* mc;
+  const uint64_t* runs;
+  uint32_t off_runs;
   BmIndexArgs ix;
   BmChunk ch;
 };
@@ -26,9 +30,11 @@
   const uint32_t wave = __builtin_amdgcn_readfirstlane(threadIdx.x / kWave);
   const BmChunk& ch = a.ch;
   {
-    const StageSeg segs[1] = {chunk_image_segment(a.ix, ch)};
-    lds_stage_segments<1, 4>(lds, segs);
+    const StageSeg segs[2] = {chunk_image_segment(a.ix, ch), StageSeg{a.off_runs, (const u32x4*)a.runs, a.runs ? ch.n_words : 0u}};
+    lds_stage_segments<2, 4>(lds, segs);
   }
+  const bool codes = a.mc != nullptr, seg_on = a.runs != nullptr;
+  KT_LDS const u64x2* runs = (KT_LDS const u64x2*)(lds + a.off_runs);
   const BmView bm = open_chunk<VETO>(lds, a.ix, ch);
   __syncthreads();
   const uint32_t n = a.n, planes = a.planes;
@@ -52,14 +58,29 @@
     const bool thru = in && vj >= 0 && (uint64_t)vj < a.vstride;
     uint64_t* qv = a.vx + (thru ? (uint32_t)vj : 0u);
     uint32_t round = 0u;
+    MatchCodes rec{0ull, 0ull};
     scan_tile<LA, VETO, NEED, false>(
         bm, on, ns, ro, [&](bool, uint32_t) {}, [&](uint32_t) { return true; },
-        [&](uint32_t, uint64_t xx, int) -> uint64_t {
+        [&](uint32_t w, uint64_t xx, int) -> uint64_t {
           if (in && round < planes) q[(uint64_t)round * a.stride] = xx;
           if (thru && round < planes) qv[(uint64_t)round * a.vstride] = xx;
+          if (codes && round < kMatchCodeLists) {
+            uint64_t x = xx;
+            if (seg_on) {
+              const u64x2 seg = runs[w];
+              x = match_run_rule(x, seg.x, seg.y);
+            }
+            while (x) {
+              const uint32_t bit = (uint32_t)__ffsll((unsigned long long)x) - 1u;
+              x &= x - 1ull;
+              match_codes_append(rec, match_code(round, bit));
+            }
+          }
           round += 1u;
           return 0ull;
         });
+    if (codes && in) a.mc[pc] = rec;
+    if (codes && thru && a.vmc) a.vmc[(uint32_t)vj] = rec;
     for (; round < planes; ++round) {
       if (in) q[(uint64_t)round * a.stride] = 0ull;
       if (thru) qv[(uint64_t)round * a.vstride] = 0ull;
@@ -68,7 +89,7 @@
 }
 
 __global__ __launch_bounds__(256) void kt_gather_match_planes(const uint64_t* mw, uint64_t stride, uint32_t planes, const int64_t* rows, int64_t n,
-                                                             uint64_t* mx, uint64_t mx_stride) {
+                                                             uint64_t* mx, uint64_t mx_stride, const MatchCodes* codes, MatchCodes* vmc) {
   for (int64_t j = (int64_t)blockIdx.x * 256 + threadIdx.x; j < n; j += (int64_t)gridDim.x * 256) {
     const uint64_t p = (uint64_t)rows[j];
     if (p >= stride) continue;
@@ -78,13 +99,15 @@
 #pragma unroll
     for (int k = 0; k < kMatchReplay; ++k)
       if ((uint32_t)k < planes) mx[(uint64_t)k * mx_stride + (uint64_t)j] = x[k];
+    if (vmc) vmc[j] = codes[p];
   }
 }
 void launch_gather_match_planes(const uint64_t* mw, uint64_t stride, uint32_t planes, const int64_t* rows, int64_t n, uint64_t* mx,
-                                uint64_t mx_stride, hipStream_t s) {
+                                uint64_t mx_stride, hipStream_t s, const MatchCodes* codes, MatchCodes* vmc) {
   if (n <= 0 || !mw || !mx || planes == 0u || planes > (uint32_t)kMatchReplay || (uint64_t)n > mx_stride) return;
   const int64_t nb = std::min<int64_t>((n + 255) / 256, 4096);
-  hipLaunchKernelGGL(kt_gather_match_planes, dim3((unsigned)nb), dim3(256), 0, s, mw, stride, planes, rows, n, mx, mx_stride);
+  hipLaunchKernelGGL(kt_gather_match_planes, dim3((unsigned)nb), dim3(256), 0, s, mw, stride, planes, rows, n, mx, mx_stride, codes,
+                     codes ? vmc : nullptr);
 }
 
 bool match_cache_fits(const IndexDev& ix) {
@@ -93,19 +116,32 @@
   return !ch.has_slow && ch.n_words != 0u && ix.bm_max_lds <= (uint32_t)kMaxLds;
 }
 
+bool match_codes_fit(const IndexDev& ix, uint32_t planes) {
+  if (!match_cache_fits(ix) || planes == 0u || planes > (uint32_t)kMatchReplay) return false;
+  const BmChunk& ch = ix.h_chunks[0];
+  if (!ch.has_adj) return true;
+  return ix.bm_runs != nullptr && ((ix.bm_max_lds + 15u) & ~15u) + ch.n_words * 16u <= (uint32_t)kMaxLds;
+}
+
 bool launch_build_match_cache(const PodTable& pods, int64_t n, const int64_t* rows_dev, const IndexDev& ix, uint64_t* mw, uint64_t stride,
-                              uint32_t planes, hipStream_t s, const MatchViewPlanes* view) {
+                              uint32_t planes, hipStream_t s, const MatchViewPlanes* view, MatchCodes* codes) {
   if (n <= 0) return true;
   if (!match_cache_fits(ix) || pods.LA > 8 || !mw || planes == 0u || planes > (uint32_t)kMatchPlanes || stride == 0u || n > (int64_t)stride)
     return false;
   MatchBuildArgs a{};
   a.meta = pods.meta, a.latom = pods.latom, a.rows = rows_dev, a.mw = mw, a.stride = stride, a.planes = planes;
   a.n = (uint32_t)n, a.cap = (uint32_t)std::min<uint64_t>(stride, 0x80000000ull);
-  if (view && view->mx && view->pos && view->stride) a.vx = view->mx, a.vpos = view->pos, a.vstride = view->stride;
+  if (view && view->mx && view->pos && view->stride) a.vx = view->mx, a.vpos = view->pos, a.vstride = view->stride, a.vmc = view->mc;
   uint32_t o = 0;
   auto take = [&](uint32_t bytes) { uint32_t r = o; o += (bytes + 15u) & ~15u; return r; };
   plan_bitmap_index(ix, a.ix, take);
   a.ch = ix.h_chunks[0];
+  if (codes && match_codes_fit(ix, planes)) {
+    a.mc = codes;
+    if (a.ch.has_adj) a.runs = ix.bm_runs + (size_t)a.ch.w0 * 2, a.off_runs = take(a.ch.n_words * 16u);
+  } else {
+    a.vmc = nullptr;
+  }
   const uint32_t lds_bytes = o;
   const int64_t tiles = (n + kWave - 1) / kWave, per_wg = kBlockIx / kWave;
   const int64_t nb = std::min<int64_t>((tiles + per_wg - 1) / per_wg, 2 * kCUs);
diff --git a/kube_throttler_amd/csrc/kt_match_codes.h b/kube_throttler_amd/csrc/kt_match_codes.h
--- /dev/null
+++ b/kube_throttler_amd/csrc/kt_match_codes.h
@@ -0,0 +1,68 @@
+#pragma once
+#include <stdint.h>
+
+#if defined(__HIPCC__)
+#define KT_MC_HD __host__ __device__ inline
+#else
+#define KT_MC_HD inline
+#endif
+
+namespace kt {
+
+constexpr uint32_t kMatchCodesMax = 15;
+constexpr uint32_t kMatchCodesOverflow = 0xFFu;
+constexpr uint32_t kMatchCodeLists = 4;
+
+struct alignas(16) MatchCodes {
+  uint64_t lo, hi;
+};
+
+KT_MC_HD uint64_t match_run_rule(uint64_t x, uint64_t seg_lo, uint64_t seg_hi) {
+  const uint64_t v = x | seg_hi;
+  return x & ~(v - seg_lo);
+}
+
+KT_MC_HD uint32_t match_codes_header(const MatchCodes& r) { return (uint32_t)(r.lo & 0xFFu); }
+KT_MC_HD uint32_t match_codes_count(const MatchCodes& r) {
+  const uint32_t h = match_codes_header(r);
+  return h == kMatchCodesOverflow ? 0u : h;
+}
+KT_MC_HD uint32_t match_code_at(const MatchCodes& r, uint32_t i) {
+  const uint32_t b = i + 1u;
+  return (uint32_t)((b < 8u ? r.lo >> (8u * b) : r.hi >> (8u * (b - 8u))) & 0xFFu);
+}
+KT_MC_HD uint32_t match_code(uint32_t k, uint32_t bit) { return k << 6 | bit; }
+KT_MC_HD uint32_t match_code_list(uint32_t code) { return code >> 6; }
+KT_MC_HD uint32_t match_code_bit(uint32_t code) { return code & 63u; }
+
+KT_MC_HD void match_codes_append(MatchCodes& r, uint32_t code) {
+  const uint32_t h = match_codes_header(r);
+  if (h == kMatchCodesOverflow) return;
+  if (h >= kMatchCodesMax) {
+    r.lo |= kMatchCodesOverflow;
+    return;
+  }
+  const uint32_t b = h + 1u;
+  if (b < 8u) r.lo |= (uint64_t)(code & 0xFFu) << (8u * b);
+  else r.hi |= (uint64_t)(code & 0xFFu) << (8u * (b - 8u));
+  r.lo += 1ull;
+}
+KT_MC_HD void match_codes_append_word(MatchCodes& r, uint32_t k, uint64_t x) {
+  while (x) {
+    uint32_t bit = 0;
+    for (uint64_t t = x; !(t & 1ull); t >>= 1) ++bit;
+    x &= x - 1ull;
+    match_codes_append(r, match_code(k, bit));
+  }
+}
+KT_MC_HD uint64_t match_codes_word(const MatchCodes& r, uint32_t k) {
+  uint64_t x = 0;
+  const uint32_t n = match_codes_count(r);
+  for (uint32_t i = 0; i < n; ++i) {
+    const uint32_t c = match_code_at(r, i);
+    if (match_code_list(c) == k) x |= 1ull << match_code_bit(c);
+  }
+  return x;
+}
+
+}
diff --git a/kube_throttler_amd/engine.py b/kube_throttler_amd/engine.py
--- a/kube_throttler_amd/engine.py
+++ b/kube_throttler_amd/engine.py
@@ -38,7 +38,7 @@
     "kt_paged_admit", "kt_admit_gangs_launch", "kt_admit_gangs_fetch", "kt_paged_admit_gangs",
     "kt_headroom_launch", "kt_headroom_fetch", "kt_paged_headroom", "kt_preempt_launch", "kt_preempt_fetch",
     "kt_preempt_reprieve_launch", "kt_preempt_gangs_launch", "kt_preempt_gangs_reprieve_launch", "kt_preempt_gangs_fetch", "kt_forecast_launch", "kt_forecast_fetch", "kt_forecast_gangs_launch", "kt_forecast_gangs_fetch", "kt_override_instants",
-    "kt_paged_preempt", "kt_paged_forecast", "kt_debug_match_planes", "kt_paged_preempt_gangs",
+    "kt_paged_preempt", "kt_paged_forecast", "kt_debug_match_planes", "kt_debug_match_codes", "kt_debug_match_runs", "kt_paged_preempt_gangs",
 ]
 HEADROOM_MAX_CAP = 0x7FFFFFFF
 PREEMPT_NONE = -1
@@ -259,6 +259,9 @@
         L.kt_partial_layout.argtypes = [C.c_int32] + [C.POINTER(C.c_int32)] * 5
         L.kt_debug_reload_env.argtypes = [C.c_void_p]
         L.kt_debug_match_planes.argtypes = [C.c_void_p, C.c_int32, C.c_int64, C.c_void_p, C.c_void_p, C.POINTER(C.c_int64), C.POINTER(C.c_int32)]
+        if hasattr(L, "kt_debug_match_codes"):
+            L.kt_debug_match_runs.argtypes = [C.c_void_p, C.c_int32, C.c_int32, C.POINTER(C.c_int32), C.POINTER(C.c_uint64), C.POINTER(C.c_uint64)]
+            L.kt_debug_match_codes.argtypes =[C.c_void_p, C.c_int32, C.c_int64, C.c_void_p, C.c_void_p, C.POINTER(C.c_int64)]
         L.kt_affected_pods.argtypes = [C.c_void_p, C.c_int64, C.c_void_p, C.c_int32, C.c_void_p, C.c_void_p]
         L.kt_paged_check.argtypes = [C.POINTER(C.c_void_p), C.c_int32, C.c_int64, C.c_void_p, C.c_int32, C.c_void_p, C.c_void_p]
         L.kt_paged_reconcile.argtypes = [C.POINTER(C.c_void_p), C.c_int32, C.c_int64, C.c_int32, C.c_uint32, C.c_int32,
@@ -489,6 +492,20 @@
         self._ck(lib().kt_debug_match_planes(self._h, int(view), cap, out.ctypes.data, rows.ctypes.data if view else None, C.byref(n), C.byref(planes)))
         return out[:, :int(n.value)], (rows[:int(n.value)] if view else None)
 
+    def match_codes(self, view=False):
+        n = C.c_int64()
+        self._ck(lib().kt_debug_match_codes(self._h, int(view), 0, None, None, C.byref(n)))
+        cap = max(int(n.value), 1)
+        out = np.zeros((cap, 16), dtype=np.uint8)
+        rows = np.zeros(cap, dtype=np.int64)
+        self._ck(lib().kt_debug_match_codes(self._h, int(view), cap, out.ctypes.data, rows.ctypes.data if view else None, C.byref(n)))
+        return out[:int(n.value)], (rows[:int(n.value)] if view else None)
+
+    def match_runs(self, ns_row, k):
+        w, lo, hi = C.c_int32(), C.c_uint64(), C.c_uint64()
+        self._ck(lib().kt_debug_match_runs(self._h, int(ns_row), int(k), C.byref(w), C.byref(lo), C.byref(hi)))
+        return int(w.value), int(lo.value), int(hi.value)
+
     def index_stats(self) -> dict:
         ch, words, visits, rows, cvis, iw, slow = (int(lib().kt_counter(self._h, k)) for k in (
             COUNTER_INDEX_CHUNKS, COUNTER_INDEX_WORDS, COUNTER_NS_WORD_VISITS, COUNTER_NS_ROWS, COUNTER_NS_CHUNK_VISITS, COUNTER_INDEX_IMAGE_WORDS,
```

Measured after the change: 25190 billion decisions/s, median of 6. 1.06x the previous value.
